# dattalab-6-cam/multicam-calibration

Hardware: AMD Instinct MI355X
Metric: LM iterations/sec (6 cams x 10k frames x 54 pts per GPU shard; + ms/Jacobian-eval) (higher is better)
Workload: dtype f64

## Files before the change

multicam-calibration_amd/build.py:

```python
import hashlib
import os
import shutil
import subprocess
import sys

PKG = os.path.dirname(os.path.abspath(__file__))
CSRC = os.path.join(PKG, "csrc")
LIB = os.path.join(PKG, "libmcba.so")
SOURCES = ["mcba_kernels.hip", "mcba_solve.hip", "mcba_triangulate.hip", "mcba_diag.hip", "mcba_calib.hip", "mcba_pnp.hip", "mcba_flat.hip", "mcba_api.hip", "mcba_lm_api.hip",
           "mcba_prefilter_api.hip", "mcba_calib_api.hip", "mcba_geom_api.hip", "mcba_comm_api.hip", "mcba_sparse.hip", "mcba_sparse_api.hip", "mcba_detect.hip", "mcba_keypoints.hip", "mcba_consensus.hip", "mcba_cov.hip", "mcba_cov_api.hip",
           "mcba_tricov.hip", "mcba_tricov_api.hip", "mcba_kpba.hip", "mcba_kpba_tiled.hip", "mcba_kpba_api.hip", "mcba_kpcam.hip", "mcba_kpcam_api.hip", "mcba_twoview.hip", "mcba_fivepoint.hip", "mcba_twoview_api.hip", "mcba_resect.hip", "mcba_resect_p3p.hip", "mcba_resect_api.hip",
           "mcba_smooth.hip", "mcba_smooth_api.hip", "mcba_smooth_cov.hip", "mcba_smooth_cov_api.hip", "mcba_traj_refine.hip", "mcba_traj_refine_api.hip"]
DEPS = SOURCES + ["mcba_gram_finish.inc", "mcba_math.h", "mcba_geom_math.h", "mcba_pnp_math.h", "mcba_keypoint_math.h", "mcba_consensus_math.h", "mcba_cov_math.h", "mcba_tricov_math.h", "mcba_kpba_math.h", "mcba_kpcam_math.h", "mcba_detect_math.h", "mcba_twoview_math.h", "mcba_fivepoint_math.h", "mcba_resect_math.h", "mcba_resect_p3p_math.h", "mcba_smooth_math.h", "mcba_smooth_cov_math.h", "mcba_traj_refine_math.h", "mcba_smooth_host.h", "mcba_hyp_score.h", "mcba_ransac_host.h", "mcba_device.h", "mcba_quadform.h", "mcba_backsub.h", "mcba_kernels.h", "mcba_gram_plan.h", "mcba_lm.h", "mcba_lm_state.h", "mcba_handle.h", os.path.join("..", "..", "include", "mcba.h")]


SCHED_FLAGS = ["-mllvm", "-amdgpu-disable-unclustered-high-rp-reschedule=1", "-mllvm", "-greedy-reverse-local-assignment=1"]


def hipcc_path():
    for cand in (shutil.which("hipcc"), "/opt/rocm/bin/hipcc"):
        if cand and os.path.exists(cand):
            return cand
    raise RuntimeError("hipcc not found: libmcba.so cannot be built (ROCm toolchain required)")


def is_stale():
    if not os.path.exists(LIB):
        return True
    t = os.path.getmtime(LIB)
    return any(os.path.getmtime(os.path.join(CSRC, d)) > t for d in DEPS)


def build(force=False, verbose=False, out=None):
    if out is None and not force and not is_stale():
        return LIB
    from concurrent.futures import ThreadPoolExecutor

    extra = os.environ.get("MCBA_HIPCC_FLAGS", "").split()
    common = [hipcc_path(), "-O3", "--offload-arch=gfx950", "-std=c++17", "-fPIC"] + SCHED_FLAGS + extra
    tag = hashlib.sha1(repr((out, common[1:])).encode()).hexdigest()[:12]
    objdir = os.path.join(CSRC, ".obj" if out is None and not extra else ".obj_" + tag)
    os.makedirs(objdir, exist_ok=True)
    flags_file = os.path.join(objdir, "flags.txt")
    flags_now = " ".join(common[1:])
    flags_same = os.path.exists(flags_file) and open(flags_file).read() == flags_now
    headers = [os.path.join(CSRC, d) for d in DEPS if d not in SOURCES]
    hdr_time = max(os.path.getmtime(hh) for hh in headers)

    def compile_one(src):
        obj = os.path.join(objdir, src.replace(".hip", ".o"))
        srcp = os.path.join(CSRC, src)
        if not force and flags_same and os.path.exists(obj) and os.path.getmtime(obj) > max(os.path.getmtime(srcp), hdr_time):
            return obj
        tmp = obj + ".%d.tmp" % os.getpid()
        cmd = common + ["-c", "-o", tmp, srcp]
        if verbose:
            print(" ".join(cmd))
        subprocess.check_call(cmd, cwd=CSRC)
        os.replace(tmp, obj)
        return obj

    with ThreadPoolExecutor(max_workers=min(len(SOURCES), os.cpu_count() or 2, 16)) as ex:
        objs = list(ex.map(compile_one, SOURCES))
    with open(flags_file, "w") as fh:
        fh.write(flags_now)
    target = out or LIB
    tmp_lib = target + ".%d.tmp" % os.getpid()
    cmd = [hipcc_path(), "--offload-arch=gfx950", "-fPIC", "-shared", "-o", tmp_lib, "-ldl"] + objs
    if verbose:
        print(" ".join(cmd))
    subprocess.check_call(cmd, cwd=CSRC)
    os.replace(tmp_lib, target)
    return target


if __name__ == "__main__":
    out = sys.argv[sys.argv.index("--out") + 1] if "--out" in sys.argv else None
    print(build(force="--force" in sys.argv, verbose=True, out=out))
```

multicam-calibration_amd/csrc/mcba_api.hip:

```cpp
#include <map>
#include <mutex>

#include "mcba_handle.h"

namespace mcba_internal {

thread_local std::string g_err;

struct ParkedBuf {
  void* p;
  hipStream_t stream;
  bool busy;
};
struct BufferPool {
  std::mutex mu;
  std::multimap<std::pair<int, size_t>, ParkedBuf> dev;
  std::multimap<std::pair<unsigned, size_t>, void*> host;
  size_t parked = 0, parked_host = 0;
  const size_t host_cap = (size_t)256 << 20;
  size_t cap() {
    static size_t c = [] { const char* e = getenv("MCBA_POOL_MB"); return (size_t)(e ? atoll(e) : 2048) << 20; }();
    return c;
  }
};
static BufferPool g_pool;

static void pool_release_all();
hipError_t pool_malloc(void** p, size_t bytes, int device, hipStream_t stream, bool any_stream) {
  {
    ParkedBuf got{nullptr, nullptr, false};
    {
      std::lock_guard<std::mutex> lk(g_pool.mu);
      auto it = g_pool.dev.find({device, bytes});
      if (it != g_pool.dev.end()) { got = it->second; g_pool.dev.erase(it); g_pool.parked -= bytes; }
    }
    if (got.p) {
      if (got.busy && (any_stream || got.stream != stream)) (void)hipStreamSynchronize(got.stream);
      *p = got.p;
      return hipSuccess;
    }
  }
  hipError_t e = hipMalloc(p, bytes);
  if (e == hipErrorOutOfMemory) {
    (void)hipGetLastError();
    pool_release_all();
    e = hipMalloc(p, bytes);
  }
  return e;
}
void pool_free(void* p, size_t bytes, int device, hipStream_t stream, bool busy) {
  if (!p) return;
  {
    std::lock_guard<std::mutex> lk(g_pool.mu);
    if (g_pool.parked + bytes <= g_pool.cap()) { g_pool.dev.insert({{device, bytes}, ParkedBuf{p, stream, busy}}); g_pool.parked += bytes; return; }
  }
  if (busy) (void)hipStreamSynchronize(stream);
  (void)hipFree(p);
}
hipError_t pool_host_malloc(void** p, size_t bytes, unsigned flags) {
  {
    std::lock_guard<std::mutex> lk(g_pool.mu);
    auto it = g_pool.host.find({flags, bytes});
    if (it != g_pool.host.end()) { *p = it->second; g_pool.host.erase(it); g_pool.parked_host -= bytes; return hipSuccess; }
  }
  return hipHostMalloc(p, bytes, flags);
}
void pool_host_free(void* p, size_t bytes, unsigned flags) {
  if (!p) return;
  std::lock_guard<std::mutex> lk(g_pool.mu);
  if (g_pool.cap() == 0 || g_pool.parked_host + bytes > g_pool.host_cap) { (void)hipHostFree(p); return; }
  g_pool.host.insert({{flags, bytes}, p});
  g_pool.parked_host += bytes;
}
static void pool_release_all() {
  std::lock_guard<std::mutex> lk(g_pool.mu);
  int cur = 0;
  (void)hipGetDevice(&cur);
  for (auto& kv : g_pool.dev) { (void)hipSetDevice(kv.first.first); if (kv.second.busy) (void)hipStreamSynchronize(kv.second.stream); (void)hipFree(kv.second.p); }
  for (auto& kv : g_pool.host) (void)hipHostFree(kv.second);
  g_pool.dev.clear();
  g_pool.host.clear();
  g_pool.parked = g_pool.parked_host = 0;
  (void)hipSetDevice(cur);
}

int poison_byte() {
  static const int b = [] { const char* e = getenv("MCBA_POISON"); const int v = e ? atoi(e) : 0; return v == 1 ? 0xFF : (v == 2 ? 0x3F : 0); }();
  return b;
}

}

using namespace mcba_internal;

static int tile_tables(int device, int NT, int** ti, int** tj) {
  static std::mutex mu;
  static std::map<std::pair<int, int>, std::pair<int*, int*>> cache;
  std::lock_guard<std::mutex> lk(mu);
  auto it = cache.find({device, NT});
  if (it == cache.end()) {
    std::vector<int> ci, cj;
    for (int a = 0; a < NT; ++a) for (int b = a; b < NT; ++b) { ci.push_back(a); cj.push_back(b); }
    int *di = nullptr, *dj = nullptr;
    HIPCHK(hipMalloc(reinterpret_cast<void**>(&di), ci.size() * sizeof(int)));
    HIPCHK(hipMalloc(reinterpret_cast<void**>(&dj), cj.size() * sizeof(int)));
    HIPCHK(hipMemcpy(di, ci.data(), ci.size() * sizeof(int), hipMemcpyHostToDevice));
    HIPCHK(hipMemcpy(dj, cj.data(), cj.size() * sizeof(int), hipMemcpyHostToDevice));
    it = cache.insert({{device, NT}, {di, dj}}).first;
  }
  *ti = it->second.first;
  *tj = it->second.second;
  return MCBA_OK;
}

static int derive_geometry(mcba_handle* h) {
  const int C = h->C, F = h->F, N = h->N, device = h->device;
  const int ncu = h->ncu, slots = 4 * h->ncu;
  h->n = h->cw * C;
  h->nsys = (size_t)h->n * h->n + 3 * h->n + 16;
  if (h->sparse) {
    h->NT = h->NP = h->G = h->sq = h->sr = 0;
    h->FS = 0;
    h->ppw = 4;
  } else {
  h->NT = (h->n + 1 + 15) / 16;
  h->NP = h->NT * (h->NT + 1) / 2;
  h->ppw = h->NP <= 64 ? 4 : 16;
  h->FS = 8;
  while (h->FS > 2 && (mcba::syrk_lds_bytes(C, h->FS, h->cw) > (size_t)h->lds_optin * 3 / 5 || (h->n + 1) * h->FS > 256 * mcba::syrk_items_per_thread())) h->FS /= 2;
  if ((h->n + 1) * h->FS > 256 * mcba::syrk_items_per_thread()) { return fail(MCBA_ERR_ARG, "too many cameras for k_syrk's per-thread item budget"); }
  if (mcba::syrk_lds_bytes(C, h->FS, h->cw) > (size_t)h->lds_optin) { return fail(MCBA_ERR_ARG, "too many cameras for the LDS staging of k_syrk"); }
  {
    int nstage = (F + h->FS - 1) / h->FS;
    int gmax = h->ppw == 4 ? std::min(512, 2 * ncu) : std::max(1, ncu / ((h->NP + 63) / 64));
    int g = std::min(nstage, gmax);
    if (h->ppw == 4) {
      h->G = g;
      h->sq = nstage / g;
      h->sr = nstage % g;
    } else {
      h->sq = (nstage + g - 1) / g;
      h->sr = 0;
      h->G = (nstage + h->sq - 1) / h->sq;
    }
  }
  }
  h->nbblocks = h->Fpad / 64;
  {
    static bool ps_ready[64] = {};
    static std::mutex ps_mu;
    bool ps_ok = (size_t)h->lds_optin >= mcba::kGramPsplitLdsMax + 2048;
    {
      std::lock_guard<std::mutex> lk(ps_mu);
      if (ps_ok && !ps_ready[device & 63]) { ps_ok = mcba::gram_psplit_set_lds_limit() == 0; ps_ready[device & 63] = ps_ok; (void)hipGetLastError(); }
    }
    mcba::GramShape shape{C, h->nfb, N, slots, h->cw, ps_ok, -1, -1};
    if (const char* e = getenv("MCBA_GRAM_SPLIT")) shape.force_split = std::max(0, std::min(5, atoi(e)));
    if (const char* e = getenv("MCBA_GRAM_NPW")) shape.force_npw = atoi(e) == 2 ? 2 : 4;
    h->gram = mcba::gram_plan(shape);
    if (h->gram.refused) { return fail(MCBA_ERR_ARG, "MCBA_GRAM_SPLIT=4/5: this device cannot give k_gram_psplit its LDS"); }
  }
  h->nch = std::max(1, std::min(std::min(8, N / 8), (4 * slots + C * h->nfb - 1) / (C * h->nfb)));
  h->nfblocks = h->G;
  h->npad = 16 * h->NT;
  h->solve_lds = mcba::solve_fits_lds(h->npad, h->lds_optin);
  if (h->sparse) {
    h->nfblocks = h->nfb;
    h->npad = mcba::sp_npad(h->n);
    h->solve_lds = 0;
  }
  return MCBA_OK;
}

static int compose_dscale(mcba_handle* h) {
  const bool any_frozen = !h->frozen_host.empty();
  h->have_red = false;
  if (h->xs_host.empty() && !any_frozen) { h->have_xscale = false; return MCBA_OK; }
  std::vector<double> d(h->nx, 0.0);
  const size_t cnt = (size_t)12 * h->C + (size_t)6 * h->F, ncam = (size_t)12 * h->C;
  for (size_t i = 0; i < cnt; ++i) {
    d[i] = h->xs_host.empty() ? 0.0 : h->xs_host[i];
    if (any_frozen && i >= ncam && h->frozen_host[i]) d[i] = -1.0;
  }
  HIPCHK(hipMemcpyAsync(h->dscale, d.data(), h->nx * sizeof(double), hipMemcpyHostToDevice, h->stream));
  HIPCHK(hipStreamSynchronize(h->stream));
  h->have_xscale = true;
  return MCBA_OK;
}

static int ensure_res(mcba_handle* h) {
  if (!h->res) return dalloc(h, &h->res, (size_t)2 * h->C * h->F * h->N, false);
  return MCBA_OK;
}


namespace mcba_internal {

int ensure_solver(mcba_handle* h) {
  if (h->have_solver) return MCBA_OK;
  const int C = h->C;
  int rc;
  if (!h->solver_arena) {
    struct Piece { double** p; size_t count; };
    size_t n_swork = h->solve_lds ? 16 : 2 * (size_t)h->npad * h->npad + 64 * (size_t)h->npad;
    if (h->sparse) n_swork = (size_t)h->npad * h->npad;
    Piece zeroed[] = {{&h->gpart2[0], (size_t)C * h->nfb * MCBA_GP}, {&h->gpart2[1], (size_t)C * h->nfb * MCBA_GP}, {&h->fbuf, (size_t)h->Fpad * MCBA_FB}, {&h->fpart, (size_t)2 * h->nfblocks},
                      {&h->cpart, (size_t)2 * C * h->nfb * h->nch}, {&h->bpart, (size_t)3 * h->nbblocks}, {&h->red_own, h->nsys + 8 + 2 * MCBA_LMS},
                      {&h->dcbuf, (size_t)h->n + 8},
                      {&h->swork, n_swork}, {&h->dscale, h->nx}, {reinterpret_cast<double**>(&h->fixed), ((size_t)h->n + 7) / 8},
                      {&h->sp_damp, h->sparse ? (size_t)h->npad : 0}, {&h->sp_y, h->sparse ? (size_t)h->npad : 0}, {reinterpret_cast<double**>(&h->sp_ctl), h->sparse ? (size_t)1 : 0}};
    Piece plain[] = {{&h->rec2[0], (size_t)h->Fpad * C * MCBA_REC}, {&h->rec2[1], (size_t)h->Fpad * C * MCBA_REC},
                     {&h->spart, (size_t)h->G * h->NP * 256 + 64},
                     {&h->gchunk, h->gram.chunk_doubles()}};
    auto padded = [](size_t count) { return (std::max<size_t>(count, 1) * sizeof(double) + 255) / 256 * 256; };
    size_t zero_bytes = 0, total = 0;
    for (auto& pc : zeroed) if (pc.count) zero_bytes += padded(pc.count);
    total = zero_bytes;
    for (auto& pc : plain) if (pc.count) total += padded(pc.count);
    if ((rc = dalloc(h, &h->solver_arena, total, false)) != MCBA_OK) return rc;
    HIPCHK(hipMemsetAsync(h->solver_arena, 0, zero_bytes, h->stream));
    if (poison_byte()) HIPCHK(hipMemsetAsync(h->solver_arena + zero_bytes, poison_byte(), total - zero_bytes, h->stream));
    size_t off = 0;
    for (auto& pc : zeroed) if (pc.count) { *pc.p = reinterpret_cast<double*>(h->solver_arena + off); off += padded(pc.count); }
    for (auto& pc : plain) if (pc.count) { *pc.p = reinterpret_cast<double*>(h->solver_arena + off); off += padded(pc.count); }
  }
  if (h->sparse) {
    h->sp_A = h->swork;
  } else if (mcba::solve_set_lds_limit(h->npad, h->solve_lds) != 0) return fail(MCBA_ERR_HIP, "cannot raise the dynamic LDS limit of k_solve_cam");
  h->fuse_backsub = h->solve_lds != 0;
  if (const char* e = getenv("MCBA_FUSE_BACKSUB")) h->fuse_backsub = h->fuse_backsub && atoi(e) != 0;
  if (h->fuse_backsub && mcba::solve_backsub_set_lds_limit(h->npad, h->cw) != 0) h->fuse_backsub = false;
  h->fuse_max_polls = 200000;
  if (const char* e = getenv("MCBA_FUSE_MAX_POLLS")) h->fuse_max_polls = std::max(0, atoi(e));
  if (!h->ring) {
    h->ring_bytes = ((size_t)kRing * MCBA_LMS + 8) * sizeof(double);
    h->ring_flags = hipHostMallocMapped | hipHostMallocCoherent;
    hipError_t e = pool_host_malloc(reinterpret_cast<void**>(&h->ring), h->ring_bytes, h->ring_flags);
    if (e != hipSuccess) { (void)hipGetLastError(); h->ring_flags = hipHostMallocDefault; e = pool_host_malloc(reinterpret_cast<void**>(&h->ring), h->ring_bytes, h->ring_flags); }
    if (e != hipSuccess) return fail(MCBA_ERR_HIP, "cannot allocate the host-mapped LM state ring");
    memset(h->ring, 0, h->ring_bytes);
    if (hipHostGetDevicePointer(reinterpret_cast<void**>(&h->ring_dev), h->ring, 0) != hipSuccess) return fail(MCBA_ERR_HIP, "hipHostGetDevicePointer failed for the LM state ring");
  }
  h->red = h->red_own;
  if (!h->sparse && (rc = tile_tables(h->device, h->NT, &h->tile_i, &h->tile_j)) != MCBA_OK) return rc;
  if (!h->pinned) {
    h->pinned_bytes = (h->nsys + 8 + MCBA_LMS + h->n) * sizeof(double);
    HIPCHK(pool_host_malloc(reinterpret_cast<void**>(&h->pinned), h->pinned_bytes, hipHostMallocDefault));
  }
  size_t lds = h->sparse ? 0 : mcba::syrk_lds_bytes(C, h->FS, h->cw);
  if (lds > 64 * 1024) {
    if (mcba::syrk_set_lds_limit(lds) != 0) return fail(MCBA_ERR_HIP, "cannot raise the dynamic LDS limit of k_syrk");
  }
  h->have_solver = true;
  if (!h->xs_host.empty() || !h->frozen_host.empty()) return compose_dscale(h);
  return MCBA_OK;
}
int upload_impl(mcba_handle* h, const double* uvs, const double* objpoints, bool sync) {
  size_t raw_count = (size_t)2 * h->C * h->F * h->N;
  hipError_t e = hipMemcpyAsync(h->obs_raw, uvs, raw_count * sizeof(double), hipMemcpyHostToDevice, h->stream);
  if (e == hipSuccess && !mcba::launch_store_small(h->stream, h->obj, objpoints, (size_t)3 * h->N))
    e = hipMemcpyAsync(h->obj, objpoints, (size_t)3 * h->N * sizeof(double), hipMemcpyHostToDevice, h->stream);
  if (e == hipSuccess) {
    Scope sc(h, K_TRANSPOSE);
    mcba::launch_transpose_obs(h->stream, h->obs_raw, h->obs_t, h->C, h->F, h->N, h->Fpad);
  }
  if (e == hipSuccess) e = hipGetLastError();
  hipError_t e2 = sync ? hipStreamSynchronize(h->stream) : hipSuccess;
  if (e != hipSuccess || e2 != hipSuccess) { g_err = std::string("upload: ") + hipGetErrorString(e != hipSuccess ? e : e2); return MCBA_ERR_HIP; }
  if (!h->obj_host) h->obj_host = static_cast<double*>(malloc((size_t)3 * h->N * sizeof(double)));
  if (h->obj_host) memcpy(h->obj_host, objpoints, (size_t)3 * h->N * sizeof(double));
  h->planar = 1;
  for (int p = 0; p < h->N; ++p) if (objpoints[3 * p + 2] != 0.0) h->planar = 0;
  if (const char* e = getenv("MCBA_GRAM_FAST")) { if (atoi(e) == 0) h->planar = 0; }
  h->have_obs = true;
  h->have_lin = h->have_red = h->have_jac = false;
  h->sp_ready = false;
  return MCBA_OK;
}

int gram_launch(mcba_handle* h, mcba::Sel sel, const double* xa, const double* xb, int la, int lb) {
  sel.cfl = h->curv_floor;
  { Scope sc(h, K_GRAM); mcba::launch_gram(h->stream, h->loss, h->f_scale, h->obs_t, h->obj, sel, xa, xb, h->rec2[la], h->rec2[lb], h->gpart2[la], h->gpart2[lb], h->C, h->N, h->Fpad, h->gram, h->planar, h->gchunk, h->loss_tab); }
  return check_launch();
}

int trial_sum(mcba_handle* h, mcba::Sel sel, int la, int lb, const mcba::DecideArgs& da) {
  { Scope sc(h, K_SUM_TRIAL); mcba::launch_sum_trial(h->stream, sel, h->gpart2[la] + (size_t)90 * h->nfb, h->gpart2[lb] + (size_t)90 * h->nfb, 1, h->nfb, (size_t)MCBA_GP * h->nfb, h->C * h->nfb, h->bpart, h->nbblocks, h->red + h->nsys, da); }
  return check_launch();
}

int backsub_launch(mcba_handle* h, mcba::Sel sel, int la, int lb, int xa, int xb, const double* delta_cam) {
  if (h->sparse && delta_cam) {
    HIPCHK(hipMemcpyAsync(h->dcbuf, delta_cam, (size_t)h->n * sizeof(double), hipMemcpyHostToDevice, h->stream));
    delta_cam = nullptr;
  }
  mcba::CamStep cs;
  if (delta_cam) memcpy(cs.v, delta_cam, h->n * sizeof(double));
  {
    Scope sc(h, K_BACKSUB);
    if (delta_cam) mcba::launch_backsub(h->stream, sel, h->rec2[la], h->rec2[lb], h->fbuf, cs, h->x[xa], h->x[xb], h->bpart, h->C, h->F, h->Fpad, h->cw);
    else mcba::launch_backsub_dev(h->stream, sel, h->rec2[la], h->rec2[lb], h->fbuf, h->dcbuf, h->x[xa], h->x[xb], h->bpart, h->C, h->F, h->Fpad, h->cw);
  }
  return check_launch();
}

int syrk_launch(mcba_handle* h, mcba::Sel sel, const mcba::SyrkFuse& fz) {
  if (h->sparse) {
    if (fz.decide) return fail(MCBA_ERR_ARG, "sparse-Schur handle: the decision is not fused into the Schur reduction");
    return sparse_build(h, sel);
  }
  { Scope sc(h, K_SYRK); mcba::launch_syrk(h->stream, sel, fz, h->rec2[0], h->rec2[1], h->fbuf, h->fpart, h->tile_i, h->tile_j, h->spart, h->C, h->F, h->Fpad, h->NT, h->NP, h->G, h->sq, h->sr, h->FS, h->ppw, h->have_xscale ? h->dscale : nullptr, h->cw); }
  return check_launch();
}

int reduce_launch(mcba_handle* h, mcba::Sel sel, int rank_slot, bool spec) {
  {
    Scope sc(h, K_REDUCE);
    mcba::launch_reduce_system(h->stream, sel, h->gpart2[0], h->gpart2[1], h->spart, h->fpart, h->tile_i, h->tile_j, h->red, h->C, h->nfb, h->G, h->NT, h->NP, h->nfblocks, rank_slot,
                               spec ? h->bpart : nullptr, h->nbblocks, spec ? post_state(h) : nullptr, h->cw, spec ? timeout_word(h) : nullptr, (double)h->last_solve_seq);
  }
  return check_launch();
}

}

extern "C" {

int mcba_abi_version(void) { return 7; }
const char* mcba_last_error(void) { return g_err.c_str(); }
const char* mcba_profile_names(void) { return kKernelNames; }

int mcba_device_count(int* count) {
  if (!count) return fail(MCBA_ERR_ARG, "count is NULL");
  hipError_t e = hipGetDeviceCount(count);
  if (e != hipSuccess) { *count = 0; g_err = hipGetErrorString(e); return MCBA_ERR_NODEVICE; }
  return MCBA_OK;
}

}

namespace mcba_internal {
int create_impl(mcba_handle** out, int C, int F, int N, int device, bool sparse) {
  const char* who = sparse ? "mcba_create_sparse" : "mcba_create";
  if (!out || C < 1 || F < 1 || N < 1) { g_err = std::string(who) + ": need cameras >= 1, frames >= 1, points >= 1"; return MCBA_ERR_ARG; }
  if (!sparse && C > 40) {
    g_err = "mcba_create: " + std::to_string(C) + " cameras -- this build handles at most 40 per handle: the (12 C + 1)-row reduced camera system is factorised by ONE workgroup "
            "(k_solve_cam: tile tables, LDS and scratch are sized for 481 rows) and k_backsub takes the camera step through the kernel arguments (480 doubles); reduced_solver=\"host\" does not "
            "lift it (the Schur product's tile grid has the same bound).  The reference has no such limit (scipy's sparse LSMR); the sparse-Schur handle (mcba_create_sparse; ops.Problem(..., schur=\"sparse\"), bundle_adjust's default above 40 cameras) has none";
    return MCBA_ERR_ARG;
  }
  int ndev = 0;
  if (hipGetDeviceCount(&ndev) != hipSuccess || ndev == 0) return fail(MCBA_ERR_NODEVICE, "no HIP device visible");
  if (device < 0 || device >= ndev) return fail(MCBA_ERR_ARG, "device ordinal out of range");
  HIPCHK(hipSetDevice(device));
  mcba_handle* h = new mcba_handle();
  h->C = C; h->F = F; h->N = N; h->device = device;
  h->sparse = sparse;
  h->speculate = !sparse;
  {
    hipDeviceProp_t prop;
    if (hipGetDeviceProperties(&prop, device) == hipSuccess) {
      if (prop.multiProcessorCount > 0) h->ncu = prop.multiProcessorCount;
      if (prop.sharedMemPerBlockOptin > 0) h->lds_optin = (int)std::min<size_t>(prop.sharedMemPerBlockOptin, 160 * 1024);
    }
  }
  if (const char* e = getenv("MCBA_STRICT_SYNC")) h->strict_sync = atoi(e) != 0;
  h->Fpad = (F + 63) / 64 * 64;
  h->nfb = h->Fpad / 64;
  h->nx = (size_t)12 * C + (size_t)6 * h->Fpad;
  {
    const int grc = derive_geometry(h);
    if (grc != MCBA_OK) { delete h; return grc; }
  }
  int rc;
#define DA(p, cnt, zero) if ((rc = dalloc(h, &h->p, (cnt), zero)) != MCBA_OK) { mcba_destroy(h); return rc; }
  DA(obs_t, (size_t)2 * C * N * h->Fpad, false);
  DA(obs_raw, (size_t)2 * C * F * N, false);
  {
    const size_t nxp = (h->nx + 31) / 32 * 32;
    DA(core_arena, 2 * nxp + (size_t)3 * N, true);
    h->x[0] = h->core_arena; h->x[1] = h->core_arena + nxp; h->obj = h->core_arena + 2 * nxp;
  }
#undef DA
  *out = h;
  return MCBA_OK;
}
}

extern "C" {

int mcba_create(mcba_handle** out, int C, int F, int N, int device) { return create_impl(out, C, F, N, device, false); }

int mcba_create_sparse(mcba_handle** out, int C, int F, int N, int device) { return create_impl(out, C, F, N, device, true); }
int mcba_is_sparse(const mcba_handle* h) { return h && h->sparse ? 1 : 0; }

int mcba_destroy(mcba_handle* h) {
  if (!h) return MCBA_OK;
  (void)hipSetDevice(h->device);
  const bool quiet = h->last_solve_seq == h->waited_seq && h->evs.empty() && !h->comm && !h->prof;
  if (!quiet) (void)hipStreamSynchronize(h->stream);
  if (h->comm && g_rccl.ok) { g_rccl.CommDestroy(h->comm); h->comm = nullptr; }
  for (auto& b : h->bufs) { pool_free(*b.slot, b.bytes, h->device, h->stream, quiet); *b.slot = nullptr; }
  free(h->obj_host);
  pool_host_free(h->pinned, h->pinned_bytes, hipHostMallocDefault);
  pool_host_free(h->ring, h->ring_bytes, h->ring_flags);
  pool_host_free(h->pf_host, h->pf_host_bytes, hipHostMallocDefault);
  for (auto& e : h->evs) { (void)hipEventDestroy(e.a); (void)hipEventDestroy(e.b); }
  for (auto& e : h->pool) (void)hipEventDestroy(e);
  delete h;
  return MCBA_OK;
}

size_t mcba_device_bytes(const mcba_handle* h) {
  size_t tot = 0;
  if (h) for (auto& b : h->bufs) tot += b.bytes;
  return tot;
}

int mcba_trim(mcba_handle* h) {
  if (!h) return fail(MCBA_ERR_ARG, "NULL handle");
  HIPCHK(hipSetDevice(h->device));
  HIPCHK(hipStreamSynchronize(h->stream));
  void** keep[] = {reinterpret_cast<void**>(&h->obs_t), reinterpret_cast<void**>(&h->obs_raw), reinterpret_cast<void**>(&h->core_arena), reinterpret_cast<void**>(&h->sub_frames),
                   reinterpret_cast<void**>(&h->blo), reinterpret_cast<void**>(&h->bhi)};
  std::vector<DevBuf> kept;
  for (auto& b : h->bufs) {
    bool k = false;
    for (void** s : keep) k = k || b.slot == s;
    if (k) { kept.push_back(b); continue; }
    pool_free(*b.slot, b.bytes, h->device);
    *b.slot = nullptr;
  }
  h->bufs.swap(kept);
  h->rec2[0] = h->rec2[1] = h->gpart2[0] = h->gpart2[1] = h->fbuf = h->fpart = h->spart = h->cpart = h->bpart = h->red_own = h->red = h->dcbuf = h->swork = h->dscale = h->gchunk = nullptr;
  h->fixed = nullptr;
  sparse_forget(h);
  h->cal_out_cap = h->cal_rel_cap = h->cal_sel_cap = h->cal_views_cap = 0;
  h->have_cal_poses = false;
  h->have_solver = h->have_lin = h->have_red = h->have_spec = h->have_jac = h->auto_ready = h->have_xscale = h->have_fixed = h->trial_ready = false;
  return MCBA_OK;
}

int mcba_download_observations(mcba_handle* h, double* uvs) {
  if (!h || !uvs) return fail(MCBA_ERR_ARG, "mcba_download_observations: bad argument");
  if (!h->have_obs) return fail(MCBA_ERR_ARG, "mcba_download_observations: no observations");
  HIPCHK(hipSetDevice(h->device));
  HIPCHK(hipMemcpyAsync(uvs, h->obs_raw, (size_t)2 * h->C * h->F * h->N * sizeof(double), hipMemcpyDeviceToHost, h->stream));
  HIPCHK(hipStreamSynchronize(h->stream));
  return MCBA_OK;
}

int mcba_pool_trim(void) {
  pool_release_all();
  return MCBA_OK;
}

int mcba_set_stream(mcba_handle* h, void* s) {
  if (!h) return fail(MCBA_ERR_ARG, "NULL handle");
  if (h->stream != reinterpret_cast<hipStream_t>(s)) HIPCHK(hipStreamSynchronize(h->stream));
  h->stream = reinterpret_cast<hipStream_t>(s);
  return MCBA_OK;
}

int mcba_synchronize(mcba_handle* h) {
  if (!h) return fail(MCBA_ERR_ARG, "NULL handle");
  HIPCHK(hipStreamSynchronize(h->stream));
  return MCBA_OK;
}

int mcba_upload_observations(mcba_handle* h, const double* uvs, const double* objpoints) {
  if (!h || !uvs || !objpoints) return fail(MCBA_ERR_ARG, "mcba_upload_observations: NULL argument");
  HIPCHK(hipSetDevice(h->device));
  return upload_impl(h, uvs, objpoints, true);
}

int mcba_set_loss(mcba_handle* h, int loss, double f_scale) {
  if (!h || loss < 0 || loss > 4 || !(f_scale > 0.0)) return fail(MCBA_ERR_ARG, "mcba_set_loss: loss in 0..4 and f_scale > 0 required");
  h->loss = loss; h->f_scale = f_scale;
  h->have_lin = h->have_red = false;
  return MCBA_OK;
}

int mcba_set_loss_table(mcba_handle* h, const double* tab3) {
  if (!h || !tab3) return fail(MCBA_ERR_ARG, "mcba_set_loss_table: NULL argument");
  if (!h->have_obs) return fail(MCBA_ERR_ARG, "mcba_set_loss_table: upload observations first");
  HIPCHK(hipSetDevice(h->device));
  int rc = ensure_res(h);
  if (rc) return rc;
  const size_t raw = (size_t)2 * h->C * h->F * h->N, plane = (size_t)2 * h->C * h->N * h->Fpad;
  if (!h->loss_tab && (rc = dalloc(h, &h->loss_tab, 3 * plane, false))) return rc;
  for (int k = 0; k < 3; ++k) {
    HIPCHK(hipMemcpyAsync(h->res, tab3 + k * raw, raw * sizeof(double), hipMemcpyHostToDevice, h->stream));
    mcba::launch_transpose_obs(h->stream, h->res, h->loss_tab + k * plane, h->C, h->F, h->N, h->Fpad);
  }
  if ((rc = check_launch())) return rc;
  HIPCHK(hipStreamSynchronize(h->stream));
  h->loss = mcba::LOSS_TABLE;
  h->f_scale = 1.0;
  h->have_lin = h->have_red = false;
  return MCBA_OK;
}

int mcba_set_camera_block(mcba_handle* h, int width) {
  if (!h || (width != 6 && width != 12)) return fail(MCBA_ERR_ARG, "mcba_set_camera_block: width 6 or 12");
  if (width == h->cw) return MCBA_OK;
  if (h->have_solver || h->solver_arena) return fail(MCBA_ERR_ARG, "mcba_set_camera_block: call it before the first solver entry point of the handle");
  if (width == 6 && !h->sparse) {
    const int nt = (6 * h->C + 1 + 15) / 16;
    if (nt * (nt + 1) / 2 > 64) return fail(MCBA_ERR_ARG, "mcba_set_camera_block: more than 26 cameras -- hold the intrinsics with the flags of mcba_lm_auto_config instead");
  }
  const int old = h->cw;
  h->cw = width;
  HIPCHK(hipSetDevice(h->device));
  const int rc = derive_geometry(h);
  if (rc != MCBA_OK) { h->cw = old; (void)derive_geometry(h); return rc; }
  h->have_lin = h->have_red = h->have_spec = false;
  h->auto_ready = false;
  return MCBA_OK;
}
int mcba_get_camera_block(const mcba_handle* h) { return h ? h->cw : 0; }

int mcba_set_curvature_floor(mcba_handle* h, double floor) {
  if (!h || !(floor > 0.0) || floor > 1.0) return fail(MCBA_ERR_ARG, "mcba_set_curvature_floor: 0 < floor <= 1");
  h->curv_floor = floor;
  return MCBA_OK;
}
double mcba_get_curvature_floor(const mcba_handle* h) { return h ? h->curv_floor : 0.0; }

int mcba_set_params(mcba_handle* h, int slot, const double* x) {
  if (!slot_ok(h, slot) || !x) return fail(MCBA_ERR_ARG, "mcba_set_params: bad handle/slot/pointer");
  HIPCHK(hipSetDevice(h->device));
  HIPCHK(hipMemcpyAsync(h->x[slot], x, ((size_t)12 * h->C + (size_t)6 * h->F) * sizeof(double), hipMemcpyHostToDevice, h->stream));
  HIPCHK(hipStreamSynchronize(h->stream));
  return MCBA_OK;
}

int mcba_get_params(mcba_handle* h, int slot, double* x) {
  if (!slot_ok(h, slot) || !x) return fail(MCBA_ERR_ARG, "mcba_get_params: bad handle/slot/pointer");
  HIPCHK(hipSetDevice(h->device));
  HIPCHK(hipMemcpyAsync(x, h->x[slot], ((size_t)12 * h->C + (size_t)6 * h->F) * sizeof(double), hipMemcpyDeviceToHost, h->stream));
  HIPCHK(hipStreamSynchronize(h->stream));
  return MCBA_OK;
}

int mcba_copy_params(mcba_handle* h, int dst, int src) {
  if (!slot_ok(h, dst) || !slot_ok(h, src)) return fail(MCBA_ERR_ARG, "mcba_copy_params: bad slot");
  if (dst == src) return MCBA_OK;
  HIPCHK(hipMemcpyAsync(h->x[dst], h->x[src], h->nx * sizeof(double), hipMemcpyDeviceToDevice, h->stream));
  return MCBA_OK;
}

static int run_cost(mcba_handle* h, int slot, double* res_dev, const double* bpart, int nbp) {
  {
    Scope sc(h, K_COST);
    mcba::launch_cost(h->stream, h->loss, h->f_scale, h->obs_t, h->obj, h->x[slot], h->cpart, res_dev, h->C, h->F, h->N, h->Fpad, h->nch);
  }
  int rc = check_launch();
  if (rc) return rc;
  {
    Scope sc(h, K_SUM_TRIAL);
    mcba::launch_sum_trial(h->stream, host_sel(0), h->cpart, h->cpart, 2, h->C * h->nfb * h->nch, 0, h->C * h->nfb * h->nch, bpart, nbp, h->red + h->nsys, mcba::DecideArgs{0, 0.0, 0.0, 0.0, 0.0, 0.0, nullptr});
  }
  return check_launch();
}

static int fetch_trial(mcba_handle* h, double* host8) {
  HIPCHK(hipMemcpyAsync(h->pinned + h->nsys, h->red + h->nsys, 8 * sizeof(double), hipMemcpyDeviceToHost, h->stream));
  HIPCHK(hipStreamSynchronize(h->stream));
  memcpy(host8, h->pinned + h->nsys, 8 * sizeof(double));
  return MCBA_OK;
}

int mcba_cost(mcba_handle* h, int slot, double* cost, double* n_residuals) {
  if (!slot_ok(h, slot) || !cost) return fail(MCBA_ERR_ARG, "mcba_cost: bad argument");
  if (!h->have_obs) return fail(MCBA_ERR_ARG, "mcba_cost: upload observations first");
  HIPCHK(hipSetDevice(h->device));
  NEED_SOLVER(h);
  int rc = run_cost(h, slot, nullptr, nullptr, 0);
  if (rc) return rc;
  double t[8];
  rc = fetch_trial(h, t);
  if (rc) return rc;
  *cost = t[0];
  if (n_residuals) *n_residuals = t[4];
  if (!isfinite(t[0])) return fail(MCBA_ERR_NONFINITE, "Residuals are not finite");
  return MCBA_OK;
}

int mcba_residuals(mcba_handle* h, int slot, double* res) {
  if (!slot_ok(h, slot) || !res) return fail(MCBA_ERR_ARG, "mcba_residuals: bad argument");
  if (!h->have_obs) return fail(MCBA_ERR_ARG, "mcba_residuals: upload observations first");
  HIPCHK(hipSetDevice(h->device));
  NEED_SOLVER(h);
  int rc = ensure_res(h);
  if (rc) return rc;
  rc = run_cost(h, slot, h->res, nullptr, 0);
  if (rc) return rc;
  HIPCHK(hipMemcpyAsync(res, h->res, (size_t)2 * h->C * h->F * h->N * sizeof(double), hipMemcpyDeviceToHost, h->stream));
  HIPCHK(hipStreamSynchronize(h->stream));
  return MCBA_OK;
}

int mcba_jacobian_eval(mcba_handle* h, int slot, int robust_scaled) {
  if (!slot_ok(h, slot)) return fail(MCBA_ERR_ARG, "mcba_jacobian_eval: bad argument");
  if (!h->have_obs) return fail(MCBA_ERR_ARG, "mcba_jacobian_eval: upload observations first");
  HIPCHK(hipSetDevice(h->device));
  int rc = ensure_res(h);
  if (rc) return rc;
  if (!h->jac) {
    rc = dalloc(h, &h->jac, (size_t)36 * h->C * h->F * h->N, false);
    if (rc) return rc;
  }
  {
    Scope sc(h, K_JACOBIAN);
    mcba::launch_jacobian(h->stream, h->loss, h->f_scale, h->obs_raw, h->obj, h->x[slot], h->jac, h->res, h->C, h->F, h->N, h->Fpad, robust_scaled);
  }
  rc = check_launch();
  if (rc) return rc;
  h->have_jac = true;
  return MCBA_OK;
}

int mcba_jacobian_download(mcba_handle* h, double* jac, double* res) {
  if (!h) return fail(MCBA_ERR_ARG, "NULL handle");
  if (!h->have_jac) return fail(MCBA_ERR_ARG, "mcba_jacobian_download: call mcba_jacobian_eval first");
  size_t cnt = (size_t)h->C * h->F * h->N;
  if (jac) HIPCHK(hipMemcpyAsync(jac, h->jac, cnt * 36 * sizeof(double), hipMemcpyDeviceToHost, h->stream));
  if (res) HIPCHK(hipMemcpyAsync(res, h->res, cnt * 2 * sizeof(double), hipMemcpyDeviceToHost, h->stream));
  HIPCHK(hipStreamSynchronize(h->stream));
  return MCBA_OK;
}

int mcba_linearize(mcba_handle* h, int slot) {
  if (!slot_ok(h, slot)) return fail(MCBA_ERR_ARG, "mcba_linearize: bad argument");
  if (!h->have_obs) return fail(MCBA_ERR_ARG, "mcba_linearize: upload observations first");
  if (h->loss == mcba::LOSS_TABLE && !h->loss_tab) return fail(MCBA_ERR_ARG, "mcba_linearize: the loss table was released (mcba_trim): call mcba_set_loss_table again");
  HIPCHK(hipSetDevice(h->device));
  NEED_SOLVER(h);
  int rc = gram_launch(h, host_sel(0), h->x[slot], h->x[slot], h->lin, h->lin);
  if (rc) return rc;
  h->have_lin = true;
  h->have_red = false;
  h->have_spec = false;
  return MCBA_OK;
}

int mcba_build_reduced(mcba_handle* h, double lambda, int rank_slot) {
  if (!h || !(lambda >= 0.0) || rank_slot < 0 || rank_slot > 11) return fail(MCBA_ERR_ARG, "mcba_build_reduced: lambda >= 0 and rank_slot in 0..11 required");
  if (!h->have_lin) return fail(MCBA_ERR_ARG, "mcba_build_reduced: call mcba_linearize first");
  HIPCHK(hipSetDevice(h->device));
  int rc;
  if ((rc = syrk_launch(h, host_sel(h->lin, lambda), no_fuse()))) return rc;
  if ((rc = reduce_launch(h, host_sel(h->lin), rank_slot, false))) return rc;
  h->have_red = true;
  return MCBA_OK;
}

size_t mcba_reduced_size(const mcba_handle* h) { return h ? h->nsys + 8 + 2 * MCBA_LMS : 0; }

int mcba_bind_reduce_buffer(mcba_handle* h, double* p) {
  if (!h) return fail(MCBA_ERR_ARG, "NULL handle");
  HIPCHK(hipSetDevice(h->device));
  NEED_SOLVER(h);
  h->red = p ? p : h->red_own;
  h->have_red = false;
  return MCBA_OK;
}

int mcba_get_reduced(mcba_handle* h, double* host) {
  if (!h || !host) return fail(MCBA_ERR_ARG, "mcba_get_reduced: bad argument");
  if (!h->have_red) return fail(MCBA_ERR_ARG, "mcba_get_reduced: call mcba_build_reduced first");
  HIPCHK(hipMemcpyAsync(h->pinned, h->red, h->nsys * sizeof(double), hipMemcpyDeviceToHost, h->stream));
  HIPCHK(hipStreamSynchronize(h->stream));
  memcpy(host, h->pinned, h->nsys * sizeof(double));
  return MCBA_OK;
}

static int step_common(mcba_handle* h, const double* delta_cam, double lambda, int src, int dst) {
  int rc = backsub_launch(h, host_sel(0, lambda), h->lin, h->lin, src, dst, delta_cam);
  if (rc || !h->have_bounds) return rc;
  mcba::launch_clip(h->stream, h->x[dst], h->blo, h->bhi, (size_t)12 * h->C + (size_t)6 * h->F);
  return check_launch();
}

int mcba_step(mcba_handle* h, const double* delta_cam, double lambda, int src, int dst) {
  if (!slot_ok(h, src) || !slot_ok(h, dst) || src == dst || !delta_cam) return fail(MCBA_ERR_ARG, "mcba_step: bad argument (slots must differ)");
  if (!h->have_red) return fail(MCBA_ERR_ARG, "mcba_step: call mcba_build_reduced first");
  HIPCHK(hipSetDevice(h->device));
  int rc = step_common(h, delta_cam, lambda, src, dst);
  if (rc) return rc;
  h->have_spec = false;
  return run_cost(h, dst, nullptr, h->bpart, h->nbblocks);
}

int mcba_step_linearize(mcba_handle* h, const double* delta_cam, double lambda, int src, int dst) {
  if (!slot_ok(h, src) || !slot_ok(h, dst) || src == dst || !delta_cam) return fail(MCBA_ERR_ARG, "mcba_step_linearize: bad argument (slots must differ)");
  if (!h->have_red) return fail(MCBA_ERR_ARG, "mcba_step_linearize: call mcba_build_reduced first");
  if (h->loss == mcba::LOSS_TABLE) return fail(MCBA_ERR_ARG, "mcba_step_linearize: a tabulated loss is set -- step (mcba_step), evaluate the function at the trial residuals, mcba_set_loss_table, then mcba_linearize");
  HIPCHK(hipSetDevice(h->device));
  int rc = step_common(h, delta_cam, lambda, src, dst);
  if (rc) return rc;
  const int alt = 1 - h->lin;
  if ((rc = gram_launch(h, host_sel(0), h->x[dst], h->x[dst], alt, alt))) return rc;
  if ((rc = trial_sum(h, host_sel(0), alt, alt, mcba::DecideArgs{0, 0.0, 0.0, 0.0, 0.0, 0.0, nullptr}))) return rc;
  h->have_spec = true;
  return MCBA_OK;
}

int mcba_accept_linearization(mcba_handle* h) {
  if (!h) return fail(MCBA_ERR_ARG, "NULL handle");
  if (!h->have_spec) return fail(MCBA_ERR_ARG, "mcba_accept_linearization: no speculative linearisation (call mcba_step_linearize first)");
  h->lin = 1 - h->lin;
  h->have_spec = false;
  h->have_red = false;
  return MCBA_OK;
}

int mcba_get_trial(mcba_handle* h, double* host8) {
  if (!h || !host8) return fail(MCBA_ERR_ARG, "mcba_get_trial: bad argument");
  return fetch_trial(h, host8);
}

int mcba_set_trial(mcba_handle* h, const double* host8) {
  if (!h || !host8 || !h->red) return fail(MCBA_ERR_ARG, "mcba_set_trial: bad argument, or no reduce buffer yet (call mcba_step first)");
  HIPCHK(hipSetDevice(h->device));
  memcpy(h->pinned + h->nsys, host8, 8 * sizeof(double));
  HIPCHK(hipMemcpyAsync(h->red + h->nsys, h->pinned + h->nsys, 8 * sizeof(double), hipMemcpyHostToDevice, h->stream));
  HIPCHK(hipStreamSynchronize(h->stream));
  return MCBA_OK;
}

int mcba_reduce_fetch(mcba_handle* h, double lambda, int rank_slot, double* host) {
  int rc = mcba_build_reduced(h, lambda, rank_slot);
  if (rc) return rc;
  return mcba_get_reduced(h, host);
}

int mcba_step_fetch(mcba_handle* h, const double* delta_cam, double lambda, int src, int dst, int linearize, double* host8) {
  int rc = linearize ? mcba_step_linearize(h, delta_cam, lambda, src, dst) : mcba_step(h, delta_cam, lambda, src, dst);
  if (rc) return rc;
  return mcba_get_trial(h, host8);
}

int mcba_set_x_scale(mcba_handle* h, const double* x_scale) {
  if (!h) return fail(MCBA_ERR_ARG, "NULL handle");
  HIPCHK(hipSetDevice(h->device));
  NEED_SOLVER(h);
  if (!x_scale) {
    if (h->xs_host.empty() && h->frozen_host.empty()) { h->have_red = false; h->have_xscale = false; return MCBA_OK; }
    h->xs_host.clear();
    return compose_dscale(h);
  }
  const size_t cnt = (size_t)12 * h->C + (size_t)6 * h->F;
  std::vector<double> d(cnt);
  for (size_t i = 0; i < cnt; ++i) {
    if (!(x_scale[i] > 0.0) || !std::isfinite(x_scale[i])) return fail(MCBA_ERR_ARG, "`x_scale` must be 'jac' or array_like with positive numbers.");
    d[i] = 1.0 / (x_scale[i] * x_scale[i]);
  }
  h->xs_host.swap(d);
  return compose_dscale(h);
}

int mcba_set_frozen(mcba_handle* h, const unsigned char* mask) {
  if (!h) return fail(MCBA_ERR_ARG, "NULL handle");
  HIPCHK(hipSetDevice(h->device));
  NEED_SOLVER(h);
  const size_t cnt = (size_t)12 * h->C + (size_t)6 * h->F, ncam = (size_t)12 * h->C;
  bool any = false;
  if (mask) for (size_t i = ncam; i < cnt; ++i) any = any || mask[i] != 0;
  if (!any) {
    if (h->frozen_host.empty()) return MCBA_OK;
    h->frozen_host.clear();
    return compose_dscale(h);
  }
  h->frozen_host.assign(mask, mask + cnt);
  return compose_dscale(h);
}

int mcba_set_bounds(mcba_handle* h, const double* lo, const double* hi) {
  if (!h || (lo == nullptr) != (hi == nullptr)) return fail(MCBA_ERR_ARG, "mcba_set_bounds: bad argument");
  HIPCHK(hipSetDevice(h->device));
  if (!lo) { h->have_bounds = false; return MCBA_OK; }
  const size_t cnt = (size_t)12 * h->C + (size_t)6 * h->F;
  for (size_t i = 0; i < cnt; ++i)
    if (!(lo[i] < hi[i])) return fail(MCBA_ERR_ARG, "Each lower bound must be strictly less than each upper bound.");
  int rc;
  if (!h->blo && (rc = dalloc(h, &h->blo, h->nx, false))) return rc;
  if (!h->bhi && (rc = dalloc(h, &h->bhi, h->nx, false))) return rc;
  std::vector<double> a(h->nx, -INFINITY), b(h->nx, INFINITY);
  memcpy(a.data(), lo, cnt * sizeof(double));
  memcpy(b.data(), hi, cnt * sizeof(double));
  HIPCHK(hipMemcpyAsync(h->blo, a.data(), h->nx * sizeof(double), hipMemcpyHostToDevice, h->stream));
  HIPCHK(hipMemcpyAsync(h->bhi, b.data(), h->nx * sizeof(double), hipMemcpyHostToDevice, h->stream));
  HIPCHK(hipStreamSynchronize(h->stream));
  h->have_bounds = true;
  return MCBA_OK;
}


int mcba_residuals_detach(mcba_handle* h, int slot, mcba_buffer** out) {
  if (!slot_ok(h, slot) || !out) return fail(MCBA_ERR_ARG, "mcba_residuals_detach: bad argument");
  if (!h->have_obs) return fail(MCBA_ERR_ARG, "mcba_residuals_detach: upload observations first");
  HIPCHK(hipSetDevice(h->device));
  NEED_SOLVER(h);
  int rc = ensure_res(h);
  if (rc) return rc;
  {
    Scope sc(h, K_COST);
    mcba::launch_cost(h->stream, h->loss, h->f_scale, h->obs_t, h->obj, h->x[slot], h->cpart, h->res, h->C, h->F, h->N, h->Fpad, h->nch, NAN);
  }
  if ((rc = check_launch())) return rc;
  mcba_buffer* b = new mcba_buffer{h->res, (size_t)2 * h->C * h->F * h->N, h->device, h->stream, h->res, (size_t)2 * h->C * h->F * h->N};
  for (size_t i = 0; i < h->bufs.size(); ++i)
    if (h->bufs[i].slot == reinterpret_cast<void**>(&h->res)) { h->bufs.erase(h->bufs.begin() + i); break; }
  h->res = nullptr;
  h->have_jac = false;
  *out = b;
  return MCBA_OK;
}
size_t mcba_buffer_count(const mcba_buffer* b) { return b ? b->count : 0; }
int mcba_buffer_download(mcba_buffer* b, double* host) {
  if (!b || !host) return fail(MCBA_ERR_ARG, "mcba_buffer_download: bad argument");
  HIPCHK(hipSetDevice(b->device));
  HIPCHK(hipMemcpyAsync(host, b->dev, b->count * sizeof(double), hipMemcpyDeviceToHost, b->stream));
  HIPCHK(hipStreamSynchronize(b->stream));
  return MCBA_OK;
}
int mcba_buffer_free(mcba_buffer* b) {
  if (!b) return MCBA_OK;
  (void)hipSetDevice(b->device);
  pool_free(b->base, b->base_count * sizeof(double), b->device, b->stream, true);
  delete b;
  return MCBA_OK;
}
int mcba_fp64_issue_rate(int device, double* tflops) {
  if (!tflops) return fail(MCBA_ERR_ARG, "mcba_fp64_issue_rate: NULL");
  *tflops = 0.0;
  if (int rc = stateless_device(device)) return rc;
  hipDeviceProp_t prop;
  int ncu = 256;
  if (hipGetDeviceProperties(&prop, device) == hipSuccess && prop.multiProcessorCount > 0) ncu = prop.multiProcessorCount;
  *tflops = mcba::measure_fp64_issue_rate(ncu);
  if (!(*tflops > 0.0)) return fail(MCBA_ERR_HIP, "mcba_fp64_issue_rate: the measurement kernel failed");
  return MCBA_OK;
}

int mcba_profile_enable(mcba_handle* h, int on) {
  if (!h) return fail(MCBA_ERR_ARG, "NULL handle");
  h->prof = on != 0;
  h->prof_mask = (on == 0 || on == 1) ? ~0u : ((unsigned)on >> 1);
  h->prof_stride = 1;
  h->prof_exact = false;
  return MCBA_OK;
}

int mcba_profile_exact(mcba_handle* h, int on) {
  if (!h) return fail(MCBA_ERR_ARG, "NULL handle");
  h->prof_exact = on != 0;
  return MCBA_OK;
}

int mcba_profile_stride(mcba_handle* h, int stride) {
  if (!h || stride < 1) return fail(MCBA_ERR_ARG, "mcba_profile_stride: stride >= 1 required");
  h->prof_stride = stride;
  return MCBA_OK;
}

int mcba_profile_bracket_overhead(mcba_handle* h, int pairs, double* us) {
  if (!h || !us || pairs < 1 || pairs > 4096) return fail(MCBA_ERR_ARG, "mcba_profile_bracket_overhead: bad argument");
  HIPCHK(hipSetDevice(h->device));
  std::vector<hipEvent_t> ev(2 * (size_t)pairs);
  for (auto& e : ev) HIPCHK(hipEventCreate(&e));
  HIPCHK(hipStreamSynchronize(h->stream));
  for (int i = 0; i < pairs; ++i) { HIPCHK(hipEventRecord(ev[2 * i], h->stream)); HIPCHK(hipEventRecord(ev[2 * i + 1], h->stream)); }
  HIPCHK(hipStreamSynchronize(h->stream));
  double tot = 0.0;
  for (int i = 0; i < pairs; ++i) { float ms = 0.f; HIPCHK(hipEventElapsedTime(&ms, ev[2 * i], ev[2 * i + 1])); tot += ms; }
  for (auto& e : ev) (void)hipEventDestroy(e);
  *us = 1e3 * tot / pairs;
  return MCBA_OK;
}

int mcba_profile_read(mcba_handle* h, double* ms_total, int* calls, int capacity, int* n_kernels) {
  if (!h || !ms_total || !calls || capacity < K_COUNT) return fail(MCBA_ERR_ARG, "mcba_profile_read: need capacity >= number of kernels");
  HIPCHK(hipStreamSynchronize(h->stream));
  for (int i = 0; i < K_COUNT; ++i) { ms_total[i] = 0.0; calls[i] = 0; }
  for (auto& e : h->evs) {
    float ms = 0.f;
    if (hipEventElapsedTime(&ms, e.a, e.b) == hipSuccess) { ms_total[e.kid] += ms; calls[e.kid] += 1; }
    h->pool.push_back(e.a);
    h->pool.push_back(e.b);
  }
  h->evs.clear();
  if (n_kernels) *n_kernels = K_COUNT;
  return MCBA_OK;
}

}
```

multicam-calibration_amd/csrc/mcba_handle.h:

```cpp
#pragma once
#include <hip/hip_runtime.h>
#include <math.h>
#include <stdlib.h>
#include <string.h>
#include <algorithm>
#include <rccl/rccl.h>
#include <string>
#include <vector>

#include "../../include/mcba.h"
#include "mcba_kernels.h"
#include "mcba_math.h"

namespace mcba_internal {

extern thread_local std::string g_err;

enum KernelId { K_TRANSPOSE = 0, K_GRAM, K_COST, K_SYRK, K_REDUCE, K_BACKSUB, K_SUM_TRIAL, K_JACOBIAN, K_DECIDE, K_SOLVE,
                K_SP_FACTOR, K_SP_PAIRS, K_SP_SOLVE_PRE, K_SP_POTRF, K_SP_TRSM, K_SP_UPDATE, K_SP_FINISH, K_COUNT };
constexpr const char* kKernelNames = "k_transpose_obs\nk_gram\nk_cost\nk_syrk\nk_reduce_system\nk_backsub\nk_sum_trial\nk_jacobian\nk_decide\nk_solve_cam"
                                     "\nk_sp_factor\nk_sp_pairs\nk_sp_solve_pre\nk_sp_potrf\nk_sp_trsm\nk_sp_update\nk_sp_finish";
constexpr int kRing = 16;

struct EvRec { int kid; hipEvent_t a, b; };
struct DevBuf { void** slot; size_t bytes; };

}

struct mcba_handle {
  int C = 0, F = 0, N = 0, Fpad = 0, nfb = 0, n = 0;
  int device = 0;
  hipStream_t stream = nullptr;
  int loss = MCBA_LOSS_SOFT_L1;
  double f_scale = 1.0;
  bool have_obs = false, have_lin = false, have_red = false, have_jac = false;
  double *obs_t = nullptr, *obs_raw = nullptr, *obj = nullptr, *x[2] = {nullptr, nullptr};
  double *rec2[2] = {nullptr, nullptr}, *gpart2[2] = {nullptr, nullptr}, *fbuf = nullptr, *fpart = nullptr;
  int lin = 0;
  bool have_spec = false;
  double *spart = nullptr, *cpart = nullptr, *bpart = nullptr;
  double *red_own = nullptr, *red = nullptr;
  double *jac = nullptr, *res = nullptr;
  double *err = nullptr, *dmean = nullptr, *dfull = nullptr, *repro = nullptr, *trans = nullptr, *und = nullptr;
  mcba::SelState* sel = nullptr;
  unsigned char* fmask = nullptr;
  unsigned char *pf_state = nullptr, *pf_status = nullptr, *pf_packed = nullptr, *pf_host = nullptr;
  double* pf_worst = nullptr;
  size_t pf_host_bytes = 0;
  double* core_arena = nullptr;
  unsigned char* solver_arena = nullptr;
  int* sub_frames = nullptr;
  double* cov_work = nullptr;
  double* outbuf = nullptr;
  double *cal_intr = nullptr, *cal_poses_t = nullptr, *cal_out = nullptr, *cal_rel = nullptr, *cal_world = nullptr;
  unsigned char *cal_valid = nullptr, *cal_nit = nullptr;
  mcba::SelState* cal_sel = nullptr;
  int* cal_views = nullptr;
  size_t cal_out_cap = 0, cal_rel_cap = 0, cal_sel_cap = 0, cal_views_cap = 0;
  bool have_cal_poses = false;
  double* obj_host = nullptr;
  int planar = 0;
  int *tile_i = nullptr, *tile_j = nullptr;
  int NT = 0, NP = 0, G = 0, sq = 0, sr = 0, FS = 0, ppw = 4, nfblocks = 0, nbblocks = 0, nch = 1;
  mcba::GramPlan gram;
  double* gchunk = nullptr;
  double curv_floor = 1.0;
  int cw = 12;
  size_t nx = 0, nsys = 0;
  double* pinned = nullptr;
  ncclComm_t comm = nullptr;
  double *dcbuf = nullptr, *swork = nullptr;
  double* dscale = nullptr;
  bool have_xscale = false;
  std::vector<double> xs_host;
  std::vector<unsigned char> frozen_host;
  double *blo = nullptr, *bhi = nullptr;
  bool have_bounds = false;
  double* loss_tab = nullptr;
  int fuse_max_polls = 200000;
  bool strict_sync = true;
  unsigned char* fixed = nullptr;
  bool have_fixed = false, auto_ready = false;
  bool speculate = true;
  double* ring = nullptr;
  double* ring_dev = nullptr;
  int npad = 0, solve_lds = 0;
  bool fuse_backsub = false, trial_ready = false;
  unsigned long long last_solve_seq = 0;
  unsigned long long waited_seq = 0;
  unsigned long long solve_launches = 0;
  int ncu = 256, lds_optin = 160 * 1024;
  bool spec_copy_ready = false;
  double ftol = 1e-8, xtol = 1e-8, gtol = 1e-8, lam_min = 1e-12, lam_max = 1e12;
  double dec_floor = 0.0;
  bool prof = false;
  unsigned prof_mask = ~0u;
  int prof_stride = 1;
  bool prof_exact = false;
  unsigned prof_count[32] = {};
  std::vector<mcba_internal::EvRec> evs;
  std::vector<hipEvent_t> pool;
  std::vector<mcba_internal::DevBuf> bufs;
  std::vector<double> hist;
  bool have_solver = false;
  size_t ring_bytes = 0, pinned_bytes = 0;
  unsigned ring_flags = 0;
  bool sparse = false, sp_ready = false;
  int sp_nent = 0, sp_npairs = 0, sp_nchunks = 0;
  int *sp_index = nullptr, *sp_frame_off = nullptr, *sp_ent_cam = nullptr, *sp_ent_frame = nullptr, *sp_items = nullptr, *sp_chunks = nullptr, *sp_pair_map = nullptr, *sp_pair_chunks = nullptr;
  int* sp_ctl = nullptr;
  double *sp_Y = nullptr, *sp_part = nullptr, *sp_A = nullptr, *sp_damp = nullptr, *sp_y = nullptr;
  size_t sp_index_ints = 0, sp_Y_count = 0, sp_part_count = 0;
};

struct mcba_buffer { double* dev; size_t count; int device; hipStream_t stream; double* base; size_t base_count; };

namespace mcba_internal {

#define HIPCHK(expr)                                                                                     \
  do {                                                                                                   \
    hipError_t e_ = (expr);                                                                              \
    if (e_ != hipSuccess) {                                                                              \
      mcba_internal::g_err = std::string(#expr) + ": " + hipGetErrorString(e_);                          \
      return MCBA_ERR_HIP;                                                                               \
    }                                                                                                    \
  } while (0)

inline int fail(int code, const char* msg) { g_err = msg; return code; }

inline int check_launch() {
  hipError_t e = hipGetLastError();
  if (e != hipSuccess) { g_err = std::string("kernel launch: ") + hipGetErrorString(e); return MCBA_ERR_HIP; }
  return MCBA_OK;
}

inline hipEvent_t get_event(mcba_handle* h) {
  if (!h->pool.empty()) { hipEvent_t e = h->pool.back(); h->pool.pop_back(); return e; }
  hipEvent_t e;
  (void)hipEventCreate(&e);
  return e;
}

struct Scope {
  mcba_handle* h; int kid; hipEvent_t a{}, b{};
  bool on, exact;
  Scope(mcba_handle* h_, int k) : h(h_), kid(k), on(h_->prof && ((h_->prof_mask >> k) & 1u) && (h_->prof_count[k]++ % (unsigned)h_->prof_stride) == 0), exact(false) {
    if (!on) return;
    a = get_event(h); b = get_event(h);
    exact = h->prof_exact && k == K_GRAM;
    if (exact) mcba::gram_time_next_launch(a, b);
    else (void)hipEventRecord(a, h->stream);
  }
  ~Scope() {
    if (!on) return;
    if (exact && mcba::gram_time_pending()) {
      mcba::gram_time_next_launch(nullptr, nullptr);
      h->pool.push_back(a); h->pool.push_back(b);
      return;
    }
    if (!exact) (void)hipEventRecord(b, h->stream);
    h->evs.push_back({kid, a, b});
  }
};

hipError_t pool_malloc(void** p, size_t bytes, int device, hipStream_t stream = nullptr, bool any_stream = false);
void pool_free(void* p, size_t bytes, int device, hipStream_t stream = nullptr, bool busy = false);
hipError_t pool_host_malloc(void** p, size_t bytes, unsigned flags);
void pool_host_free(void* p, size_t bytes, unsigned flags);
int poison_byte();

template <class T>
int dalloc(mcba_handle* h, T** p, size_t count, bool zero = true) {
  const size_t bytes = std::max<size_t>(count, 1) * sizeof(T);
  HIPCHK(pool_malloc(reinterpret_cast<void**>(p), bytes, h->device, h->stream));
  h->bufs.push_back({reinterpret_cast<void**>(p), bytes});
  if (zero) HIPCHK(hipMemsetAsync(*p, 0, bytes, h->stream));
  else if (int pz = poison_byte()) HIPCHK(hipMemsetAsync(*p, pz, bytes, h->stream));
  return MCBA_OK;
}

struct RcclApi {
  bool ok = false;
  ncclResult_t (*GetUniqueId)(ncclUniqueId*) = nullptr;
  ncclResult_t (*CommInitRank)(ncclComm_t*, int, ncclUniqueId, int) = nullptr;
  ncclResult_t (*AllReduce)(const void*, void*, size_t, ncclDataType_t, ncclRedOp_t, ncclComm_t, hipStream_t) = nullptr;
  ncclResult_t (*CommDestroy)(ncclComm_t) = nullptr;
  ncclResult_t (*CommCount)(const ncclComm_t, int*) = nullptr;
  const char* (*GetErrorString)(ncclResult_t) = nullptr;
};
extern RcclApi g_rccl;

inline int stateless_device(int device, const char* who = nullptr) {
  int ndev = 0;
  if (hipGetDeviceCount(&ndev) != hipSuccess || ndev == 0) return fail(MCBA_ERR_NODEVICE, "no HIP device visible");
  if (device < 0 || device >= ndev) { g_err = who ? std::string(who) + ": device ordinal out of range" : "device ordinal out of range"; return MCBA_ERR_ARG; }
  HIPCHK(hipSetDevice(device));
  return MCBA_OK;
}

inline int lds_optin_of(int device) {
  hipDeviceProp_t prop;
  if (hipGetDeviceProperties(&prop, device) == hipSuccess && prop.sharedMemPerBlockOptin > 0) return (int)std::min<size_t>(prop.sharedMemPerBlockOptin, 160 * 1024);
  return 64 * 1024;
}

struct StatelessCall {
  std::vector<void*> bufs;
  hipEvent_t e0 = nullptr, e1 = nullptr;
  ~StatelessCall() {
    for (void* b : bufs) (void)hipFree(b);
    if (e0) (void)hipEventDestroy(e0);
    if (e1) (void)hipEventDestroy(e1);
  }
  template <class T>
  int alloc(T** p, size_t count, bool poison) {
    const size_t bytes = count * sizeof(T) > 0 ? count * sizeof(T) : 16;
    void* v = nullptr;
    HIPCHK(hipMalloc(&v, bytes));
    bufs.push_back(v);
    *p = static_cast<T*>(v);
    if (int pz = poison ? poison_byte() : 0) HIPCHK(hipMemset(v, pz, bytes));
    return MCBA_OK;
  }
  template <class T>
  int scratch(T** p, size_t count) { return alloc(p, count, true); }
  template <class T>
  int put(T* dst, const T* host, size_t count) {
    HIPCHK(hipMemcpy(dst, host, count * sizeof(T), hipMemcpyHostToDevice));
    return MCBA_OK;
  }
  template <class T>
  int upload(T** p, const T* host, size_t count) {
    if (int rc = alloc(p, count, false)) return rc;
    return put(*p, host, count);
  }
  template <class T>
  int download(T* host, const T* src, size_t count) {
    HIPCHK(hipMemcpy(host, src, count * sizeof(T), hipMemcpyDeviceToHost));
    return MCBA_OK;
  }
  hipError_t start() {
    hipError_t e = hipEventCreate(&e0);
    if (e == hipSuccess) e = hipEventCreate(&e1);
    if (e == hipSuccess) e = hipEventRecord(e0, nullptr);
    return e;
  }
  hipError_t stop(double* kernel_ms) {
    hipError_t e = hipEventRecord(e1, nullptr);
    if (e == hipSuccess) e = hipEventSynchronize(e1);
    if (e == hipSuccess && kernel_ms) {
      float ms = 0.f;
      e = hipEventElapsedTime(&ms, e0, e1);
      *kernel_ms = ms;
    }
    return e;
  }
};

template <int N>
struct StageEvents {
  hipEvent_t ev[N] = {};
  int marked = 0;
  ~StageEvents() { for (hipEvent_t e : ev) if (e) (void)hipEventDestroy(e); }
  hipError_t create() {
    hipError_t e = hipSuccess;
    for (int i = 0; i < N && e == hipSuccess; ++i) e = hipEventCreate(&ev[i]);
    return e;
  }
  hipError_t mark() { return hipEventRecord(ev[marked++], nullptr); }
  hipError_t fill(const StatelessCall& call, double total, double* kernel_ms) const {
    double ms[N + 2] = {total};
    for (int i = 0; i <= N; ++i) {
      float span = 0.f;
      hipError_t e = hipEventElapsedTime(&span, i == 0 ? call.e0 : ev[i - 1], i == N ? call.e1 : ev[i]);
      if (e != hipSuccess) return e;
      ms[1 + i] = span;
    }
    for (int i = 0; i < N + 2; ++i) kernel_ms[i] = ms[i];
    return hipSuccess;
  }
};

inline int check_weights(const char* who, const double* weights, size_t count) {
  if (!weights) return MCBA_OK;
  for (size_t i = 0; i < count; ++i)
    if (weights[i] < 0.0 || weights[i] > 1.7976931348623157e308) {
      g_err = std::string(who) + ": weights must be finite and not negative (0 or NaN = the detection is unseen)";
      return MCBA_ERR_ARG;
    }
  return MCBA_OK;
}
inline int upload_sqrt_weights(StatelessCall& call, const double* weights, size_t count, double** d_sw) {
  *d_sw = nullptr;
  if (!weights) return MCBA_OK;
  std::vector<double> sq(count);
  for (size_t i = 0; i < count; ++i) sq[i] = weights[i] > 0.0 ? sqrt(weights[i]) : 0.0;
  return call.upload(d_sw, sq.data(), count);
}

inline int slot_ok(const mcba_handle* h, int slot) { return h && (slot == 0 || slot == 1); }

int create_impl(mcba_handle** out, int C, int F, int N, int device, bool sparse);
int ensure_solver(mcba_handle* h);
#define NEED_SOLVER(h) do { int rc_ = mcba_internal::ensure_solver(h); if (rc_) return rc_; } while (0)
int upload_impl(mcba_handle* h, const double* uvs, const double* objpoints, bool sync);

inline mcba::Sel host_sel(int idx, double lam = 0.0) { return mcba::Sel{nullptr, idx, lam, 0, 0.0}; }
inline mcba::Sel dev_sel(const mcba_handle* h, int flip) { return mcba::Sel{h->red + h->nsys + 8, flip, 0.0, 0, 0.0}; }
inline mcba::Sel spec_sel(const mcba_handle* h) { return mcba::Sel{h->red + h->nsys + 8, 0, h->lam_min, 1, h->dec_floor}; }
inline double* post_state(const mcba_handle* h) { return h->red + h->nsys + 8 + MCBA_LMS; }
inline mcba::Sel post_sel(const mcba_handle* h) { return mcba::Sel{post_state(h), 0, 0.0, 0, 0.0}; }
inline double* timeout_word(const mcba_handle* h) { return h->dcbuf + h->n + 1; }
inline mcba::SyrkFuse no_fuse() { mcba::SyrkFuse z{}; return z; }

int gram_launch(mcba_handle* h, mcba::Sel sel, const double* xa, const double* xb, int la, int lb);
int trial_sum(mcba_handle* h, mcba::Sel sel, int la, int lb, const mcba::DecideArgs& da);
int backsub_launch(mcba_handle* h, mcba::Sel sel, int la, int lb, int xa, int xb, const double* delta_cam);
int syrk_launch(mcba_handle* h, mcba::Sel sel, const mcba::SyrkFuse& fz);
int reduce_launch(mcba_handle* h, mcba::Sel sel, int rank_slot, bool spec);

int sparse_build(mcba_handle* h, mcba::Sel sel);
int sparse_solve(mcba_handle* h, const mcba::SolveArgs& a);
void sparse_forget(mcba_handle* h);

}
```

multicam-calibration_amd/csrc/mcba_kernels.h:

```cpp
#pragma once
#include <hip/hip_runtime.h>
#include <stddef.h>

#include <type_traits>

#define MCBA_REC 100
#define MCBA_GP 92
#define MCBA_FB 40

#include "mcba_gram_plan.h"
#include "mcba_lm_state.h"
#include "mcba_math.h"

namespace mcba {
template <int... Vs, class F>
int with_int(int v, F&& f) {
  int rc = 1;
  (void)((v == Vs && ((rc = f(std::integral_constant<int, Vs>{})), true)) || ...);
  return rc;
}
template <int... Vs>
struct IntList {};
template <int... Vs, class F>
int with_int(IntList<Vs...>, int v, F&& f) { return with_int<Vs...>(v, f); }
template <int... Vs, class F>
void for_each_int(IntList<Vs...>, F&& f) { (f(std::integral_constant<int, Vs>{}), ...); }
using LossList = IntList<LOSS_LINEAR, LOSS_SOFT_L1, LOSS_HUBER, LOSS_CAUCHY, LOSS_ARCTAN>;
template <class F>
int with_loss(int loss, F&& f) { return with_int(LossList{}, loss, f); }
template <class F>
int with_bool(bool b, F&& f) { return b ? f(std::true_type{}) : f(std::false_type{}); }
template <class F>
void for_each_bool(F&& f) { f(std::false_type{}); f(std::true_type{}); }
template <class F>
int with_weights(const double* sw, F&& f) { return with_bool(sw != nullptr, f); }
template <class... P, class... A>
int launch(void (*kernel)(P...), dim3 grid, dim3 block, size_t lds, hipStream_t st, const A&... args) {
  hipLaunchKernelGGL(kernel, grid, block, lds, st, args...);
  return 0;
}
template <class... P, class... A>
int launch_with_lds(void (*kernel)(P...), dim3 grid, size_t lds, hipStream_t st, A... args) {
  if (lds > 64 * 1024 && hipFuncSetAttribute(reinterpret_cast<const void*>(kernel), hipFuncAttributeMaxDynamicSharedMemorySize, (int)lds) != hipSuccess) return 1;
  return launch(kernel, grid, dim3(256), lds, st, args...);
}

struct CamStep {
  double v[480];
};

struct Sel {
  const double* lms;
  int idx;
  double lam;
  int spec;
  double dec;
  double cfl = 1.0;
};
struct SyrkFuse {
  int decide;
  const double* cp0;
  const double* cp1;
  int cinner;
  int cstride;
  int cdense;
  size_t couter;
  int ncp;
  const double* bpart;
  int nbp;
  double* trial_out;
  double* lms_post;
  DecideArgs da;
  const double* timeout_word;
  double seq_prev;
};
struct SolveArgs {
  const double* red;
  const double* lms_in;
  double* lms;
  double* work;
  double* dc;
  const double* x0;
  const double* x1;
  const unsigned char* fixed;
  const double* dscale;
  double* host_state;
  double* flag;
  const double* timeout_word;
  double seq;
  double gtol, lam_max;
  int n, npad, use_lds;
  int cw;
  int decide;
  double lam_min, ftol, xtol;
  double dec_floor;
  double stage_tag;
};
void launch_transpose_obs(hipStream_t st, const double* raw, double* obs_t, int C, int F, int N, int Fpad);
void launch_gram(hipStream_t st, int loss, double f_scale, const double* obs_t, const double* obj, Sel s, const double* x0, const double* x1, double* rec0, double* rec1, double* gp0, double* gp1, int C, int N, int Fpad,
                 const GramPlan& plan, int planar = 0, double* chunk = nullptr, const double* ltab = nullptr);
void gram_time_next_launch(hipEvent_t start, hipEvent_t stop);
bool gram_time_pending();
int gram_psplit_set_lds_limit();
void launch_cost(hipStream_t st, int loss, double f_scale, const double* obs_t, const double* obj, const double* x, double* cpart, double* res, int C, int F, int N, int Fpad, int nch,
                 double fill = 0.0);
size_t syrk_lds_bytes(int C, int FS, int cw = 12);
void launch_syrk(hipStream_t st, Sel s, const SyrkFuse& fz, const double* rec0, const double* rec1, double* fbuf, double* fpart, const int* tile_i, const int* tile_j, double* spart, int C, int F, int Fpad, int NT, int NP, int G, int sq, int sr, int FS, int ppw,
                 const double* dscale = nullptr,
                 int cw = 12);
int syrk_items_per_thread();
void launch_reduce_system(hipStream_t st, Sel s, const double* gp0, const double* gp1, const double* spart, const double* fpart, const int* tile_i, const int* tile_j, double* red, int C, int nfb, int G, int NT, int NP, int nfblocks, int rank_slot,
                          const double* bpart = nullptr, int nbp = 0, double* state_copy = nullptr, int cw = 12,
                          const double* timeout_word = nullptr, double seq_prev = 0.0);
void launch_backsub(hipStream_t st, Sel s, const double* rec0, const double* rec1, const double* fbuf, const CamStep& dc, double* x0, double* x1, double* bpart, int C, int F, int Fpad, int cw = 12);
void launch_backsub_dev(hipStream_t st, Sel s, const double* rec0, const double* rec1, const double* fbuf, const double* dc_dev, double* x0, double* x1, double* bpart, int C, int F, int Fpad, int cw = 12);
size_t solve_lds_bytes(int npad, int use_lds);
int solve_fits_lds(int npad, int lds_limit);
int solve_set_lds_limit(int npad, int use_lds);
void launch_solve_cam(hipStream_t st, const SolveArgs& a);
int solve_backsub_set_lds_limit(int npad, int cw = 12);
void launch_solve_backsub(hipStream_t st, const SolveArgs& a, Sel sl, const double* rec0, const double* rec1, const double* fbuf, double* x0, double* x1, double* bpart, int C, int F, int Fpad,
                          const double* early_state, int max_polls, int spec, double* timeout_dev, double* timeout_host,
                          int strict = 0);
void launch_sum_trial(hipStream_t st, Sel s, const double* cp0, const double* cp1, int cstride, int cinner, size_t couter, int ncp, const double* bpart, int nbp, double* out, DecideArgs da);
void launch_decide(hipStream_t st, const double* trial8, DecideArgs da);
void launch_lm_init(hipStream_t st, const double* red_scal, double* lms, double lam0, int sel, double cfl, double cfl_switch, double* clear8 = nullptr);
void launch_pack_result(hipStream_t st, const double* x, const double* gc, const double* fbuf, const unsigned char* fixed, double* out, int C, int F, int cw);
void launch_jacobian(hipStream_t st, int loss, double f_scale, const double* obs_raw, const double* obj, const double* x, double* jac, double* res, int C, int F, int N, int Fpad, int robust);
int syrk_set_lds_limit(size_t bytes);
void launch_sp_seen(hipStream_t st, const double* obs_raw, unsigned char* seen, int C, int F, int N);
void launch_sp_factor(hipStream_t st, Sel s, const double* rec0, const double* rec1, double* fbuf, double* fpart, const int* frame_off, const int* ent_cam, const int* ent_frame, int nent,
                      double* Y, const double* dscale, int C, int F, int Fpad, int cw);
void launch_sp_pairs(hipStream_t st, Sel s, const double* Y, const double* fbuf, const int* items, const int* chunks, int nchunks, double* part, const double* gp0, const double* gp1,
                     const int* pair_map, const int* pair_chunks, double* red, int C, int nfb, int cw);
int sp_npad(int n);
void launch_sp_solve(hipStream_t st, const SolveArgs& a, int* ctl, double* damp, double* A, double* y, void (*bracket)(void*, int, int), void* ctx);
void launch_frame_err(hipStream_t st, const double* obs_t, const double* obj, const double* x, double* err, double* mean_cf, double* full_cf, int C, int F, int N, int Fpad,
                      void* prefilter_state = nullptr);
struct SelState {
  unsigned long long prefix;
  unsigned long long rank;
  unsigned long long count;
  unsigned long long value;
  unsigned int hist[256];
};
constexpr int kSelMaxRanks = 8;
MCBA_HD double sel_value(const SelState& s) { return __builtin_bit_cast(double, s.value); }
MCBA_HD double sel_median(const SelState& lo, const SelState& hi) {
  const double m = 0.5 * (sel_value(lo) + sel_value(hi));
  return lo.count ? m : __builtin_nan("");
}
void launch_select(hipStream_t st, const double* v, const unsigned char* fmask, size_t per_group, int groups, int Fpad, SelState* sel,
                   int skey,
                   const unsigned long long* ranks = nullptr, int nranks = 0);
int launch_select_hist(hipStream_t st, const double* v, const unsigned char* fmask, size_t per_group, int Fpad, SelState* sel, unsigned long long prefix, int pass, unsigned int* hist256);
size_t prefilter_state_bytes();
void launch_prefilter_select(hipStream_t st, const double* err, const double* mean_cf, const double* full_cf, unsigned char* fmask, unsigned char* status, double* worst, void* state,
                             unsigned char* packed, int C, int F, int N, int Fpad, double threshold, bool state_cleared = false);
void launch_prefilter_status(hipStream_t st, unsigned char* status, const double* worst, void* state, unsigned char* packed, int F, double threshold, int from_state);
void launch_gather_params(hipStream_t st, const double* x_src, const int* frames, double* x_dst, int C, int Fdst);
void launch_clip(hipStream_t st, double* x, const double* lo, const double* hi, size_t n);
bool launch_store_small(hipStream_t st, double* dst, const double* src_host, size_t n);
double measure_fp64_issue_rate(int ncu);
void launch_gather_frames(hipStream_t st, const double* src_raw, const int* frames, double* dst_raw, int C, int Fsrc, int Fdst, int N,
                          const int* only_cam = nullptr);
void launch_seen_bits(hipStream_t st, const double* obs_raw, size_t count, unsigned long long* words);
void launch_undistort(hipStream_t st, const double* uv, double* out, size_t n, const double* K4, const double* dist5, int iters);
void launch_reproj_diag(hipStream_t st, const double* obs_t, const double* obj, const double* x, const double* dist5, const double* bn, double* und, double* repro, double* trans, double* err, int C, int F, int N,
                        int Fpad, int iters, int lm_iters);
void launch_view_complete(hipStream_t st, const double* obs_t, unsigned char* out, int C, int F, int N, int Fpad);
void launch_pnp(hipStream_t st, int mode, const double* obs_t, const double* obj, const double* intr9, const int* views, int nviews, const double* bn3, int C, int F, int N, int Fpad, int und_iters, int lm_iters,
                double* out, double* poses_t, unsigned char* valid, unsigned char* nit);
void launch_zhang(hipStream_t st, const double* H, const unsigned char* ok, const int* views, int nviews, const double* sizes, int C, double* intr9, unsigned char* closed);
void launch_pose_pairs(hipStream_t st, const double* poses, size_t sc, size_t sf, size_t sk, const int* edges, int n_edges, int F, int Fpad, double* rel);
void launch_pose_chain(hipStream_t st, const SelState* sel, const int* edges, int n_edges, int root, int C, double* ext, double* transforms, double* counts);
void launch_pose_consensus(hipStream_t st, const double* poses, size_t sc, size_t sf, size_t sk, const double* ext, int C, int F, int Fpad, double* world, double* out);
struct TriCams {
  double P[8][12];
  double K[8][4];
  double dist[8][5];
};
void launch_calib_views(hipStream_t st, const double* uvs, const double* obj, const double* intr9, const double* poses, int V, int N, double* out);
int launch_triangulate(hipStream_t st, int C, const double* uvs, const TriCams& cams, double* out, size_t npts, int iters);
int launch_triangulate_wave(hipStream_t st, int C, const double* uvs, const void* cams_dev, double* out, size_t npts, int iters);
struct KpCam;
struct TcCam;
int launch_project(hipStream_t st, int mode, const double* pts, size_t npts, const KpCam* cams, int C, double* out);
int launch_keypoint_errors(hipStream_t st, const double* pts, const double* uvs, size_t npts, size_t npad, const KpCam* cams, int C, double* err);
template <bool WEIGHTED>
struct KpDetections;
template <>
struct KpDetections<false> {
  const double2* det;
  size_t npts;
  __device__ KpDetections(const double2* uvs, const double*, size_t npts_, size_t p) : det(uvs + p), npts(npts_) {}
  __host__ __device__ void operator()(int c, double& ou, double& ov) const {
    const double2 o = det[(size_t)c * npts];
    ou = o.x; ov = o.y;
  }
};
template <>
struct KpDetections<true> {
  const double2* det;
  const double* sq;
  size_t npts;
  __device__ KpDetections(const double2* uvs, const double* sw, size_t npts_, size_t p) : det(uvs + p), sq(sw + p), npts(npts_) {}
  __host__ __device__ void operator()(int c, double& ou, double& ov, double& s) const {
    const double2 o = det[(size_t)c * npts];
    ou = o.x; ov = o.y;
    s = sq[(size_t)c * npts];
  }
};
template <int SRC_STRIDE>
__device__ __forceinline__ void stage_cam_doubles(KpCam* s_cam, const double* __restrict__ src, int C) {
  double* dst = reinterpret_cast<double*>(s_cam);
  for (int i = threadIdx.x; i < 21 * C; i += blockDim.x) dst[i] = SRC_STRIDE == 21 ? src[i] : src[SRC_STRIDE * (i / 21) + i % 21];
  __syncthreads();
}
__device__ __forceinline__ void stage_cams(KpCam* s_cam, const KpCam* __restrict__ cams, int C) { stage_cam_doubles<21>(s_cam, reinterpret_cast<const double*>(cams), C); }
__device__ __forceinline__ void stage_cams(KpCam* s_cam, const TcCam* __restrict__ cams, int C) { stage_cam_doubles<30>(s_cam, reinterpret_cast<const double*>(cams), C); }
int launch_tri_refine(hipStream_t st, int loss, const double* uvs, const double* start, size_t npts, const KpCam* cams, int C, double f_scale, int max_iterations, double* out, double* info,
                      const double* sw = nullptr);
enum ConsensusForm { CONSENSUS_AUTO = -1, CONSENSUS_LANE = 0, CONSENSUS_WAVE = 1, CONSENSUS_LANE_SEARCH = 2 };
int launch_consensus(hipStream_t st, int form, int loss, const double* uvs, size_t npts, const KpCam* cams, int C, double threshold, int min_views, int und_iters, double f_scale,
                     int max_iterations, double* out, unsigned long long* mask, double* hyp, double* info);
constexpr int kHypThreads = 256, kHypPPT = 4, kHypPoints = kHypThreads * kHypPPT;
constexpr int kHypChunk = 64;
inline size_t hyp_score_blocks(size_t n) { return (n + kHypPoints - 1) / kHypPoints; }
inline size_t hyp_point_blocks(size_t n) { return (n + kHypThreads - 1) / kHypThreads; }
void launch_hyp_finish(hipStream_t st, const double* part_c, const unsigned* part_n, size_t nblk, int C, int H, const int* status, double* cost, unsigned* count);
struct TvCams { double ka[4], da[5], kb[4], db[5]; };
void launch_tv_prepare(hipStream_t st, const double* uv_a, const double* uv_b, size_t M, const TvCams& cams, int und_iters, double* prep);
void launch_tv_hypotheses(hipStream_t st, const double* prep, size_t M, const int* samples, int H, const double* e_in, const TvCams& cams, double* E, double* F, int* status);
void launch_tv_score(hipStream_t st, const double* prep, size_t M, const double* F, int H, double threshold, double* part_c, unsigned* part_n);
void launch_tv_finish(hipStream_t st, const double* part_c, const unsigned* part_n, size_t nblk, int H, const double* E, const int* status, double* cost, unsigned* count, int* win_idx, double* best4,
                      double* cand);
void launch_tv_pose(hipStream_t st, const double* prep, size_t M, const double* F, const int* status, double threshold, const double* cand, unsigned* part_f, int* win_idx, double* best4, double* rt12,
                    unsigned char* inliers, double* points);
void launch_tv5_hypotheses(hipStream_t st, const double* prep, size_t M, const int* samples, int H, const TvCams& cams, double* E10, double* F10, int* status10, double* Ep, double* Fp, int* stp,
                           int* map, int* n_packed);
void launch_rs_prepare(hipStream_t st, const double* points, const double* uvs, size_t P, int C, const double* cams, int und_iters, double* prep, unsigned char* usable);
void launch_rs_hypotheses(hipStream_t st, const double* points, const double* prep, size_t P, int C, const int* samples, int H, const double* pose_in, const double* cams, double* pose, double* KP,
                          int* status);
void launch_rs3_hypotheses(hipStream_t st, const double* points, const double* prep, size_t P, int C, const int* samples, int H, const double* cams, double* pose, double* KP, int* status);
void launch_rs_score(hipStream_t st, const double* points, const double* prep, const unsigned char* usable, size_t P, int C, const double* KP, int H, double threshold, double* part_c,
                     unsigned* part_n);
void launch_rs_finish(hipStream_t st, const double* part_c, const unsigned* part_n, size_t nblk, int C, int H, const double* pose, const int* status, double* cost, unsigned* count, int* win_idx,
                      double* best4, double* rt12);
void launch_rs_mask(hipStream_t st, const double* points, const double* prep, const unsigned char* usable, size_t P, int C, const double* KP, const int* status, int H, double threshold,
                    const int* win_idx, unsigned char* inliers);
int launch_rs_normal(hipStream_t st, int loss, bool cost_only, const double* points, const double* uvs, const unsigned char* mask, size_t P, int n, const int* ids, const TcCam* tcs, double f_scale,
                     double* part, double* sys);
int launch_cov_wss(hipStream_t st, int loss, double f_scale, const double* res, size_t count, double* part, double* out);
void launch_cov_check(hipStream_t st, const double* rec, unsigned char* flag, int* counts, int C, int F, int Fpad);
void launch_cov_cam(hipStream_t st, const double* S0, int n, int cw, int gauge, double sigma2, double* R, double* M, double* isd, double* Sig, int ld, int* pivot);
int cov_frames_group(int n, int lds_limit, int force_g);
int launch_cov_frames(hipStream_t st, const double* rec, const double* fbuf, const unsigned char* flag, const double* Sig, int ld, double sigma2, double* out, int C, int F, int Fpad, int cw, int G);

int tricov_point_blocks(size_t npts);
int launch_tricov_point(hipStream_t st, int loss, const double* uvs, const double* pts, size_t npts, const TcCam* cams, int C, double f_scale, double sigma2_in, double* hinv, int* views, int* status,
                        double* part, double* info, const double* sw = nullptr);
void launch_tricov_scale(hipStream_t st, const double* hinv, const int* status, const double* info, size_t npts, double* det6);
int tricov_group(int n, int lds_limit, int force_g);
int launch_tricov_cal(hipStream_t st, int loss, const double* uvs, const double* pts, size_t npts, const TcCam* cams, int C, double f_scale, const double* hinv, const int* status, const double* Sig,
                      int ld, const double* info, double* det6, double* cal6, int G, const double* sw = nullptr);

struct SmLevel;
struct SmData;
void launch_smooth_prepare(hipStream_t st, size_t T, int K, const double* pts, const double* cov6, const double* w_in, double* p, double* winv, double* w, int* n_usable);
int launch_smooth_reduce(hipStream_t st, const SmLevel* lv, int levels, const SmData& td, int K, const int* list, int nact, int* bad, bool rhs = false);
int launch_smooth_backsub(hipStream_t st, const SmLevel* lv, int levels, const SmData& td, int K, const int* list, int nact, bool rhs = false);
int launch_smooth_solve(hipStream_t st, const SmLevel* lv, int levels, const SmData& td, int K, const int* list, int nact, int* bad, double* part, double* res);

int launch_smooth_selinv(hipStream_t st, const SmLevel* lv, int levels, const SmData& td, double* const* z, double* cov6, double* lag9, int K, const int* list, int nact);

struct TrData;
int launch_traj_count(hipStream_t st, const TrData& rd, int C, int K, int* n_usable, int* n_single, int* n_bad);
int launch_traj_linearise(hipStream_t st, int loss, const TrData& rd, const KpCam* cams, int C, int K, const int* run);
int launch_traj_trial(hipStream_t st, int loss, const TrData& rd, const KpCam* cams, int C, int K, const int* list, int nact, double* part, double* res);
int launch_traj_apply(hipStream_t st, const TrData& rd, int K, const double* alpha);

int kpba_group(int C, int lds_limit, int force_g);
int kpba_groups(size_t npts);
size_t kpba_partial_size(int C);
int launch_kpba_status(hipStream_t st, const double* uvs, const double* pts, size_t npts, const TcCam* cams, int C, int* status, const double* sw = nullptr, bool wide = false);
int launch_kpba_reduce(hipStream_t st, int loss, const double* uvs, const double* pts, const int* status, size_t npts, const TcCam* cams, const int* held, int C, double f_scale, double lam, int G,
                       double* part, double* sys, const double* sw = nullptr);
int launch_kpba_step(hipStream_t st, int loss, const double* uvs, const double* pts, double* trial, const int* status, size_t npts, const TcCam* cams2, const double* dtheta, int C, double f_scale,
                     double lam, double* part4, double* out4, const double* sw = nullptr, bool wide = false);
void launch_kpba_finish(hipStream_t st, const double* part, int nwg, int C, double* sys);
void launch_kpba_finish_sized(hipStream_t st, const double* part, int nwg, int NP, int nacc, double* sys);
int kpcam_group(int C, int lds_limit, int force_g);
size_t kpcam_partial_size(int C);
size_t kpcam_reduce_lds(int C, int G);
int launch_kpcam_reduce(hipStream_t st, int loss, const double* uvs, const double* pts, const int* status, size_t npts, const TcCam* cams, const int* held, int C, double f_scale, double lam, int G,
                        double* part, double* sys, const double* sw = nullptr);
int launch_kpcam_step(hipStream_t st, int loss, const double* uvs, const double* pts, double* trial, const int* status, size_t npts, const TcCam* cams2, const double* dtheta, int C, double f_scale,
                      double lam, double* part4, double* out4, const double* sw = nullptr);
constexpr int kKtMaxCams = 64, kKtBand = 16, kKtGroup = 16;
int kpba_tiled_groups(int C, size_t npts);
int kpba_tiled_pairs(int C);
size_t kpba_tiled_lds();
int launch_kpba_reduce_tiled(hipStream_t st, int loss, const double* uvs, const double* pts, const int* status, size_t npts, const TcCam* cams, const int* held, int C, double f_scale, double lam,
                             double* fac, double* part, double* sys, const double* sw = nullptr);
}
```

multicam-calibration_amd/csrc/mcba_kernels.hip:

```cpp
#include <hip/hip_runtime.h>
#include <hip/hip_ext.h>
#include <stdlib.h>
#include <type_traits>
#include "mcba_math.h"
#include <algorithm>
#include "mcba_kernels.h"
#include "mcba_lm.h"
#include "mcba_device.h"
#include "mcba_backsub.h"

#ifndef MCBA_GRAM_PIPE
#define MCBA_GRAM_PIPE 1
#endif

namespace mcba {

template <int CTRL>
__device__ __forceinline__ double dpp_perm(double v) {
  union { double d; int i[2]; } a, b;
  a.d = v;
  b.i[0] = __builtin_amdgcn_mov_dpp(a.i[0], CTRL, 0xF, 0xF, true);
  b.i[1] = __builtin_amdgcn_mov_dpp(a.i[1], CTRL, 0xF, 0xF, true);
  return b.d;
}
template <int LEVEL>
__device__ __forceinline__ double halve_pair(double x, double y, int lane) {
  if constexpr (LEVEL <= 1) {
    union { double d; unsigned u[2]; } a, b;
    a.d = x; b.d = y;
    if constexpr (LEVEL == 0) {
      auto r0 = __builtin_amdgcn_permlane32_swap(a.u[0], b.u[0], false, false);
      auto r1 = __builtin_amdgcn_permlane32_swap(a.u[1], b.u[1], false, false);
      a.u[0] = r0[0]; b.u[0] = r0[1]; a.u[1] = r1[0]; b.u[1] = r1[1];
    } else {
      auto r0 = __builtin_amdgcn_permlane16_swap(a.u[0], b.u[0], false, false);
      auto r1 = __builtin_amdgcn_permlane16_swap(a.u[1], b.u[1], false, false);
      a.u[0] = r0[0]; b.u[0] = r0[1]; a.u[1] = r1[0]; b.u[1] = r1[1];
    }
    return a.d + b.d;
  } else {
    constexpr int BIT = LEVEL == 2 ? 8 : LEVEL == 3 ? 4 : 2;
    constexpr int CTRL = LEVEL == 2 ? 0x140 : LEVEL == 3 ? 0x141 : 0x1B;
    const bool up = (lane & BIT) != 0;
    const double keep = up ? y : x, send = up ? x : y;
    return keep + dpp_perm<CTRL>(send);
  }
}
template <int LEVEL>
__device__ __forceinline__ double pair_sum(double v) {
  if constexpr (LEVEL == 4) return v + dpp_perm<0x1B>(v);
  else return v + dpp_perm<0xB1>(v);
}
template <int K, int LEVEL = 0>
__device__ __forceinline__ void wave_reduce_scatter(double* v, double (&out)[3], int lane) {
  if constexpr (K > 3) {
    constexpr int H = K / 2;
#pragma unroll
    for (int k = 0; k < H; ++k) v[k] = halve_pair<LEVEL>(v[k], v[k + H], lane);
    wave_reduce_scatter<H, LEVEL + 1>(v, out, lane);
  } else {
#pragma unroll
    for (int r = 0; r < 3; ++r) {
      double t = v[r];
      if constexpr (LEVEL <= 4) t = pair_sum<4>(t);
      t = pair_sum<5>(t);
      out[r] = t;
    }
    static_assert(LEVEL == 4 || LEVEL == 5, "K must be 48 or 96");
  }
}
__device__ __forceinline__ double uni(double v) {
  union { double d; int i[2]; } u;
  u.d = v;
  u.i[0] = __builtin_amdgcn_readfirstlane(u.i[0]);
  u.i[1] = __builtin_amdgcn_readfirstlane(u.i[1]);
  return u.d;
}
__device__ __forceinline__ bool is_num(double v) { return v == v; }
template <int LOSS, bool UNIT = false>
__device__ __forceinline__ void obs_weights(double r, bool valid, double fs2, double ifs2, double cfl, double& cost, double& w2, double& g) {
  double rh, gw, ww;
  loss_weights<LOSS, UNIT>(r, fs2, ifs2, rh, gw, ww);
  cost += valid ? rh : 0.0;
  w2 = valid ? lm_weight(gw, ww, cfl) : 0.0;
  g = valid ? gw * r : 0.0;
}

__device__ __forceinline__ void obs_weights_table(double r, bool valid, double rh, double gw, double ww, double cfl, double& cost, double& w2, double& g) {
  cost += valid ? rh : 0.0;
  w2 = valid ? lm_weight(gw, ww, cfl) : 0.0;
  g = valid ? gw * r : 0.0;
}

__global__ __launch_bounds__(256) void k_transpose_obs(const double2* __restrict__ raw, double2* __restrict__ obs_t, int C, int F, int N, int Fpad) {
  __shared__ double2 tile[64][17];
  const int fb = blockIdx.x, c = blockIdx.y, p0 = 16 * blockIdx.z;
  const int tx = threadIdx.x & 15, ty = threadIdx.x >> 4;
  double2 nanv;
  nanv.x = nanv.y = __builtin_nan("");
#pragma unroll
  for (int fr = 0; fr < 4; ++fr) {
    const int f = fb * 64 + fr * 16 + ty, p = p0 + tx;
    tile[fr * 16 + ty][tx] = (f < F && p < N) ? raw[((size_t)c * F + f) * N + p] : nanv;
  }
  __syncthreads();
  const int fl = threadIdx.x & 63, pp = threadIdx.x >> 6;
#pragma unroll
  for (int k = 0; k < 4; ++k) {
    const int p = p0 + pp + 4 * k;
    if (p < N) obs_t[((size_t)c * N + p) * Fpad + fb * 64 + fl] = tile[fl][pp + 4 * k];
  }
}

template <int LOSS, int ROLE, bool FAST = false, int MODE = 0, int NPW = 1>
__device__ __forceinline__ void gram_body(const CamConst& s_cam, const double2* __restrict__ obs_t, const double* __restrict__ obj, const double* __restrict__ x,
                                          double* __restrict__ rec, double* __restrict__ gpart, int c, int fb, int lane, int C, int N, int Fpad, int nfb, double fs2, double ifs2, double cfl,
                                          const double (&pz0)[6], const double2 (&pre)[4], double* s_cost, int nrun, int p_lo = 0, int p_hi = -1, double2* chunk = nullptr, int nchunk = 1,
                                          size_t chunk_stride = 0, const double2* __restrict__ ltab = nullptr) {
  static_assert(LOSS != LOSS_TABLE || (ROLE != 2 && MODE == 0), "the tabulated loss runs the split-role kernel (k_gram_table)");
  if (p_hi < 0) p_hi = N;
  static_assert(MODE == 0 || ((ROLE == 2 || (MODE == 3 && ROLE == 0)) && MCBA_GRAM_PIPE), "point chunks exist for the pipelined loop only (both roles; role A alone in MODE 3: intrinsics held fixed)");
  static_assert(MODE == 3 ? (NPW == 2 || NPW == 4) : NPW == 1, "NPW wavefronts share a (camera, frame block) in MODE 3 only");
  const int f = fb * 64 + lane;
  Intr K;
  K.fx = uni(s_cam.fx); K.fy = uni(s_cam.fy); K.cx = uni(s_cam.cx); K.cy = uni(s_cam.cy); K.k1 = uni(s_cam.k1); K.k2 = uni(s_cam.k2);
  double Rc[9], tc[3];
#pragma unroll
  for (int i = 0; i < 9; ++i) Rc[i] = uni(s_cam.R[i]);
#pragma unroll
  for (int i = 0; i < 3; ++i) tc[i] = uni(s_cam.t[i]);

  const double* pose = x + 12 * C + 6 * (size_t)f;
  PairConst pc;
  double abc[3];
  {
    double Rf[9];
    rot_only(pz0, Rf, abc);
    make_pair_const(Rc, tc, Rf, pz0 + 3, pc);
  }

  constexpr bool DO_A = ROLE != 1, DO_B = ROLE != 0;
  GramA ga;
  GramB gb;
  if (DO_A) gram_zero(ga);
  if (DO_B) gram_zero(gb);
  double cost = 0.0;
  bool any = false;
  constexpr int PF = 2;
  const double2* op = obs_t + (size_t)c * N * Fpad + f;
  double2 ring[PF];
  double xring[PF][3];
#pragma unroll
  for (int j = 0; j < PF; ++j) {
    const int pj = min(j, N - 1);
    ring[j] = pre[j];
    xring[j][0] = obj[3 * pj]; xring[j][1] = obj[3 * pj + 1]; xring[j][2] = obj[3 * pj + 2];
  }
  auto point = [&](double2 o2, const double Xo[3], int pi) {
    bool vu = is_num(o2.x), vv = is_num(o2.y);
    if (vu || vv) {
      any = true;
      ObsCommon q;
      obs_common(K, pc, Xo, q);
      double wu2, wv2, gu, gv;
      if constexpr (LOSS == LOSS_TABLE) {
        const size_t plane = (size_t)C * N * Fpad, at = (size_t)c * N * Fpad + (size_t)pi * Fpad + f;
        const double2 t0 = ltab[at], t1 = ltab[plane + at], t2 = ltab[2 * plane + at];
        obs_weights_table(o2.x - q.up, vu, t0.x, t1.x, t2.x, cfl, cost, wu2, gu);
        obs_weights_table(o2.y - q.vp, vv, t0.y, t1.y, t2.y, cfl, cost, wv2, gv);
      } else {
      obs_weights<LOSS>(o2.x - q.up, vu, fs2, ifs2, cfl, cost, wu2, gu);
      obs_weights<LOSS>(o2.y - q.vp, vv, fs2, ifs2, cfl, cost, wv2, gv);
      }
      {
        double E[6];
        obs_row_cam<0>(q, E);
        if (DO_A) gram_add_row<0>(ga, E, wu2, gu);
        if (DO_B) { double l4 = q.fa * q.s; gram_add_row<0>(gb, E, wu2, gu, q.a * q.d, l4, l4 * q.s); }
      }
      {
        double E[6];
        obs_row_cam<1>(q, E);
        if (DO_A) gram_add_row<1>(ga, E, wv2, gv);
        if (DO_B) { double l4 = q.fb * q.s; gram_add_row<1>(gb, E, wv2, gv, q.b * q.d, l4, l4 * q.s); }
      }
    }
  };
  if constexpr ((ROLE == 2 || MODE == 3) && MCBA_GRAM_PIPE) {
    constexpr int RD = 4;
    double2 r4[RD];
    double x4[RD][3];
#pragma unroll
    for (int j = 0; j < RD; ++j) {
      int pj = min(p_lo + j, p_hi - 1);
      if constexpr (MODE == 3) pj = max(pj, 0);
      r4[j] = pre[j];
      x4[j][0] = obj[3 * pj]; x4[j][1] = obj[3 * pj + 1]; x4[j][2] = obj[3 * pj + 2];
    }
    ObsLead qc;
    obs_lead<true, FAST>(pc, x4[0], qc, is_num(r4[0].x) || is_num(r4[0].y));
    auto accumulate = [&](double2 o2, const double Xo[3], const ObsLead& ql) {
      ObsCommon q;
      obs_finish(K, ql, q);
      const bool vu = is_num(o2.x), vv = is_num(o2.y);
      any = any || vu || vv;
      double wu2, wv2, gu, gv;
      obs_weights<LOSS, FAST>(o2.x - q.up, vu, fs2, ifs2, cfl, cost, wu2, gu);
      obs_weights<LOSS, FAST>(o2.y - q.vp, vv, fs2, ifs2, cfl, cost, wv2, gv);
      {
        double E[6];
        obs_row_cam<0>(q, E);
        gram_add_row<0>(ga, E, wu2, gu);
        if constexpr (DO_B) {
        double l4 = q.fa * q.s;
        gram_add_row<0>(gb, E, wu2, gu, q.a * q.d, l4, l4 * q.s);
        }
      }
      {
        double E[6];
        obs_row_cam<1>(q, E);
        gram_add_row<1>(ga, E, wv2, gv);
        if constexpr (DO_B) {
        double l4 = q.fb * q.s;
        gram_add_row<1>(gb, E, wv2, gv, q.b * q.d, l4, l4 * q.s);
        }
      }
    };
    int p = p_lo;
    if constexpr (MODE != 2)
    for (; p + RD <= p_hi; p += RD) {
#pragma unroll
      for (int j = 0; j < RD; ++j) {
        const int jn = (j + 1) % RD;
        ObsLead qn;
        obs_lead<true, FAST>(pc, x4[jn], qn, is_num(r4[jn].x) || is_num(r4[jn].y));
        const double2 o2 = r4[j];
        const double Xo[3] = {x4[j][0], x4[j][1], x4[j][2]};
        const int pn = min(p + j + RD, p_hi - 1);
        r4[j] = op[(size_t)pn * Fpad];
        x4[j][0] = obj[3 * pn]; x4[j][1] = obj[3 * pn + 1]; x4[j][2] = obj[3 * pn + 2];
        accumulate(o2, Xo, qc);
        qc = qn;
      }
    }
    if constexpr (MODE != 2)
#pragma unroll
    for (int j = 0; j < RD; ++j) {
      if (p + j < p_hi) {
        const int jn = (j + 1) % RD;
        ObsLead qn;
        obs_lead<true, FAST>(pc, x4[jn], qn, is_num(r4[jn].x) || is_num(r4[jn].y));
        accumulate(r4[j], x4[j], qc);
        qc = qn;
      }
    }
  } else {
  int p = 0;
  for (; p + PF <= N; p += PF) {
#pragma unroll
    for (int j = 0; j < PF; ++j) {
      double2 o2 = ring[j];
      double Xo[3] = {xring[j][0], xring[j][1], xring[j][2]};
      const int pn = min(p + j + PF, N - 1);
      ring[j] = op[(size_t)pn * Fpad];
      xring[j][0] = obj[3 * pn]; xring[j][1] = obj[3 * pn + 1]; xring[j][2] = obj[3 * pn + 2];
      point(o2, Xo, p + j);
    }
  }
#pragma unroll
  for (int j = 0; j < PF; ++j)
    if (p + j < N) point(ring[j], xring[j], p + j);
  }

  if constexpr (MODE == 1) {
    double raw[kGramRaw];
#pragma unroll
    for (int i = 0; i < 21; ++i) raw[i] = ga.ee[i];
#pragma unroll
    for (int i = 0; i < 6; ++i) { raw[21 + i] = ga.he[i]; raw[81 + i] = gb.hi[i]; }
    raw[27] = cost;
#pragma unroll
    for (int i = 0; i < 17; ++i) raw[28 + i] = gb.ii[i];
#pragma unroll
    for (int i = 0; i < 36; ++i) raw[45 + i] = gb.ie[i];
    raw[87] = any ? 1.0 : 0.0;
#pragma unroll
    for (int k = 0; k < kGramRaw; k += 2) chunk[(k >> 1) * 64] = make_double2(raw[k], raw[k + 1]);
    return;
  }
  if constexpr (MODE == 2) {
    constexpr int HR = kGramRaw / 2, CB = 3;
    double acc[kGramRaw];
#pragma unroll
    for (int k = 0; k < kGramRaw; ++k) acc[k] = 0.0;
    for (int c0 = 0; c0 < nchunk; c0 += CB) {
      double2 v[CB][HR];
#pragma unroll
      for (int j = 0; j < CB; ++j) {
        const double2* src = chunk + (size_t)min(c0 + j, nchunk - 1) * chunk_stride;
#pragma unroll
        for (int k = 0; k < HR; ++k) v[j][k] = src[k * 64];
      }
#pragma unroll
      for (int j = 0; j < CB; ++j) {
        if (c0 + j < nchunk) {
#pragma unroll
          for (int k = 0; k < HR; ++k) { acc[2 * k] += v[j][k].x; acc[2 * k + 1] += v[j][k].y; }
        }
      }
    }
#pragma unroll
    for (int i = 0; i < 21; ++i) ga.ee[i] = acc[i];
#pragma unroll
    for (int i = 0; i < 6; ++i) { ga.he[i] = acc[21 + i]; gb.hi[i] = acc[81 + i]; }
    cost = acc[27];
#pragma unroll
    for (int i = 0; i < 17; ++i) gb.ii[i] = acc[28 + i];
#pragma unroll
    for (int i = 0; i < 36; ++i) gb.ie[i] = acc[45 + i];
    any = acc[87] != 0.0;
  }
  if constexpr (MODE == 3) {
    const int wv = __builtin_amdgcn_readfirstlane((int)(threadIdx.x >> 6)), part = wv % NPW, grp = wv / NPW;
    if constexpr (NPW == 4) {
      constexpr int NBL = 32, NBH = 27;
      double* xA = reinterpret_cast<double*>(chunk) + lane;
      double* xL = xA + 4 * kGramRawA * 64;
      double* xH = xL + 3 * NBL * 64;
      {
        double* d = xA + part * (kGramRawA * 64);
#pragma unroll
        for (int i = 0; i < 21; ++i) d[i * 64] = ga.ee[i];
#pragma unroll
        for (int i = 0; i < 6; ++i) d[(21 + i) * 64] = ga.he[i];
        d[27 * 64] = cost;
        d[28 * 64] = any ? 1.0 : 0.0;
      }
      if (DO_B && part != 1) {
        double* d = xL + (part == 0 ? 0 : part - 1) * (NBL * 64);
#pragma unroll
        for (int i = 0; i < 11; ++i) d[i * 64] = gb.ii[i];
#pragma unroll
        for (int i = 0; i < 18; ++i) d[(11 + i) * 64] = gb.ie[i];
#pragma unroll
        for (int i = 0; i < 3; ++i) d[(29 + i) * 64] = gb.hi[i];
      }
      if (DO_B && part != 2) {
        double* d = xH + (part == 3 ? 2 : part) * (NBH * 64);
#pragma unroll
        for (int i = 0; i < 6; ++i) d[i * 64] = gb.ii[11 + i];
#pragma unroll
        for (int i = 0; i < 18; ++i) d[(6 + i) * 64] = gb.ie[18 + i];
#pragma unroll
        for (int i = 0; i < 3; ++i) d[(24 + i) * 64] = gb.hi[3 + i];
      }
      double pz[6];
#pragma unroll
      for (int i = 0; i < 6; ++i) pz[i] = pose[i];
      __syncthreads();
      if (!DO_B && (part == 1 || part == 2)) return;
      ChainConst ch;
      {
        double Rf[9], Jrf[9], Jrc[9];
        rot_and_jr(pz, Rf, Jrf, abc);
#pragma unroll
        for (int i = 0; i < 9; ++i) Jrc[i] = uni(s_cam.Jr[i]);
        make_chain_const(Rc, Jrc, Rf, Jrf, pz + 3, ch);
        chain_to_cam_rows(pc.Rcf, ch);
      }
      double2* r2 = reinterpret_cast<double2*>(rec + ((size_t)c * nfb + fb) * (MCBA_REC * 64)) + lane;
      double red[48];
#pragma unroll
      for (int i = 0; i < 48; ++i) red[i] = 0.0;
      int kofs_lo = 0, kofs_hi = 0, nlo = 0, nown = 0;
      if (part == 0 || part == 3) {
        GramA gs;
#pragma unroll
        for (int i = 0; i < 21; ++i) gs.ee[i] = xA[i * 64];
#pragma unroll
        for (int i = 0; i < 6; ++i) gs.he[i] = xA[(21 + i) * 64];
        double cs = xA[27 * 64];
        bool an = xA[28 * 64] != 0.0;
#pragma unroll
        for (int j = 1; j < 4; ++j) {
          const double* sA = xA + j * (kGramRawA * 64);
#pragma unroll
          for (int i = 0; i < 21; ++i) gs.ee[i] += sA[i * 64];
#pragma unroll
          for (int i = 0; i < 6; ++i) gs.he[i] += sA[(21 + i) * 64];
          cs += sA[27 * 64];
          an = an || sA[28 * 64] != 0.0;
        }
        double U[78], gc[12], W[72], V[21], gf[6];
        gram_expand(gs, ch, U, gc, W, V, gf);
        if (part == 3) {
#pragma unroll
          for (int i = 36; i < 72; i += 2) r2[(i >> 1) * 64] = make_double2(W[i], W[i + 1]);
#pragma unroll
          for (int i = 0; i < 20; i += 2) r2[(36 + (i >> 1)) * 64] = make_double2(V[i], V[i + 1]);
          r2[46 * 64] = make_double2(V[20], gf[0]);
          r2[47 * 64] = make_double2(gf[1], gf[2]);
          r2[48 * 64] = make_double2(gf[3], gf[4]);
          r2[49 * 64] = make_double2(gf[5], 0.0);
        } else {
#pragma unroll
          for (int a = 6; a < 12; ++a) {
#pragma unroll
            for (int b = a; b < 12; ++b) red[tri12(a, b) - 57] = U[tri12(a, b)];
            red[78 + a - 63] = gc[a];
          }
          red[27] = cs;
          red[28] = an ? 1.0 : 0.0;
          kofs_lo = 57; kofs_hi = 63; nlo = 21; nown = 29;
        }
      } else if constexpr (DO_B) {
        GramB gs;
        gram_zero(gs);
        if (part == 1) {
#pragma unroll
          for (int i = 0; i < 11; ++i) gs.ii[i] = xL[i * 64] + gb.ii[i];
#pragma unroll
          for (int i = 0; i < 18; ++i) gs.ie[i] = xL[(11 + i) * 64] + gb.ie[i];
#pragma unroll
          for (int i = 0; i < 3; ++i) gs.hi[i] = xL[(29 + i) * 64] + gb.hi[i];
#pragma unroll
          for (int j = 1; j < 3; ++j) {
            const double* sB = xL + j * (NBL * 64);
#pragma unroll
            for (int i = 0; i < 11; ++i) gs.ii[i] += sB[i * 64];
#pragma unroll
            for (int i = 0; i < 18; ++i) gs.ie[i] += sB[(11 + i) * 64];
#pragma unroll
            for (int i = 0; i < 3; ++i) gs.hi[i] += sB[(29 + i) * 64];
          }
        } else {
#pragma unroll
          for (int i = 0; i < 6; ++i) gs.ii[11 + i] = ((xH[i * 64] + xH[(NBH + i) * 64]) + gb.ii[11 + i]) + xH[(2 * NBH + i) * 64];
#pragma unroll
          for (int i = 0; i < 18; ++i) gs.ie[18 + i] = ((xH[(6 + i) * 64] + xH[(NBH + 6 + i) * 64]) + gb.ie[18 + i]) + xH[(2 * NBH + 6 + i) * 64];
#pragma unroll
          for (int i = 0; i < 3; ++i) gs.hi[3 + i] = ((xH[(24 + i) * 64] + xH[(NBH + 24 + i) * 64]) + gb.hi[3 + i]) + xH[(2 * NBH + 24 + i) * 64];
        }
        double U[78], gc[12], W[72];
        gram_expand(gs, ch, U, gc, W);
        if (part == 1) {
#pragma unroll
          for (int i = 0; i < 18; i += 2) r2[(i >> 1) * 64] = make_double2(W[i], W[i + 1]);
#pragma unroll
          for (int j = 0; j < 33; ++j) red[j] = U[j];
#pragma unroll
          for (int a = 0; a < 3; ++a) red[33 + a] = gc[a];
          kofs_lo = 0; kofs_hi = 78 - 33; nlo = 33; nown = 36;
        } else {
#pragma unroll
          for (int i = 18; i < 36; i += 2) r2[(i >> 1) * 64] = make_double2(W[i], W[i + 1]);
#pragma unroll
          for (int j = 0; j < 24; ++j) red[j] = U[33 + j];
#pragma unroll
          for (int a = 0; a < 3; ++a) red[24 + a] = gc[3 + a];
          kofs_lo = 33; kofs_hi = 81 - 24; nlo = 24; nown = 27;
        }
      }
      if (part != 3) {
        double o3[3];
        wave_reduce_scatter<48>(red, o3, lane);
        if ((lane & 3) == 0) {
          double* gp = gpart + (size_t)c * MCBA_GP * nfb + fb;
#pragma unroll
          for (int r = 0; r < 3; ++r) {
            const int j = 3 * (lane >> 2) + r;
            if (j < nown) gp[(size_t)(j < nlo ? kofs_lo + j : kofs_hi + j) * nfb] = o3[r];
          }
        }
      }
    } else {
    double* xa = reinterpret_cast<double*>(chunk) + (size_t)grp * ((NPW - 1) * (DO_B ? kGramRaw : kGramRawA) * 64) + lane;
    double* xb = xa + (NPW - 1) * kGramRawA * 64;
    if (part != 0) {
      double* d = xa + (part - 1) * (kGramRawA * 64);
#pragma unroll
      for (int i = 0; i < 21; ++i) d[i * 64] = ga.ee[i];
#pragma unroll
      for (int i = 0; i < 6; ++i) d[(21 + i) * 64] = ga.he[i];
      d[27 * 64] = cost;
      d[28 * 64] = any ? 1.0 : 0.0;
    }
    if (DO_B && part != 1) {
      double* d = xb + (part == 0 ? 0 : part - 1) * (kGramRawB * 64);
#pragma unroll
      for (int i = 0; i < 17; ++i) d[i * 64] = gb.ii[i];
#pragma unroll
      for (int i = 0; i < 36; ++i) d[(17 + i) * 64] = gb.ie[i];
#pragma unroll
      for (int i = 0; i < 6; ++i) d[(53 + i) * 64] = gb.hi[i];
    }
    __syncthreads();
    if (part == 0) {
#pragma unroll
      for (int j = 1; j < NPW; ++j) {
        const double* sA = xa + (j - 1) * (kGramRawA * 64);
#pragma unroll
        for (int i = 0; i < 21; ++i) ga.ee[i] += sA[i * 64];
#pragma unroll
        for (int i = 0; i < 6; ++i) ga.he[i] += sA[(21 + i) * 64];
        cost += sA[27 * 64];
        any = any || sA[28 * 64] != 0.0;
      }
      {
#define GF_ROLE 0
#define GF_A true
#define GF_B false
#define GF_PRESUM false
#include "mcba_gram_finish.inc"
#undef GF_ROLE
#undef GF_A
#undef GF_B
#undef GF_PRESUM
      }
    } else if (DO_B && part == 1) {
      {
        const double* sB = xb;
#pragma unroll
        for (int i = 0; i < 17; ++i) gb.ii[i] = sB[i * 64] + gb.ii[i];
#pragma unroll
        for (int i = 0; i < 36; ++i) gb.ie[i] = sB[(17 + i) * 64] + gb.ie[i];
#pragma unroll
        for (int i = 0; i < 6; ++i) gb.hi[i] = sB[(53 + i) * 64] + gb.hi[i];
      }
#pragma unroll
      for (int j = 2; j < NPW; ++j) {
        const double* sB = xb + (j - 1) * (kGramRawB * 64);
#pragma unroll
        for (int i = 0; i < 17; ++i) gb.ii[i] += sB[i * 64];
#pragma unroll
        for (int i = 0; i < 36; ++i) gb.ie[i] += sB[(17 + i) * 64];
#pragma unroll
        for (int i = 0; i < 6; ++i) gb.hi[i] += sB[(53 + i) * 64];
      }
      {
#define GF_ROLE 1
#define GF_A false
#define GF_B true
#define GF_PRESUM false
#include "mcba_gram_finish.inc"
#undef GF_ROLE
#undef GF_A
#undef GF_B
#undef GF_PRESUM
      }
    }
    }
    return;
  }
#define GF_ROLE ROLE
#define GF_A DO_A
#define GF_B DO_B
#define GF_PRESUM true
#include "mcba_gram_finish.inc"
#undef GF_ROLE
#undef GF_A
#undef GF_B
#undef GF_PRESUM
}

struct GramStart {
  const double* x;
  double* rec;
  double* gpart;
  double pz[6];
  double2 pre[4];
  int fb, lane;
  bool run;
  double cfl;
};
__device__ __forceinline__ void gram_start(GramStart& g, CamConst& s_cam, const double2* __restrict__ obs_t, Sel sl, const double* __restrict__ x0, const double* __restrict__ x1, double* rec0, double* rec1,
                                           double* gp0, double* gp1, int C, int N, int Fpad, int fb0, int fb1, int p_lo = 0, int p_hi = -1, int npw = 1,
                                           int bxo = -1, int co = -1) {
  if (p_hi < 0) p_hi = N;
  const int c = co >= 0 ? co : (int)blockIdx.y;
  const int bx = bxo >= 0 ? bxo : (int)blockIdx.x;
  const int wave = threadIdx.x >> 6;
  g.lane = threadIdx.x & 63;
  g.fb = fb0 + bx * ((blockDim.x >> 6) / npw) + wave / npw;
  const bool have = g.fb < fb1;
  const int fbc = have ? g.fb : fb1 - 1;
  double st3 = 0.0, st14 = 0.0, st15 = 0.0, st25 = sl.cfl;
  if (sl.lms) { st3 = sl.lms[3]; st14 = sl.lms[MCBA_LM_SKIP]; st15 = sl.lms[MCBA_LM_DONE]; st25 = sl.lms[MCBA_LM_CFL]; }
  const size_t po = (size_t)12 * C + 6 * ((size_t)fbc * 64 + g.lane);
  double pa[6], pb[6], ca[12], cb[12];
#pragma unroll
  for (int i = 0; i < 6; ++i) { pa[i] = x0[po + i]; pb[i] = x1[po + i]; }
  if (threadIdx.x == 0) {
#pragma unroll
    for (int i = 0; i < 12; ++i) { ca[i] = x0[12 * c + i]; cb[i] = x1[12 * c + i]; }
  }
  const double2* op = obs_t + (size_t)c * N * Fpad + (size_t)fbc * 64 + g.lane;
#pragma unroll
  for (int j = 0; j < 4; ++j) g.pre[j] = op[(size_t)min(p_lo + j, p_hi - 1) * Fpad];
  const bool active = !sl.lms || (st15 == 0.0 && st14 == 0.0);
  const bool spec = sl.spec && st14 == 0.0;
  const int sidx = sl.lms ? ((static_cast<int>(st3) ^ sl.idx ^ (spec ? 1 : 0)) & 1) : sl.idx;
  g.x = sidx ? x1 : x0;
  g.rec = sidx ? rec1 : rec0;
  g.gpart = sidx ? gp1 : gp0;
#pragma unroll
  for (int i = 0; i < 6; ++i) g.pz[i] = sidx ? pb[i] : pa[i];
  if (active && threadIdx.x == 0) {
    double cm[12];
#pragma unroll
    for (int i = 0; i < 12; ++i) cm[i] = sidx ? cb[i] : ca[i];
    make_cam_const(cm, s_cam);
  }
  g.cfl = st25;
  g.run = active;
  if (active) __syncthreads();
  g.run = active && have;
}

template <int LOSS>
__global__ __launch_bounds__(256, 2) void k_gram_split(const double2* __restrict__ obs_t, const double* __restrict__ obj, Sel sl, const double* __restrict__ x0, const double* __restrict__ x1,
                                                       double* __restrict__ rec0, double* __restrict__ rec1, double* __restrict__ gp0, double* __restrict__ gp1, int C, int N, int Fpad, int nfb, int fb0, int fb1,
                                                       double fs2, double ifs2) {
  __shared__ CamConst s_cam;
  __shared__ double s_cost[8];
  GramStart g;
  gram_start(g, s_cam, obs_t, sl, x0, x1, rec0, rec1, gp0, gp1, C, N, Fpad, fb0, fb1);
  if (!g.run) return;
  const int c = blockIdx.y;
  const int nrun = min(4, fb1 - (fb0 + (int)blockIdx.x * 4));
  if (blockIdx.z == 0) gram_body<LOSS, 0>(s_cam, obs_t, obj, g.x, g.rec, g.gpart, c, g.fb, g.lane, C, N, Fpad, nfb, fs2, ifs2, g.cfl, g.pz, g.pre, s_cost, nrun);
  else gram_body<LOSS, 1>(s_cam, obs_t, obj, g.x, g.rec, g.gpart, c, g.fb, g.lane, C, N, Fpad, nfb, fs2, ifs2, g.cfl, g.pz, g.pre, s_cost, nrun);
}

__global__ __launch_bounds__(256, 2) void k_gram_table(const double2* __restrict__ obs_t, const double* __restrict__ obj, Sel sl, const double* __restrict__ x0, const double* __restrict__ x1,
                                                       double* __restrict__ rec0, double* __restrict__ rec1, double* __restrict__ gp0, double* __restrict__ gp1, int C, int N, int Fpad, int nfb, int fb0, int fb1,
                                                       const double2* __restrict__ ltab) {
  __shared__ CamConst s_cam;
  __shared__ double s_cost[8];
  GramStart g;
  gram_start(g, s_cam, obs_t, sl, x0, x1, rec0, rec1, gp0, gp1, C, N, Fpad, fb0, fb1);
  if (!g.run) return;
  const int c = blockIdx.y;
  const int nrun = min(4, fb1 - (fb0 + (int)blockIdx.x * 4));
  if (blockIdx.z == 0) gram_body<LOSS_TABLE, 0>(s_cam, obs_t, obj, g.x, g.rec, g.gpart, c, g.fb, g.lane, C, N, Fpad, nfb, 1.0, 1.0, g.cfl, g.pz, g.pre, s_cost, nrun, 0, -1, nullptr, 1, 0, ltab);
  else gram_body<LOSS_TABLE, 1>(s_cam, obs_t, obj, g.x, g.rec, g.gpart, c, g.fb, g.lane, C, N, Fpad, nfb, 1.0, 1.0, g.cfl, g.pz, g.pre, s_cost, nrun, 0, -1, nullptr, 1, 0, ltab);
}

template <int LOSS, bool FAST>
__global__ __launch_bounds__(256) void k_gram(const double2* __restrict__ obs_t, const double* __restrict__ obj, Sel sl, const double* __restrict__ x0, const double* __restrict__ x1,
                                                 double* __restrict__ rec0, double* __restrict__ rec1, double* __restrict__ gp0, double* __restrict__ gp1, int C, int N, int Fpad, int nfb, int fb0, int fb1,
                                                 double fs2, double ifs2) {
  __shared__ CamConst s_cam;
  __shared__ double s_cost[8];
  GramStart g;
  gram_start(g, s_cam, obs_t, sl, x0, x1, rec0, rec1, gp0, gp1, C, N, Fpad, fb0, fb1);
  if (!g.run) return;
  const int nrun = min(4, fb1 - (fb0 + (int)blockIdx.x * 4));
  gram_body<LOSS, 2, FAST>(s_cam, obs_t, obj, g.x, g.rec, g.gpart, blockIdx.y, g.fb, g.lane, C, N, Fpad, nfb, fs2, ifs2, g.cfl, g.pz, g.pre, s_cost, nrun);
}

template <int LOSS, bool FAST, int NPW, int ROLE = 2>
__global__ __launch_bounds__(256) void k_gram_psplit(const double2* __restrict__ obs_t, const double* __restrict__ obj, Sel sl, const double* __restrict__ x0, const double* __restrict__ x1,
                                                        double* __restrict__ rec0, double* __restrict__ rec1, double* __restrict__ gp0, double* __restrict__ gp1, int C, int N, int Fpad, int nfb, int fb0, int fb1,
                                                        double fs2, double ifs2) {
  __shared__ CamConst s_cam;
  __shared__ double s_cost[8];
  extern __shared__ __align__(16) double s_xch[];
  const int part = __builtin_amdgcn_readfirstlane((int)(threadIdx.x >> 6)) % NPW;
  const int p_lo = (int)(((long long)N * part) / NPW), p_hi = (int)(((long long)N * (part + 1)) / NPW);
  GramStart g;
  gram_start(g, s_cam, obs_t, sl, x0, x1, rec0, rec1, gp0, gp1, C, N, Fpad, fb0, fb1, p_lo, max(p_hi, p_lo + 1), NPW);
  if (!g.run) return;
  gram_body<LOSS, ROLE, FAST, 3, NPW>(s_cam, obs_t, obj, g.x, g.rec, g.gpart, blockIdx.y, g.fb, g.lane, C, N, Fpad, nfb, fs2, ifs2, g.cfl, g.pz, g.pre, s_cost, 0, p_lo, p_hi, reinterpret_cast<double2*>(s_xch));
}

template <int LOSS, bool FAST, int NPW>
__global__ __launch_bounds__(256) void k_gram_mixed(const double2* __restrict__ obs_t, const double* __restrict__ obj, Sel sl, const double* __restrict__ x0, const double* __restrict__ x1,
                                                       double* __restrict__ rec0, double* __restrict__ rec1, double* __restrict__ gp0, double* __restrict__ gp1, int C, int N, int Fpad, int nfb, int fba,
                                                       int nf, int nt, double fs2, double ifs2) {
  __shared__ CamConst s_cam;
  __shared__ double s_cost[8];
  extern __shared__ __align__(16) double s_xch[];
  const int id = blockIdx.x;
  GramStart g;
  if (id < nf * C) {
    const int c = id / nf, bx = id - c * nf;
    gram_start(g, s_cam, obs_t, sl, x0, x1, rec0, rec1, gp0, gp1, C, N, Fpad, 0, fba, 0, -1, 1, bx, c);
    if (!g.run) return;
    const int nrun = min(4, fba - bx * 4);
    gram_body<LOSS, 2, FAST>(s_cam, obs_t, obj, g.x, g.rec, g.gpart, c, g.fb, g.lane, C, N, Fpad, nfb, fs2, ifs2, g.cfl, g.pz, g.pre, s_cost, nrun);
  } else {
    const int id2 = id - nf * C, c = id2 / nt, bx = id2 - c * nt;
    const int part = __builtin_amdgcn_readfirstlane((int)(threadIdx.x >> 6)) % NPW;
    const int p_lo = (int)(((long long)N * part) / NPW), p_hi = (int)(((long long)N * (part + 1)) / NPW);
    gram_start(g, s_cam, obs_t, sl, x0, x1, rec0, rec1, gp0, gp1, C, N, Fpad, fba, nfb, p_lo, max(p_hi, p_lo + 1), NPW, bx, c);
    if (!g.run) return;
    gram_body<LOSS, 2, FAST, 3, NPW>(s_cam, obs_t, obj, g.x, g.rec, g.gpart, c, g.fb, g.lane, C, N, Fpad, nfb, fs2, ifs2, g.cfl, g.pz, g.pre, s_cost, 0, p_lo, p_hi, reinterpret_cast<double2*>(s_xch));
  }
}

template <int LOSS, bool FAST>
__global__ __launch_bounds__(64) void k_gram_chunk(const double2* __restrict__ obs_t, const double* __restrict__ obj, Sel sl, const double* __restrict__ x0, const double* __restrict__ x1,
                                                       double2* __restrict__ chunk, int C, int N, int Fpad, int nfb, int fb0, int fb1, double fs2, double ifs2, int ppc, int nchunk) {
  __shared__ CamConst s_cam;
  __shared__ double s_cost[8];
  const int p_lo = (int)blockIdx.z * ppc, p_hi = min(N, p_lo + ppc);
  GramStart g;
  gram_start(g, s_cam, obs_t, sl, x0, x1, nullptr, nullptr, nullptr, nullptr, C, N, Fpad, fb0, fb1, p_lo, p_hi);
  if (!g.run) return;
  const int ntb = fb1 - fb0;
  double2* dst = chunk + ((((size_t)blockIdx.y * ntb + (g.fb - fb0)) * nchunk + blockIdx.z) * (kGramRaw / 2)) * 64 + g.lane;
  gram_body<LOSS, 2, FAST, 1>(s_cam, obs_t, obj, g.x, nullptr, nullptr, blockIdx.y, g.fb, g.lane, C, N, Fpad, nfb, fs2, ifs2, g.cfl, g.pz, g.pre, s_cost, 0, p_lo, p_hi, dst);
}
template <int LOSS, bool FAST>
__global__ __launch_bounds__(256) void k_gram_combine(const double2* __restrict__ obs_t, const double* __restrict__ obj, Sel sl, const double* __restrict__ x0, const double* __restrict__ x1,
                                                         double* __restrict__ rec0, double* __restrict__ rec1, double* __restrict__ gp0, double* __restrict__ gp1, const double2* __restrict__ chunk,
                                                         int C, int N, int Fpad, int nfb, int fb0, int fb1, double fs2, double ifs2, int nchunk) {
  __shared__ CamConst s_cam;
  __shared__ double s_cost[8];
  GramStart g;
  gram_start(g, s_cam, obs_t, sl, x0, x1, rec0, rec1, gp0, gp1, C, N, Fpad, fb0, fb1);
  if (!g.run) return;
  const int nrun = min(4, fb1 - (fb0 + (int)blockIdx.x * 4));
  const int ntb = fb1 - fb0;
  const double2* src = chunk + (((size_t)blockIdx.y * ntb + (g.fb - fb0)) * nchunk * (kGramRaw / 2)) * 64 + g.lane;
  gram_body<LOSS, 2, FAST, 2>(s_cam, obs_t, obj, g.x, g.rec, g.gpart, blockIdx.y, g.fb, g.lane, C, N, Fpad, nfb, fs2, ifs2, g.cfl, g.pz, g.pre, s_cost, nrun, 0, N, const_cast<double2*>(src), nchunk,
                              (size_t)(kGramRaw / 2) * 64);
}

template <int LOSS, bool WRITE_RES>
__global__ __launch_bounds__(256) void k_cost(const double2* __restrict__ obs_t, const double* __restrict__ obj, const double* __restrict__ x,
                                              double* __restrict__ cpart, double* __restrict__ res, int C, int F, int N, int Fpad, int nfb, int nch, double fs2, double ifs2,
                                              double fill) {
  __shared__ CamConst s_cam;
  const int c = blockIdx.y;
  if (threadIdx.x == 0) make_cam_const(x + 12 * c, s_cam);
  __syncthreads();
  const int wave = threadIdx.x >> 6, lane = threadIdx.x & 63;
  const int fb = blockIdx.x * 4 + wave;
  if (fb >= nfb) return;
  const int f = fb * 64 + lane;
  const int ch = blockIdx.z;
  const int p0 = (int)(((long long)N * ch) / nch), p1 = (int)(((long long)N * (ch + 1)) / nch);
  Intr K;
  K.fx = uni(s_cam.fx); K.fy = uni(s_cam.fy); K.cx = uni(s_cam.cx); K.cy = uni(s_cam.cy); K.k1 = uni(s_cam.k1); K.k2 = uni(s_cam.k2);
  double Rc[9], tc[3];
#pragma unroll
  for (int i = 0; i < 9; ++i) Rc[i] = uni(s_cam.R[i]);
#pragma unroll
  for (int i = 0; i < 3; ++i) tc[i] = uni(s_cam.t[i]);
  const double* pose = x + 12 * C + 6 * (size_t)f;
  double pz[6];
#pragma unroll
  for (int i = 0; i < 6; ++i) pz[i] = pose[i];
  PairConst pc;
  {
    double Rf[9];
    rot_only(pz, Rf);
    make_pair_const(Rc, tc, Rf, pz + 3, pc);
  }
  double cost = 0.0, nres = 0.0;
  const double2* op = obs_t + (size_t)c * N * Fpad + f;
  constexpr int PF = 4;
  double2 ring[PF];
#pragma unroll
  for (int j = 0; j < PF; ++j) ring[j] = op[(size_t)min(p0 + j, p1 - 1) * Fpad];
  auto point = [&](double2 o2, int p) {
    bool vu = is_num(o2.x), vv = is_num(o2.y);
    double ru = 0.0, rv = 0.0;
    if (vu || vv) {
      double Xo[3] = {obj[3 * p], obj[3 * p + 1], obj[3 * p + 2]};
      double up, vp;
      project_only(K, pc, Xo, up, vp);
      double rh, gw, w2;
      ru = o2.x - up; rv = o2.y - vp;
      loss_weights<LOSS>(ru, fs2, ifs2, rh, gw, w2);
      cost += vu ? rh : 0.0;
      loss_weights<LOSS>(rv, fs2, ifs2, rh, gw, w2);
      cost += vv ? rh : 0.0;
      nres += (vu ? 1.0 : 0.0) + (vv ? 1.0 : 0.0);
    }
    if (WRITE_RES && f < F) {
      *reinterpret_cast<double2*>(res + (((size_t)c * F + f) * N + p) * 2) = make_double2(vu ? ru : fill, vv ? rv : fill);
    }
  };
  int p = p0;
  for (; p + PF <= p1; p += PF) {
#pragma unroll
    for (int j = 0; j < PF; ++j) {
      double2 o2 = ring[j];
      ring[j] = op[(size_t)min(p + j + PF, p1 - 1) * Fpad];
      point(o2, p + j);
    }
  }
#pragma unroll
  for (int j = 0; j < PF; ++j)
    if (p + j < p1) point(ring[j], p + j);
  double cs = wave_sum(cost), ns = wave_sum(nres);
  size_t o = 2 * (((size_t)c * nfb + fb) * nch + ch);
  if (lane == 0) { cpart[o] = cs; cpart[o + 1] = ns; }
}

typedef double mfma_d4 __attribute__((ext_vector_type(4)));
constexpr int kSyrkSuper = 32;

template <int PPW, int IPT, bool DECIDE, bool XS, int CW = 12>
__global__ __launch_bounds__(256, PPW <= 4 ? 2 : 1) void k_syrk(Sel sl, SyrkFuse fz, const double* __restrict__ rec0, const double* __restrict__ rec1, double* __restrict__ fbuf, double* __restrict__ fpart,
                                              const int* __restrict__ tile_i, const int* __restrict__ tile_j, double* __restrict__ spart, int C, int F, int Fpad, int NT, int NP, int sq, int sr, int FS,
                                              const double* __restrict__ dscale, int xg, int yg) {
  int bx = blockIdx.x, by = blockIdx.y, gx = gridDim.x;
  if (xg > 0) {
    const int id = blockIdx.x, xcd = id & 7, slot = id >> 3, nfull = xg >> 3;
    gx = xg;
    if (slot < nfull * yg) {
      by = slot % yg;
      bx = (slot / yg) * 8 + xcd;
    } else {
      const int e = (slot - nfull * yg) * 8 + xcd;
      bx = 8 * nfull + e / yg;
      by = e % yg;
      if (bx >= xg) return;
    }
  }
  extern __shared__ __align__(16) double lds[];
  __shared__ double s_st[MCBA_LMS];
  __shared__ double s_sum[8];
  __shared__ double s_tw;
  const int t = threadIdx.x, lane = t & 63;
  const int wave = __builtin_amdgcn_readfirstlane(t >> 6);
  const bool have_state = sl.lms != nullptr;
  if (have_state && t < MCBA_LMS) s_st[t] = sl.lms[t];
  if (DECIDE && t == MCBA_LMS) s_tw = fz.timeout_word ? *fz.timeout_word : -1.0;
  if (DECIDE) {
    const double *pa, *pb;
    int stride = 1, count, inner = 1 << 30;
    size_t outer = 0;
    int dense = 1 << 30;
    if (wave == 0) { pa = fz.cp0; pb = fz.cp1; count = fz.ncp; inner = fz.cinner; outer = fz.couter; stride = fz.cstride; dense = fz.cdense; }
    else { pa = pb = fz.bpart + (wave - 1); stride = 3; count = fz.nbp; }
    const bool two = pa != pb;
    double sa = 0.0, sb = 0.0;
    for (int base = 0; base < count; base += 512) {
      double va[8], vb[8];
#pragma unroll
      for (int k = 0; k < 8; ++k) {
        const int idx = base + lane + 64 * k;
        const int hi = idx / inner, lo = idx - hi * inner;
        const size_t at = (size_t)hi * outer + (size_t)(lo < dense ? lo * stride : dense * stride + (lo - dense));
        va[k] = idx < count ? pa[at] : 0.0;
        vb[k] = (two && idx < count) ? pb[at] : 0.0;
      }
#pragma unroll
      for (int k = 0; k < 8; ++k) { sa += va[k]; sb += vb[k]; }
    }
    sa = wave_sum63(sa);
    sb = wave_sum63(sb);
    if (lane == 63) { s_sum[wave] = sa; s_sum[4 + wave] = sb; }
  }
  __syncthreads();
  if (have_state && s_st[MCBA_LM_DONE] != 0.0) {
    if (DECIDE && bx == 0 && by == 0 && t < MCBA_LMS) fz.lms_post[t] = s_st[t];
    return;
  }
  if (DECIDE) {
    if (t == 0) {
      const bool stale = s_tw == fz.seq_prev && fz.seq_prev > 0.0;
      if (s_st[MCBA_LM_SKIP] != 0.0 || stale) lm_mark_rebuild(s_st);
      else {
        const bool trial1 = ((static_cast<int>(s_st[3]) ^ 1) & 1) != 0;
        const double tr[8] = {trial1 ? s_sum[4] : s_sum[0], s_sum[1], s_sum[2], s_sum[3], 0.0, 0.0, 0.0, 0.0};
        s_sum[0] = tr[0];
        DecideArgs da = fz.da;
        da.decide = 2;
        da.lms = s_st;
        lm_decide(tr, da);
      }
    }
    __syncthreads();
    if (bx == 0 && by == 0) {
      if (t < MCBA_LMS) fz.lms_post[t] = s_st[t];
      if (t < 4) fz.trial_out[t] = s_sum[t];
    }
  }
  int sidx;
  double lambda;
  if (have_state) {
    const bool spec = sl.spec && s_st[MCBA_LM_SKIP] == 0.0;
    sidx = (static_cast<int>(s_st[3]) ^ sl.idx ^ (spec ? 1 : 0)) & 1;
    lambda = spec ? lm_spec_lambda(s_st[1], sl.lam, sl.dec) : s_st[1];
  } else {
    sidx = sl.idx;
    lambda = sl.lam;
  }
  const double* __restrict__ rec = sidx ? rec1 : rec0;
  const int n = CW * C, nfb = Fpad >> 6;
  const int RS = 6 * FS + 2;
  double* s_y = lds;
  double* s_L = lds + (size_t)NT * 16 * RS;

  int qi[PPW], rowa[PPW], rowb[PPW];
  mfma_d4 acc[PPW];
#pragma unroll
  for (int k = 0; k < PPW; ++k) {
    int q = by * (4 * PPW) + wave + 4 * k;
    qi[k] = q < NP ? q : -1;
    int ti = 0, tj = 0;
    if (q < NP) {
      int rem = q;
      while (rem >= NT - ti) { rem -= NT - ti; ++ti; }
      tj = ti + rem;
    }
    rowa[k] = (16 * ti + (lane & 15)) * RS + (lane >> 4);
    rowb[k] = (16 * tj + (lane & 15)) * RS + (lane >> 4);
    acc[k] = mfma_d4{0.0, 0.0, 0.0, 0.0};
  }
  for (int i = t; i < (NT * 16 - (n + 1)) * RS; i += 256) s_y[(size_t)(n + 1) * RS + i] = 0.0;

  const int f0 = (bx * sq + min(bx, sr)) * FS, f1 = min(F, f0 + (sq + (bx < sr ? 1 : 0)) * FS);
  double wreg[IPT][6];

  const int tb = t % FS, tr0 = t / FS, rstep = 256 / FS;
  auto prefetch = [&](int fb) {
#pragma unroll
    for (int it = 0; it < IPT; ++it) {
      int row = tr0 + rstep * it, b = tb, f = fb + b;
      if (row < n) {
        int c = row / CW, lr = row - CW * c + (12 - CW);
        const double2* w2 = reinterpret_cast<const double2*>(rec + ((size_t)c * nfb + (f >> 6)) * (MCBA_REC * 64)) + (size_t)(3 * lr) * 64 + (f & 63);
#pragma unroll
        for (int k = 0; k < 3; ++k) { double2 v = w2[k * 64]; wreg[it][2 * k] = v.x; wreg[it][2 * k + 1] = v.y; }
      }
    }
  };
  double* s_V = s_L + kSyrkSuper * 34;
  double gmax = 0.0, nfail = 0.0;
  auto vsum = [&](int s0, int ns) {
    const int fl = t & 31, part = t >> 5;
    const int f = s0 + min(fl, ns - 1);
    const double2* r2 = reinterpret_cast<const double2*>(rec + (size_t)(f >> 6) * (MCBA_REC * 64)) + (size_t)(36 + part) * 64 + (f & 63);
    const size_t cstride = (size_t)nfb * (MCBA_REC * 64 / 2);
    const bool two = part + 8 < 14;
    double2 a0 = make_double2(0.0, 0.0), a1 = make_double2(0.0, 0.0);
    constexpr int CB = 8;
    for (int c0 = 0; c0 < C; c0 += CB) {
      double2 u0[CB], u1[CB];
#pragma unroll
      for (int j = 0; j < CB; ++j) {
        const size_t o = (size_t)min(c0 + j, C - 1) * cstride;
        u0[j] = r2[o];
        u1[j] = r2[o + (two ? 8 * 64 : 0)];
      }
#pragma unroll
      for (int j = 0; j < CB; ++j) {
        if (c0 + j < C) { a0.x += u0[j].x; a0.y += u0[j].y; a1.x += u1[j].x; a1.y += u1[j].y; }
      }
    }
    if (fl < ns) {
      double* v = s_V + fl * 28;
      v[2 * part] = a0.x; v[2 * part + 1] = a0.y;
      if (two) { v[2 * (part + 8)] = a1.x; v[2 * (part + 8) + 1] = a1.y; }
    }
  };
  auto factor = [&](int s0, int ns) {
    const bool on = lane < ns;
    double* row = s_L + lane * 34;
    if (lane >= kSyrkSuper) return;
    if (on) {
      double V[28];
#pragma unroll
      for (int k = 0; k < 28; ++k) V[k] = s_V[lane * 28 + k];
      double* gf = V + 21;
      double D[6], dsv[6];
#pragma unroll
      for (int k = 0; k < 6; ++k) {
        double d = V[tri6(k, k)];
        const double ds = XS ? dscale[(size_t)12 * C + 6 * (size_t)(s0 + lane) + k] : 0.0;
        D[k] = ds > 0.0 ? ds : (d > 0.0 ? d : 1.0);
        dsv[k] = ds;
        V[tri6(k, k)] = d + lambda * D[k];
      }
      double gfm[6];
      unsigned fm = 0;
#pragma unroll
      for (int k = 0; k < 6; ++k) { gfm[k] = gf[k]; if (XS && dsv[k] < 0.0) fm |= 1u << k; }
      if (XS && fm) {
#pragma unroll
        for (int k = 0; k < 6; ++k) {
          if ((fm >> k) & 1u) {
#pragma unroll
            for (int j = 0; j < 6; ++j) V[j <= k ? tri6(j, k) : tri6(k, j)] = j == k ? 1.0 : 0.0;
            gfm[k] = 0.0;
          }
        }
      }
      double Lp[21], id[6], z[6];
      const bool ok = chol6i(V, Lp);
#pragma unroll
      for (int k = 0; k < 6; ++k) id[k] = Lp[k * (k + 1) / 2 + k];
      fwd6(Lp, id, gfm, z);
#pragma unroll
      for (int k = 0; k < 21; ++k) row[k] = Lp[k];
#pragma unroll
      for (int k = 0; k < 6; ++k) { row[21 + k] = id[k]; row[27 + k] = z[k]; gmax = fmax(gmax, fabs(gfm[k])); }
      if (XS) row[33] = (double)fm;
      nfail += ok ? 0.0 : 1.0;
      if (by == 0) {
        double o[40];
#pragma unroll
        for (int k = 0; k < 21; ++k) o[k] = Lp[k];
#pragma unroll
        for (int k = 0; k < 6; ++k) { o[21 + k] = z[k]; o[27 + k] = gf[k]; o[33 + k] = D[k]; }
        o[39] = XS ? (double)fm : 0.0;
        double* fbp = fbuf + (size_t)(s0 + lane) * MCBA_FB;
#pragma unroll
        for (int k = 0; k < 40; k += 2) *reinterpret_cast<double2*>(fbp + k) = make_double2(o[k], o[k + 1]);
      }
    } else {
#pragma unroll
      for (int k = 0; k < 34; ++k) row[k] = 0.0;
    }
  };

#define SLAP(i) do { } while (0)
  prefetch(f0);
  for (int s0 = f0; s0 < f1; s0 += kSyrkSuper) {
    const int s1 = min(f1, s0 + kSyrkSuper);
    vsum(s0, s1 - s0);
    __syncthreads();
    SLAP(4);
    if (wave == 0) factor(s0, s1 - s0);
    __syncthreads();
    SLAP(0);
    for (int fb = s0; fb < s1; fb += FS) {
      {
        double Lr[27];
        const double* Lp = s_L + (fb - s0 + tb) * 34;
#pragma unroll
        for (int k = 0; k < 27; ++k) Lr[k] = Lp[k];
        const bool live = fb + tb < F;
        const unsigned fm = XS ? (unsigned)Lp[33] : 0u;
#pragma unroll
        for (int it = 0; it < IPT; ++it) {
          const int row = tr0 + rstep * it;
          if (row <= n) {
            double* dst = s_y + (size_t)row * RS + tb * 6;
            if (row < n) {
              double yr[6];
              if (XS && fm) {
#pragma unroll
                for (int k = 0; k < 6; ++k) wreg[it][k] = ((fm >> k) & 1u) ? 0.0 : wreg[it][k];
              }
              fwd6(Lr, Lr + 21, wreg[it], yr);
#pragma unroll
              for (int k = 0; k < 6; ++k) dst[k] = live ? yr[k] : 0.0;
            } else {
#pragma unroll
              for (int k = 0; k < 6; ++k) dst[k] = Lp[27 + k];
            }
          }
        }
      }
      __syncthreads();
      SLAP(1);
      if (fb + FS < f1) prefetch(fb + FS);
      const int nks = (6 * FS) / 4;
      double a0[PPW], b0[PPW], a1[PPW], b1[PPW];
#pragma unroll
      for (int k = 0; k < PPW; ++k) { a0[k] = s_y[rowa[k]]; b0[k] = s_y[rowb[k]]; }
      for (int ks = 0; ks + 1 < nks; ks += 2) {
#pragma unroll
        for (int k = 0; k < PPW; ++k) { a1[k] = s_y[rowa[k] + 4 * ks + 4]; b1[k] = s_y[rowb[k] + 4 * ks + 4]; }
#pragma unroll
        for (int k = 0; k < PPW; ++k) acc[k] = __builtin_amdgcn_mfma_f64_16x16x4f64(a0[k], b0[k], acc[k], 0, 0, 0);
        if (ks + 2 < nks) {
#pragma unroll
          for (int k = 0; k < PPW; ++k) { a0[k] = s_y[rowa[k] + 4 * ks + 8]; b0[k] = s_y[rowb[k] + 4 * ks + 8]; }
        }
#pragma unroll
        for (int k = 0; k < PPW; ++k) acc[k] = __builtin_amdgcn_mfma_f64_16x16x4f64(a1[k], b1[k], acc[k], 0, 0, 0);
      }
      if (nks & 1) {
#pragma unroll
        for (int k = 0; k < PPW; ++k) acc[k] = __builtin_amdgcn_mfma_f64_16x16x4f64(a0[k], b0[k], acc[k], 0, 0, 0);
      }
      SLAP(2);
      __syncthreads();
      SLAP(3);
    }
  }
  if (wave == 0 && by == 0) {
    const double wm = wave_max(gmax), wn = wave_sum63(nfail);
    if (lane == 63) { fpart[2 * bx] = wm; fpart[2 * bx + 1] = wn; }
  }
#pragma unroll
  for (int k = 0; k < PPW; ++k) {
    if (qi[k] >= 0) {
      const size_t G = gx;
      double* o = spart + ((size_t)(4 * qi[k]) * G + bx) * 64 + lane;
      o[0] = acc[k][0]; o[G * 64] = acc[k][1]; o[2 * G * 64] = acc[k][2]; o[3 * G * 64] = acc[k][3];
    }
  }
}

__device__ __forceinline__ double run_sum(const double* __restrict__ p, int count, int lane) {
  double s = 0.0;
  for (int base = 0; base < count; base += 256) {
    double v[4];
#pragma unroll
    for (int k = 0; k < 4; ++k) { int i = base + lane + 64 * k; v[k] = i < count ? p[i] : 0.0; }
    s += (v[0] + v[1]) + (v[2] + v[3]);
  }
  return wave_sum63(s);
}

template <int RR>
__global__ __launch_bounds__(1024) void k_reduce_system(Sel sl, const double* __restrict__ gp0, const double* __restrict__ gp1, const double* __restrict__ spart, const double* __restrict__ fpart,
                                                        const int* __restrict__ tile_i, const int* __restrict__ tile_j, double* __restrict__ red, int C, int nfb, int G, int NT, int NP,
                                                        int nfblocks, int rank_slot, const double* __restrict__ bpart, int nbp, double* __restrict__ state_copy, int cw,
                                                        const double* __restrict__ timeout_word, double seq_prev) {
  const int n = cw * C, coff = 12 - cw;
  const int wave = threadIdx.x >> 6, lane = threadIdx.x & 63;
  __shared__ double s_part[RR][16][64];
  __shared__ double s_u[RR][16];
  const size_t camstride = (size_t)MCBA_GP * nfb;
  constexpr int BPQ = 16 / RR;
  if ((int)blockIdx.x < BPQ * NP) {
    const int q = blockIdx.x / BPQ, reg = RR == 1 ? (blockIdx.x >> 2) & 3 : blockIdx.x & 3, rr0 = RR == 1 ? blockIdx.x & 3 : 0;
    const int ti = tile_i[q], tj = tile_j[q];
    const int rg = lane >> 4, el = lane & 15;
    constexpr int NK = RR == 1 ? 8 : 2;
    double pv[RR][NK];
#pragma unroll
    for (int r = 0; r < RR; ++r) {
      const double* p = spart + (size_t)(4 * q + reg) * G * 64 + 16 * (rr0 + r) + el;
#pragma unroll
      for (int k = 0; k < NK; ++k) { const int g = wave + 16 * (rg + 4 * k); pv[r][k] = g < G ? p[(size_t)g * 64] : 0.0; }
    }
    if (!sel_active(sl, false)) return;
    const double* __restrict__ gpart = sel_index(sl) ? gp1 : gp0;
    const double* up[RR];
#pragma unroll
    for (int r = 0; r < RR; ++r) {
      up[r] = nullptr;
      const int row = 16 * ti + (rr0 + r) + 4 * reg, col = 16 * tj + wave;
      if (row < n && col < n && row / cw == col / cw) {
        int cam = row / cw, li = row - cw * cam + coff, lj = col - cw * cam + coff;
        int a = li <= lj ? li : lj, b2 = li <= lj ? lj : li;
        up[r] = gpart + cam * camstride + (size_t)tri12(a, b2) * nfb;
      } else if (col == n && row < n) {
        int cam = row / cw, li = row - cw * cam + coff;
        up[r] = gpart + cam * camstride + (size_t)(78 + li) * nfb;
      }
    }
    double us[RR];
#pragma unroll
    for (int r = 0; r < RR; ++r) us[r] = 0.0;
    for (int base = 0; base < nfb; base += 256) {
      double w[RR][4];
#pragma unroll
      for (int r = 0; r < RR; ++r) {
#pragma unroll
        for (int k = 0; k < 4; ++k) { const int i = base + lane + 64 * k; w[r][k] = (up[r] && i < nfb) ? up[r][i] : 0.0; }
      }
#pragma unroll
      for (int r = 0; r < RR; ++r) us[r] += (w[r][0] + w[r][1]) + (w[r][2] + w[r][3]);
    }
#pragma unroll
    for (int r = 0; r < RR; ++r) {
      const double u = wave_sum63(us[r]);
      if (lane == 63) s_u[r][wave] = u;
      double sum = 0.0;
#pragma unroll
      for (int k = 0; k < NK; ++k) sum += pv[r][k];
      s_part[r][wave][lane] = sum;
    }
    __syncthreads();
    if (wave < RR) {
      const int r = wave;
      double t = 0.0;
#pragma unroll
      for (int k = 0; k < 16; ++k) t += s_part[r][k][lane];
      const double v = (__shfl(t, el, 64) + __shfl(t, el + 16, 64)) + (__shfl(t, el + 32, 64) + __shfl(t, el + 48, 64));
      if (lane < 16) {
        const int row = 16 * ti + (rr0 + r) + 4 * reg, col = 16 * tj + el;
        if (row < n && col < n) {
          double out = s_u[r][el] - v;
          red[(size_t)row * n + col] = out;
          if (ti != tj) red[(size_t)col * n + row] = out;
        } else if (col == n && row < n) {
          red[(size_t)n * n + row] = v - s_u[r][el];
        }
      }
    }
    return;
  }
  if (!sel_active(sl, false)) return;
  const double* __restrict__ gpart = sel_index(sl) ? gp1 : gp0;
  const int task = ((int)blockIdx.x - BPQ * NP) * 16 + wave;
  double* tail = red + (size_t)n * n + n;
  if (task < n) {
    int cam = task / cw, l = task - cw * cam + coff;
    double v = run_sum(gpart + cam * camstride + (size_t)tri12(l, l) * nfb, nfb, lane);
    if (lane == 63) tail[task] = v;
  } else if (task < 2 * n) {
    int jj = task - n, cam = jj / cw, l = jj - cw * cam + coff;
    double v = run_sum(gpart + cam * camstride + (size_t)(78 + l) * nfb, nfb, lane);
    if (lane == 63) tail[n + jj] = v;
  } else if (task < 2 * n + 16) {
    int jj = task - 2 * n;
    double v = 0.0;
    if (jj == 0 || jj == 1) {
      double a = 0.0;
      const int total = C * nfb;
      for (int base = 0; base < total; base += 512) {
        double w[8];
#pragma unroll
        for (int k = 0; k < 8; ++k) {
          const int i = base + lane + 64 * k;
          const int cam = i / nfb, fbk = i - cam * nfb;
          w[k] = i < total ? gpart[cam * camstride + (size_t)(90 + jj) * nfb + fbk] : 0.0;
        }
        a += ((w[0] + w[1]) + (w[2] + w[3])) + ((w[4] + w[5]) + (w[6] + w[7]));
      }
      v = wave_sum63(a);
    } else if (jj == 2) {
      double a = 0.0;
      for (int k = lane; k < nfblocks; k += 64) a += fpart[2 * k + 1];
      v = wave_sum63(a);
    } else if (jj == 4 + rank_slot) {
      double a = 0.0;
      for (int k = lane; k < nfblocks; k += 64) a = fmax(a, fpart[2 * k]);
      v = wave_max(a);
    }
    if (lane == 63) tail[2 * n + jj] = v;
  } else if (bpart && task < 2 * n + 24) {
    const int jj = task - (2 * n + 16);
    double a = 0.0;
    if (jj == 5 && lane == 0 && timeout_word && seq_prev > 0.0 && *timeout_word == seq_prev) a = 1.0;
    if (jj == 0 || jj == 4) {
      const int total = C * nfb, kk = jj == 0 ? 90 : 91;
      for (int base = 0; base < total; base += 512) {
        double w[8];
#pragma unroll
        for (int k = 0; k < 8; ++k) {
          const int i = base + lane + 64 * k;
          const int cam = i / nfb, fbk = i - cam * nfb;
          w[k] = i < total ? gpart[cam * camstride + (size_t)kk * nfb + fbk] : 0.0;
        }
        a += ((w[0] + w[1]) + (w[2] + w[3])) + ((w[4] + w[5]) + (w[6] + w[7]));
      }
    } else if (jj >= 1 && jj <= 3) {
      for (int base = 0; base < nbp; base += 512) {
        double w[8];
#pragma unroll
        for (int k = 0; k < 8; ++k) { const int i = base + lane + 64 * k; w[k] = i < nbp ? bpart[3 * i + (jj - 1)] : 0.0; }
        a += ((w[0] + w[1]) + (w[2] + w[3])) + ((w[4] + w[5]) + (w[6] + w[7]));
      }
    }
    const double v = wave_sum63(a);
    if (lane == 63) tail[2 * n + 16 + jj] = v;
  } else if (bpart && state_copy && task == 2 * n + 24) {
    if (lane < MCBA_LMS) state_copy[lane] = sl.lms[lane];
  }
}

template <class DcSrc, int CW>
__global__ __launch_bounds__(64 * kBacksubWaves) void k_backsub(Sel sl, const double* __restrict__ rec0, const double* __restrict__ rec1, const double* __restrict__ fbuf, const DcSrc dcs,
                                                                double* __restrict__ x0, double* __restrict__ x1, double* __restrict__ bpart, int C, int F, int Fpad) {
  __shared__ double s_t[kBacksubWaves][6][64];
  backsub_body<DcSrc, CW>(sl, rec0, rec1, fbuf, dcs, x0, x1, bpart, C, F, Fpad, (int)blockIdx.x, (int)(blockDim.x >> 6), s_t, nullptr);
}

__global__ __launch_bounds__(512) void k_sum_trial(Sel sl, const double* __restrict__ cp0, const double* __restrict__ cp1, int cstride, int cinner, size_t couter, int ncp, const double* __restrict__ bpart, int nbp, double* __restrict__ out, DecideArgs da) {
  double st3 = 0.0, st14 = 0.0, st15 = 0.0;
  if (sl.lms) { st3 = sl.lms[3]; st14 = sl.lms[MCBA_LM_SKIP]; st15 = sl.lms[MCBA_LM_DONE]; }
  LmPre pre = {};
  if (da.decide && threadIdx.x == 0) lm_prefetch(da.lms, pre);
  __shared__ double s_out[8];
  const int w = threadIdx.x >> 6, l = threadIdx.x & 63;
  const double *pa = nullptr, *pb = nullptr;
  int stride = 1, count = 0, inner = 1 << 30;
  size_t outer = 0;
  if (w == 0) { pa = cp0; pb = cp1; stride = cstride; count = ncp; inner = cinner; outer = couter; }
  else if (w >= 1 && w <= 3 && bpart) { pa = pb = bpart + (w - 1); stride = 3; count = nbp; }
  else if (w == 4) {
    const size_t off = cstride == 2 ? 1 : (size_t)cinner;
    pa = cp0 + off; pb = cp1 + off; stride = cstride; count = ncp; inner = cinner; outer = couter;
  }
  const bool two = pa != pb;
  double sa = 0.0, sb = 0.0;
  for (int base = 0; base < count; base += 512) {
    double va[8], vb[8];
#pragma unroll
    for (int k = 0; k < 8; ++k) {
      int idx = base + l + 64 * k;
      int hi = idx / inner, lo = idx - hi * inner;
      const size_t at = (size_t)hi * outer + (size_t)lo * stride;
      va[k] = idx < count ? pa[at] : 0.0;
      vb[k] = (two && idx < count) ? pb[at] : 0.0;
    }
#pragma unroll
    for (int k = 0; k < 8; ++k) { sa += va[k]; sb += vb[k]; }
  }
  const bool active = !sl.lms || (st15 == 0.0 && st14 == 0.0);
  if (!active) {
    if (da.decide && threadIdx.x == 0 && st15 == 0.0) lm_mark_rebuild(da.lms);
    return;
  }
  const int sidx = sl.lms ? ((static_cast<int>(st3) ^ sl.idx) & 1) : sl.idx;
  double s = (two && sidx) ? sb : sa;
  s = wave_sum63(s);
  if (l == 63) { out[w] = s; s_out[w] = s; }
  if (da.decide) {
    __syncthreads();
    if (threadIdx.x == 0) lm_decide(s_out, da, pre);
  }
}

__global__ void k_decide(const double* __restrict__ trial8, DecideArgs da) {
  if (threadIdx.x != 0 || blockIdx.x != 0 || da.lms[MCBA_LM_DONE] != 0.0) return;
  if (da.lms[MCBA_LM_SKIP] != 0.0) lm_mark_rebuild(da.lms);
  else lm_decide(trial8, da);
}

template <int LOSS>
__global__ __launch_bounds__(64) void k_jacobian(const double2* __restrict__ obs_raw, const double* __restrict__ obj, const double* __restrict__ x, double* __restrict__ jac,
                                                 double* __restrict__ res, int C, int F, int N, int Fpad, int robust, double fs2, double ifs2) {
  __shared__ double s_rows[64 * 37];
  const int f = blockIdx.x, c = blockIdx.y, lane = threadIdx.x;
  CamConst cc;
  make_cam_const(x + 12 * c, cc);
  const double* pose = x + 12 * C + 6 * (size_t)f;
  double pz[6];
#pragma unroll
  for (int i = 0; i < 6; ++i) pz[i] = pose[i];
  double Rf[9], Jrf[9];
  rot_and_jr(pz, Rf, Jrf);
  PairConst pc;
  make_pair_const(cc.R, cc.t, Rf, pz + 3, pc);
  ChainConst ch;
  make_chain_const(cc.R, cc.Jr, Rf, Jrf, pz + 3, ch);
  Intr K{cc.fx, cc.fy, cc.cx, cc.cy, cc.k1, cc.k2};
  for (int p0 = 0; p0 < N; p0 += 64) {
    const int p = p0 + lane;
    const int np = min(64, N - p0);
    if (p < N) {
      double2 o2 = obs_raw[((size_t)c * F + f) * N + p];
      bool vu = is_num(o2.x), vv = is_num(o2.y);
      double Xo[3] = {obj[3 * p], obj[3 * p + 1], obj[3 * p + 2]};
      ObsRows o;
      obs_rows(K, pc, Xo, o);
      double ru = o2.x - o.up, rv = o2.y - o.vp;
      double su = -1.0, sv = -1.0;
      if (robust) {
        double rh, gw, w2;
        loss_weights<LOSS>(ru, fs2, ifs2, rh, gw, w2);
        su = -sqrt(w2);
        loss_weights<LOSS>(rv, fs2, ifs2, rh, gw, w2);
        sv = -sqrt(w2);
      }
      su = vu ? su : 0.0;
      sv = vv ? sv : 0.0;
      double Jcu[12], Jcv[12], Jfu[6], Jfv[6];
      expand_rows(o, ch, Jcu, Jcv, Jfu, Jfv);
      double* sr = s_rows + lane * 37;
#pragma unroll
      for (int k = 0; k < 12; ++k) { sr[k] = su * Jcu[k]; sr[18 + k] = sv * Jcv[k]; }
#pragma unroll
      for (int k = 0; k < 6; ++k) { sr[12 + k] = su * Jfu[k]; sr[30 + k] = sv * Jfv[k]; }
      if (res) *reinterpret_cast<double2*>(res + (((size_t)c * F + f) * N + p) * 2) = make_double2(vu ? ru : 0.0, vv ? rv : 0.0);
    }
    __syncthreads();
    double2* out = reinterpret_cast<double2*>(jac + (((size_t)c * F + f) * N + p0) * 36);
    for (int j = lane; j < np * 18; j += 64) {
      int pp = j / 18, kk = (j % 18) * 2;
      typedef double nt_d2 __attribute__((ext_vector_type(2)));
      nt_d2 v = {s_rows[pp * 37 + kk], s_rows[pp * 37 + kk + 1]};
      __builtin_nontemporal_store(v, reinterpret_cast<nt_d2*>(out) + j);
    }
    __syncthreads();
  }
}

void launch_transpose_obs(hipStream_t st, const double* raw, double* obs_t, int C, int F, int N, int Fpad) {
  k_transpose_obs<<<dim3(Fpad / 64, C, (N + 15) / 16), dim3(256), 0, st>>>(reinterpret_cast<const double2*>(raw), reinterpret_cast<double2*>(obs_t), C, F, N, Fpad);
}

static thread_local hipEvent_t t_ext_start = nullptr, t_ext_stop = nullptr;
void gram_time_next_launch(hipEvent_t start, hipEvent_t stop) { t_ext_start = start; t_ext_stop = stop; }
bool gram_time_pending() { return t_ext_start != nullptr; }

using GramNpwList = IntList<4, 2>;

void launch_gram(hipStream_t st, int loss, double f_scale, const double* obs_t, const double* obj, Sel s, const double* x0, const double* x1, double* rec0, double* rec1, double* gp0, double* gp1, int C, int N, int Fpad,
                 const GramPlan& p, int planar, double* chunk, const double* ltab) {
  const int nfb = Fpad / 64;
  const dim3 block(256);
  const double2* o2 = reinterpret_cast<const double2*>(obs_t);
  if (loss == LOSS_TABLE) {
    k_gram_table<<<dim3(GramPlan::quads(nfb), C, p.with_b ? 2 : 1), block, 0, st>>>(o2, obj, s, x0, x1, rec0, rec1, gp0, gp1, C, N, Fpad, nfb, 0, nfb, reinterpret_cast<const double2*>(ltab));
    return;
  }
  const double fs2 = f_scale * f_scale, ifs2 = 1.0 / fs2;
  const bool fast = planar && f_scale == 1.0;
  const int head = p.fused_blocks();
  auto go = [&](auto kernel, dim3 grid, size_t lds, int fb0, int fb1) { return launch(kernel, grid, block, lds, st, o2, obj, s, x0, x1, rec0, rec1, gp0, gp1, C, N, Fpad, nfb, fb0, fb1, fs2, ifs2); };
  auto fused = [&](int fb1) {
    const dim3 grid(GramPlan::quads(fb1), C, 1);
    hipEvent_t ea = t_ext_start, eb = t_ext_stop;
    const bool timed = ea && eb;
    if (timed) t_ext_start = t_ext_stop = nullptr;
    return with_loss(loss, [&](auto L) { return with_bool(fast, [&](auto FAST) {
      const auto kernel = k_gram<decltype(L)::value, decltype(FAST)::value>;
      if (!timed) return go(kernel, grid, 0, 0, fb1);
      hipExtLaunchKernelGGL(kernel, grid, block, 0, st, ea, eb, 0, o2, obj, s, x0, x1, rec0, rec1, gp0, gp1, C, N, Fpad, nfb, 0, fb1, fs2, ifs2);
      return 0;
    }); });
  };
  auto roles = [&](int fb0, int nroles) {
    return with_loss(loss, [&](auto L) { return go(k_gram_split<decltype(L)::value>, dim3(GramPlan::quads(nfb - fb0), C, nroles), 0, fb0, nfb); });
  };
  auto point_split = [&](auto&& launch) {
    return with_loss(loss, [&](auto L) { return with_bool(fast, [&](auto FAST) { return with_int(GramNpwList{}, p.npw, [&](auto NPW) { return launch(L, FAST, NPW); }); }); });
  };
  switch (p.whole) {
    case GRAM_PSPLIT:
      (void)point_split([&](auto L, auto FAST, auto NPW) { return with_bool(p.with_b, [&](auto B) {
        return go(k_gram_psplit<decltype(L)::value, decltype(FAST)::value, decltype(NPW)::value, decltype(B)::value ? 2 : 0>, dim3(p.psplit_groups(nfb), C, 1), p.psplit_lds_bytes(), 0, nfb);
      }); });
      return;
    case GRAM_ROLES: (void)roles(0, 2); return;
    case GRAM_ROLE_A: (void)roles(0, 1); return;
    case GRAM_FUSED: break;
  }
  switch (p.tail) {
    case GRAM_TAIL_NONE: (void)fused(nfb); return;
    case GRAM_TAIL_ROLES: (void)fused(head); (void)roles(head, 2); return;
    case GRAM_TAIL_CHUNKS: {
      (void)fused(head);
      double2* ck = reinterpret_cast<double2*>(chunk);
      (void)with_loss(loss, [&](auto L) { return with_bool(fast, [&](auto FAST) {
        launch(k_gram_chunk<decltype(L)::value, decltype(FAST)::value>, dim3(p.tail_blocks(), C, p.nrun), dim3(64), 0, st, o2, obj, s, x0, x1, ck, C, N, Fpad, nfb, head, nfb, fs2, ifs2, p.ppc, p.nrun);
        return launch(k_gram_combine<decltype(L)::value, decltype(FAST)::value>, dim3(GramPlan::quads(p.tail_blocks()), C, 1), block, 0, st, o2, obj, s, x0, x1, rec0, rec1, gp0, gp1, ck, C, N, Fpad, nfb, head, nfb, fs2, ifs2, p.nrun);
      }); });
      return;
    }
    case GRAM_TAIL_PSPLIT: {
      const int nf = GramPlan::quads(head), nt = p.psplit_groups(p.tail_blocks());
      (void)point_split([&](auto L, auto FAST, auto NPW) {
        return launch(k_gram_mixed<decltype(L)::value, decltype(FAST)::value, decltype(NPW)::value>, dim3((nf + nt) * C), block, p.psplit_lds_bytes(), st, o2, obj, s, x0, x1, rec0, rec1, gp0, gp1, C, N, Fpad, nfb, head, nf, nt, fs2, ifs2);
      });
      return;
    }
  }
}

void launch_cost(hipStream_t st, int loss, double f_scale, const double* obs_t, const double* obj, const double* x, double* cpart, double* res, int C, int F, int N, int Fpad, int nch, double fill) {
  int nfb = Fpad / 64;
  dim3 grid((nfb + 3) / 4, C, nch), block(256);
  double fs2 = f_scale * f_scale, ifs2 = 1.0 / fs2;
  if (loss == LOSS_TABLE) loss = LOSS_LINEAR;
  (void)with_loss(loss, [&](auto L) { return with_bool(res != nullptr, [&](auto WRITE_RES) {
    return launch(k_cost<decltype(L)::value, decltype(WRITE_RES)::value>, grid, block, 0, st, reinterpret_cast<const double2*>(obs_t), obj, x, cpart, res, C, F, N, Fpad, nfb, nch, fs2, ifs2, fill);
  }); });
}

size_t syrk_lds_bytes(int C, int FS, int cw) {
  int NT = (cw * C + 1 + 15) / 16;
  return ((size_t)NT * 16 * (6 * FS + 2) + (size_t)kSyrkSuper * (34 + 28)) * sizeof(double);
}

constexpr int kSyrkIpt = 5, kSyrkIptSmall = 3;
struct SyrkShape { int ppw, ipt, cw; };
constexpr SyrkShape kSyrkShapes[] = {{4, kSyrkIpt, 12}, {4, kSyrkIptSmall, 12}, {16, kSyrkIpt, 12}, {4, kSyrkIpt, 6}, {4, kSyrkIptSmall, 6}};
using SyrkShapeList = IntList<0, 1, 2, 3, 4>;
template <int SHAPE, bool DECIDE, bool XS>
constexpr auto syrk_kernel = k_syrk<kSyrkShapes[SHAPE].ppw, kSyrkShapes[SHAPE].ipt, DECIDE, XS, kSyrkShapes[SHAPE].cw>;

void launch_syrk(hipStream_t st, Sel s, const SyrkFuse& fz, const double* rec0, const double* rec1, double* fbuf, double* fpart, const int* tile_i, const int* tile_j, double* spart, int C, int F, int Fpad, int NT, int NP, int G, int sq, int sr, int FS, int ppw,
                 const double* dscale, int cw) {
  const size_t lds = syrk_lds_bytes(C, FS, cw);
  const bool small = (cw * C + 1) * FS <= 256 * kSyrkIptSmall;
  const int shape = cw == 6 ? (small ? 4 : 3) : ppw <= 4 ? (small ? 1 : 0) : 2;
  const int gy = (NP + 4 * kSyrkShapes[shape].ppw - 1) / (4 * kSyrkShapes[shape].ppw);
  const bool remap = gy > 1;
  const dim3 grid(remap ? 8 * ((G / 8) * gy + ((G % 8) * gy + 7) / 8) : G, remap ? 1 : gy);
  const int xg = remap ? G : 0, yg = remap ? gy : 0;
  (void)with_int(SyrkShapeList{}, shape, [&](auto SHAPE) { return with_bool(fz.decide != 0, [&](auto DECIDE) { return with_bool(dscale != nullptr, [&](auto XS) {
    return launch(syrk_kernel<decltype(SHAPE)::value, decltype(DECIDE)::value, decltype(XS)::value>, grid, dim3(256), lds, st, s, fz, rec0, rec1, fbuf, fpart, tile_i, tile_j, spart, C, F, Fpad, NT, NP, sq, sr, FS, dscale, xg, yg);
  }); }); });
}

int syrk_items_per_thread() { return kSyrkIpt; }

void launch_reduce_system(hipStream_t st, Sel s, const double* gp0, const double* gp1, const double* spart, const double* fpart, const int* tile_i, const int* tile_j, double* red, int C, int nfb, int G, int NT, int NP, int nfblocks, int rank_slot,
                          const double* bpart, int nbp, double* state_copy, int cw, const double* timeout_word, double seq_prev) {
  int n = cw * C;
  int tail_blocks = (2 * n + 16 + (bpart ? 9 : 0) + 15) / 16;
  if (NP >= 64 && G <= 128) k_reduce_system<4><<<dim3(4 * NP + tail_blocks), dim3(1024), 0, st>>>(s, gp0, gp1, spart, fpart, tile_i, tile_j, red, C, nfb, G, NT, NP, nfblocks, rank_slot, bpart, nbp, state_copy, cw, timeout_word, seq_prev);
  else k_reduce_system<1><<<dim3(16 * NP + tail_blocks), dim3(1024), 0, st>>>(s, gp0, gp1, spart, fpart, tile_i, tile_j, red, C, nfb, G, NT, NP, nfblocks, rank_slot, bpart, nbp, state_copy, cw, timeout_word, seq_prev);
}

template <class DcSrc>
static void backsub_go(hipStream_t st, Sel s, const double* rec0, const double* rec1, const double* fbuf, const DcSrc& dc, double* x0, double* x1, double* bpart, int C, int F, int Fpad, int cw) {
  (void)with_int<6, 12>(cw == 6 ? 6 : 12, [&](auto CW) {
    return launch(k_backsub<DcSrc, decltype(CW)::value>, dim3(Fpad / 64), dim3(64 * std::min(C, kBacksubWaves)), 0, st, s, rec0, rec1, fbuf, dc, x0, x1, bpart, C, F, Fpad);
  });
}
void launch_backsub(hipStream_t st, Sel s, const double* rec0, const double* rec1, const double* fbuf, const CamStep& dc, double* x0, double* x1, double* bpart, int C, int F, int Fpad, int cw) {
  backsub_go(st, s, rec0, rec1, fbuf, dc, x0, x1, bpart, C, F, Fpad, cw);
}
void launch_backsub_dev(hipStream_t st, Sel s, const double* rec0, const double* rec1, const double* fbuf, const double* dc_dev, double* x0, double* x1, double* bpart, int C, int F, int Fpad, int cw) {
  backsub_go(st, s, rec0, rec1, fbuf, DevStep{dc_dev}, x0, x1, bpart, C, F, Fpad, cw);
}

void launch_sum_trial(hipStream_t st, Sel s, const double* cp0, const double* cp1, int cstride, int cinner, size_t couter, int ncp, const double* bpart, int nbp, double* out, DecideArgs da) {
  k_sum_trial<<<dim3(1), dim3(512), 0, st>>>(s, cp0, cp1, cstride, cinner, couter, ncp, bpart, nbp, out, da);
}

__global__ void k_lm_init(const double* __restrict__ red_scal, double* __restrict__ lms, double lam0, double sel, double cfl, double cfl_switch, double* __restrict__ clear8) {
  const int i = threadIdx.x;
  if (clear8 && i >= 56) clear8[i - 56] = 0.0;
  if (i >= MCBA_LMS) return;
  double v = 0.0;
  if (i == 0) v = red_scal[0];
  else if (i == 1) v = lam0;
  else if (i == 2) v = 2.0;
  else if (i == 3) v = sel;
  else if (i == MCBA_LM_CFL) v = cfl;
  else if (i == MCBA_LM_CFL_SWITCH) v = cfl_switch;
  lms[i] = v;
}
void launch_lm_init(hipStream_t st, const double* red_scal, double* lms, double lam0, int sel, double cfl, double cfl_switch, double* clear8) {
  static_assert(MCBA_LMS <= 56, "threads 56..63 of k_lm_init clear the eight release words");
  k_lm_init<<<dim3(1), dim3(64), 0, st>>>(red_scal, lms, lam0, (double)sel, cfl, cfl_switch, clear8);
}

__global__ __launch_bounds__(256) void k_pack_result(const double* __restrict__ x, const double* __restrict__ gc, const double* __restrict__ fbuf, const unsigned char* __restrict__ fixed, double* __restrict__ out, int C, int F,
                                                     int cw) {
  const size_t nx = (size_t)12 * C + (size_t)6 * F, i = (size_t)blockIdx.x * 256 + threadIdx.x;
  if (i >= nx) return;
  out[i] = x[i];
  double g;
  if (i < (size_t)12 * C) {
    const int c = (int)i / 12, k = (int)i % 12;
    const int row = cw == 12 ? (int)i : (k >= 6 ? 6 * c + (k - 6) : -1);
    g = row >= 0 && !(fixed && fixed[row]) ? gc[row] : 0.0;
  } else {
    const size_t j = i - (size_t)12 * C, f = j / 6, k = j - 6 * f;
    g = fbuf[f * MCBA_FB + 27 + k];
  }
  out[nx + i] = g;
}
void launch_pack_result(hipStream_t st, const double* x, const double* gc, const double* fbuf, const unsigned char* fixed, double* out, int C, int F, int cw) {
  const size_t nx = (size_t)12 * C + (size_t)6 * F;
  k_pack_result<<<dim3((unsigned)((nx + 255) / 256)), dim3(256), 0, st>>>(x, gc, fbuf, fixed, out, C, F, cw);
}

void launch_decide(hipStream_t st, const double* trial8, DecideArgs da) {
  k_decide<<<dim3(1), dim3(64), 0, st>>>(trial8, da);
}

void launch_jacobian(hipStream_t st, int loss, double f_scale, const double* obs_raw, const double* obj, const double* x, double* jac, double* res, int C, int F, int N, int Fpad, int robust) {
  if (loss == LOSS_TABLE) { loss = LOSS_LINEAR; robust = 0; }
  double fs2 = f_scale * f_scale, ifs2 = 1.0 / fs2;
  (void)with_loss(loss, [&](auto L) { return launch(k_jacobian<decltype(L)::value>, dim3(F, C), dim3(64), 0, st, reinterpret_cast<const double2*>(obs_raw), obj, x, jac, res, C, F, N, Fpad, robust, fs2, ifs2); });
}

static int raise_lds_limit(const void* kernel, size_t bytes) { return (int)hipFuncSetAttribute(kernel, hipFuncAttributeMaxDynamicSharedMemorySize, (int)bytes); }

int gram_psplit_set_lds_limit() {
  int rc = 0;
  for_each_int(LossList{}, [&](auto L) { for_each_bool([&](auto FAST) { for_each_int(GramNpwList{}, [&](auto NPW) {
    constexpr int l = decltype(L)::value, npw = decltype(NPW)::value;
    constexpr bool fast = decltype(FAST)::value;
    static_assert(gram_xch_doubles(npw, false) * sizeof(double) <= 64 * 1024, "k_gram_psplit<..., ROLE 0> needs the LDS opt-in too");
    for (const void* k : {reinterpret_cast<const void*>(k_gram_psplit<l, fast, npw, 2>), reinterpret_cast<const void*>(k_gram_mixed<l, fast, npw>)}) {
      const int r = raise_lds_limit(k, kGramPsplitLdsMax);
      rc = rc ? rc : r;
    }
  }); }); });
  return rc;
}

int syrk_set_lds_limit(size_t bytes) {
  int rc = 0;
  for_each_int(SyrkShapeList{}, [&](auto SHAPE) { for_each_bool([&](auto DECIDE) { for_each_bool([&](auto XS) {
    const int r = raise_lds_limit(reinterpret_cast<const void*>(syrk_kernel<decltype(SHAPE)::value, decltype(DECIDE)::value, decltype(XS)::value>), bytes);
    rc = rc ? rc : r;
  }); }); });
  return rc;
}

}
```

Baseline: 9893.

## Pack 72-row Schur SYRK into 12 hand-picked 16x16 rectangles covering lower triangle

For the 6-camera, 12-parameter case (n=72), the SYRK stage now covers the symmetric Schur complement with 12 packed 16x16 MFMA tiles built from 8-row groups, instead of the generic tile list over a padded 73-column matrix. The RHS column is dropped from the MFMA tiles and computed as a per-row scalar dot product accumulated in registers, written to a new rpart buffer, and reduced in extra tail tasks of the reduce kernel. This is meant to cut redundant MFMA tiles and padding work, LDS rows and reduction blocks. The cost is a specialized kernel shape (smaller items per thread, PPW=3) and a fixed hard-coded covering that only applies when C*12 equals 72.

```diff
diff --git a/multicam-calibration_amd/build.py b/multicam-calibration_amd/build.py
--- a/multicam-calibration_amd/build.py
+++ b/multicam-calibration_amd/build.py
@@ -11,7 +11,7 @@
            "mcba_prefilter_api.hip", "mcba_calib_api.hip", "mcba_geom_api.hip", "mcba_comm_api.hip", "mcba_sparse.hip", "mcba_sparse_api.hip", "mcba_detect.hip", "mcba_keypoints.hip", "mcba_consensus.hip", "mcba_cov.hip", "mcba_cov_api.hip",
            "mcba_tricov.hip", "mcba_tricov_api.hip", "mcba_kpba.hip", "mcba_kpba_tiled.hip", "mcba_kpba_api.hip", "mcba_kpcam.hip", "mcba_kpcam_api.hip", "mcba_twoview.hip", "mcba_fivepoint.hip", "mcba_twoview_api.hip", "mcba_resect.hip", "mcba_resect_p3p.hip", "mcba_resect_api.hip",
            "mcba_smooth.hip", "mcba_smooth_api.hip", "mcba_smooth_cov.hip", "mcba_smooth_cov_api.hip", "mcba_traj_refine.hip", "mcba_traj_refine_api.hip"]
-DEPS = SOURCES + ["mcba_gram_finish.inc", "mcba_math.h", "mcba_geom_math.h", "mcba_pnp_math.h", "mcba_keypoint_math.h", "mcba_consensus_math.h", "mcba_cov_math.h", "mcba_tricov_math.h", "mcba_kpba_math.h", "mcba_kpcam_math.h", "mcba_detect_math.h", "mcba_twoview_math.h", "mcba_fivepoint_math.h", "mcba_resect_math.h", "mcba_resect_p3p_math.h", "mcba_smooth_math.h", "mcba_smooth_cov_math.h", "mcba_traj_refine_math.h", "mcba_smooth_host.h", "mcba_hyp_score.h", "mcba_ransac_host.h", "mcba_device.h", "mcba_quadform.h", "mcba_backsub.h", "mcba_kernels.h", "mcba_gram_plan.h", "mcba_lm.h", "mcba_lm_state.h", "mcba_handle.h", os.path.join("..", "..", "include", "mcba.h")]
+DEPS = SOURCES + ["mcba_gram_finish.inc", "mcba_math.h", "mcba_geom_math.h", "mcba_pnp_math.h", "mcba_keypoint_math.h", "mcba_consensus_math.h", "mcba_cov_math.h", "mcba_tricov_math.h", "mcba_kpba_math.h", "mcba_kpcam_math.h", "mcba_detect_math.h", "mcba_twoview_math.h", "mcba_fivepoint_math.h", "mcba_resect_math.h", "mcba_resect_p3p_math.h", "mcba_smooth_math.h", "mcba_smooth_cov_math.h", "mcba_traj_refine_math.h", "mcba_smooth_host.h", "mcba_hyp_score.h", "mcba_ransac_host.h", "mcba_device.h", "mcba_quadform.h", "mcba_backsub.h", "mcba_kernels.h", "mcba_gram_plan.h", "mcba_syrk_pack.h", "mcba_lm.h", "mcba_lm_state.h", "mcba_handle.h", os.path.join("..", "..", "include", "mcba.h")]
 
 
 SCHED_FLAGS = ["-mllvm", "-amdgpu-disable-unclustered-high-rp-reschedule=1", "-mllvm", "-greedy-reverse-local-assignment=1"]
diff --git a/multicam-calibration_amd/csrc/mcba_api.hip b/multicam-calibration_amd/csrc/mcba_api.hip
--- a/multicam-calibration_amd/csrc/mcba_api.hip
+++ b/multicam-calibration_amd/csrc/mcba_api.hip
@@ -144,6 +144,9 @@
       h->G = (nstage + h->sq - 1) / h->sq;
     }
   }
+  h->syrk_pack = mcba::syrk_pack_applies(C, h->cw, h->FS);
+  if (const char* e = getenv("MCBA_SYRK_PACK")) h->syrk_pack = h->syrk_pack && atoi(e) != 0;
+  if (h->syrk_pack) h->NP = mcba::kSyrkPackRects;
   }
   h->nbblocks = h->Fpad / 64;
   {
@@ -210,7 +213,7 @@
                       {&h->swork, n_swork}, {&h->dscale, h->nx}, {reinterpret_cast<double**>(&h->fixed), ((size_t)h->n + 7) / 8},
                       {&h->sp_damp, h->sparse ? (size_t)h->npad : 0}, {&h->sp_y, h->sparse ? (size_t)h->npad : 0}, {reinterpret_cast<double**>(&h->sp_ctl), h->sparse ? (size_t)1 : 0}};
     Piece plain[] = {{&h->rec2[0], (size_t)h->Fpad * C * MCBA_REC}, {&h->rec2[1], (size_t)h->Fpad * C * MCBA_REC},
-                     {&h->spart, (size_t)h->G * h->NP * 256 + 64},
+                     {&h->spart, (size_t)h->G * h->NP * 256 + 64}, {&h->rpart, h->syrk_pack ? (size_t)mcba::kSyrkPackN * h->G : 0},
                      {&h->gchunk, h->gram.chunk_doubles()}};
     auto padded = [](size_t count) { return (std::max<size_t>(count, 1) * sizeof(double) + 255) / 256 * 256; };
     size_t zero_bytes = 0, total = 0;
@@ -247,7 +250,7 @@
     h->pinned_bytes = (h->nsys + 8 + MCBA_LMS + h->n) * sizeof(double);
     HIPCHK(pool_host_malloc(reinterpret_cast<void**>(&h->pinned), h->pinned_bytes, hipHostMallocDefault));
   }
-  size_t lds = h->sparse ? 0 : mcba::syrk_lds_bytes(C, h->FS, h->cw);
+  size_t lds = h->sparse ? 0 : mcba::syrk_lds_bytes(C, h->FS, h->cw, h->syrk_pack);
   if (lds > 64 * 1024) {
     if (mcba::syrk_set_lds_limit(lds) != 0) return fail(MCBA_ERR_HIP, "cannot raise the dynamic LDS limit of k_syrk");
   }
@@ -309,7 +312,7 @@
     if (fz.decide) return fail(MCBA_ERR_ARG, "sparse-Schur handle: the decision is not fused into the Schur reduction");
     return sparse_build(h, sel);
   }
-  { Scope sc(h, K_SYRK); mcba::launch_syrk(h->stream, sel, fz, h->rec2[0], h->rec2[1], h->fbuf, h->fpart, h->tile_i, h->tile_j, h->spart, h->C, h->F, h->Fpad, h->NT, h->NP, h->G, h->sq, h->sr, h->FS, h->ppw, h->have_xscale ? h->dscale : nullptr, h->cw); }
+  { Scope sc(h, K_SYRK); mcba::launch_syrk(h->stream, sel, fz, h->rec2[0], h->rec2[1], h->fbuf, h->fpart, h->tile_i, h->tile_j, h->spart, h->C, h->F, h->Fpad, h->NT, h->NP, h->G, h->sq, h->sr, h->FS, h->ppw, h->have_xscale ? h->dscale : nullptr, h->cw, h->syrk_pack ? h->rpart : nullptr); }
   return check_launch();
 }
 
@@ -317,7 +320,7 @@
   {
     Scope sc(h, K_REDUCE);
     mcba::launch_reduce_system(h->stream, sel, h->gpart2[0], h->gpart2[1], h->spart, h->fpart, h->tile_i, h->tile_j, h->red, h->C, h->nfb, h->G, h->NT, h->NP, h->nfblocks, rank_slot,
-                               spec ? h->bpart : nullptr, h->nbblocks, spec ? post_state(h) : nullptr, h->cw, spec ? timeout_word(h) : nullptr, (double)h->last_solve_seq);
+                               spec ? h->bpart : nullptr, h->nbblocks, spec ? post_state(h) : nullptr, h->cw, spec ? timeout_word(h) : nullptr, (double)h->last_solve_seq, h->syrk_pack ? h->rpart : nullptr);
   }
   return check_launch();
 }
@@ -432,7 +435,7 @@
     *b.slot = nullptr;
   }
   h->bufs.swap(kept);
-  h->rec2[0] = h->rec2[1] = h->gpart2[0] = h->gpart2[1] = h->fbuf = h->fpart = h->spart = h->cpart = h->bpart = h->red_own = h->red = h->dcbuf = h->swork = h->dscale = h->gchunk = nullptr;
+  h->rec2[0] = h->rec2[1] = h->gpart2[0] = h->gpart2[1] = h->fbuf = h->fpart = h->spart = h->rpart = h->cpart = h->bpart = h->red_own = h->red = h->dcbuf = h->swork = h->dscale = h->gchunk = nullptr;
   h->fixed = nullptr;
   sparse_forget(h);
   h->cal_out_cap = h->cal_rel_cap = h->cal_sel_cap = h->cal_views_cap = 0;
diff --git a/multicam-calibration_amd/csrc/mcba_handle.h b/multicam-calibration_amd/csrc/mcba_handle.h
--- a/multicam-calibration_amd/csrc/mcba_handle.h
+++ b/multicam-calibration_amd/csrc/mcba_handle.h
@@ -61,6 +61,8 @@
   double* obj_host = nullptr;
   int planar = 0;
   int *tile_i = nullptr, *tile_j = nullptr;
+  bool syrk_pack = false;
+  double* rpart = nullptr;
   int NT = 0, NP = 0, G = 0, sq = 0, sr = 0, FS = 0, ppw = 4, nfblocks = 0, nbblocks = 0, nch = 1;
   mcba::GramPlan gram;
   double* gchunk = nullptr;
diff --git a/multicam-calibration_amd/csrc/mcba_kernels.h b/multicam-calibration_amd/csrc/mcba_kernels.h
--- a/multicam-calibration_amd/csrc/mcba_kernels.h
+++ b/multicam-calibration_amd/csrc/mcba_kernels.h
@@ -9,6 +9,7 @@
 #define MCBA_FB 40
 
 #include "mcba_gram_plan.h"
+#include "mcba_syrk_pack.h"
 #include "mcba_lm_state.h"
 #include "mcba_math.h"
 
@@ -104,14 +105,17 @@
 int gram_psplit_set_lds_limit();
 void launch_cost(hipStream_t st, int loss, double f_scale, const double* obs_t, const double* obj, const double* x, double* cpart, double* res, int C, int F, int N, int Fpad, int nch,
                  double fill = 0.0);
-size_t syrk_lds_bytes(int C, int FS, int cw = 12);
+size_t syrk_lds_bytes(int C, int FS, int cw = 12, bool pack = false);
 void launch_syrk(hipStream_t st, Sel s, const SyrkFuse& fz, const double* rec0, const double* rec1, double* fbuf, double* fpart, const int* tile_i, const int* tile_j, double* spart, int C, int F, int Fpad, int NT, int NP, int G, int sq, int sr, int FS, int ppw,
                  const double* dscale = nullptr,
-                 int cw = 12);
+                 int cw = 12,
+                 double* rpart = nullptr);
 int syrk_items_per_thread();
+bool syrk_pack_applies(int C, int cw, int FS);
 void launch_reduce_system(hipStream_t st, Sel s, const double* gp0, const double* gp1, const double* spart, const double* fpart, const int* tile_i, const int* tile_j, double* red, int C, int nfb, int G, int NT, int NP, int nfblocks, int rank_slot,
                           const double* bpart = nullptr, int nbp = 0, double* state_copy = nullptr, int cw = 12,
-                          const double* timeout_word = nullptr, double seq_prev = 0.0);
+                          const double* timeout_word = nullptr, double seq_prev = 0.0,
+                          const double* rpart = nullptr);
 void launch_backsub(hipStream_t st, Sel s, const double* rec0, const double* rec1, const double* fbuf, const CamStep& dc, double* x0, double* x1, double* bpart, int C, int F, int Fpad, int cw = 12);
 void launch_backsub_dev(hipStream_t st, Sel s, const double* rec0, const double* rec1, const double* fbuf, const double* dc_dev, double* x0, double* x1, double* bpart, int C, int F, int Fpad, int cw = 12);
 size_t solve_lds_bytes(int npad, int use_lds);
diff --git a/multicam-calibration_amd/csrc/mcba_kernels.hip b/multicam-calibration_amd/csrc/mcba_kernels.hip
--- a/multicam-calibration_amd/csrc/mcba_kernels.hip
+++ b/multicam-calibration_amd/csrc/mcba_kernels.hip
@@ -804,10 +804,10 @@
 typedef double mfma_d4 __attribute__((ext_vector_type(4)));
 constexpr int kSyrkSuper = 32;
 
-template <int PPW, int IPT, bool DECIDE, bool XS, int CW = 12>
+template <int PPW, int IPT, bool DECIDE, bool XS, int CW = 12, bool PACK = false>
 __global__ __launch_bounds__(256, PPW <= 4 ? 2 : 1) void k_syrk(Sel sl, SyrkFuse fz, const double* __restrict__ rec0, const double* __restrict__ rec1, double* __restrict__ fbuf, double* __restrict__ fpart,
                                               const int* __restrict__ tile_i, const int* __restrict__ tile_j, double* __restrict__ spart, int C, int F, int Fpad, int NT, int NP, int sq, int sr, int FS,
-                                              const double* __restrict__ dscale, int xg, int yg) {
+                                              const double* __restrict__ dscale, int xg, int yg, double* __restrict__ rpart) {
   int bx = blockIdx.x, by = blockIdx.y, gx = gridDim.x;
   if (xg > 0) {
     const int id = blockIdx.x, xcd = id & 7, slot = id >> 3, nfull = xg >> 3;
@@ -895,14 +895,25 @@
   const double* __restrict__ rec = sidx ? rec1 : rec0;
   const int n = CW * C, nfb = Fpad >> 6;
   const int RS = 6 * FS + 2;
+  const int yrows = PACK ? kSyrkPackN : NT * 16;
   double* s_y = lds;
-  double* s_L = lds + (size_t)NT * 16 * RS;
+  double* s_L = lds + (size_t)yrows * RS;
 
   int qi[PPW], rowa[PPW], rowb[PPW];
   mfma_d4 acc[PPW];
 #pragma unroll
   for (int k = 0; k < PPW; ++k) {
     int q = by * (4 * PPW) + wave + 4 * k;
+    if (PACK) {
+      unsigned w = syrk_pack_word(4 * k);
+#pragma unroll
+      for (int j = 1; j < 4; ++j) w = wave == j ? syrk_pack_word(4 * k + j) : w;
+      qi[k] = q;
+      rowa[k] = syrk_pack_a_offset(w, lane, RS);
+      rowb[k] = syrk_pack_b_offset(w, lane, RS);
+      acc[k] = mfma_d4{0.0, 0.0, 0.0, 0.0};
+      continue;
+    }
     qi[k] = q < NP ? q : -1;
     int ti = 0, tj = 0;
     if (q < NP) {
@@ -914,7 +925,10 @@
     rowb[k] = (16 * tj + (lane & 15)) * RS + (lane >> 4);
     acc[k] = mfma_d4{0.0, 0.0, 0.0, 0.0};
   }
-  for (int i = t; i < (NT * 16 - (n + 1)) * RS; i += 256) s_y[(size_t)(n + 1) * RS + i] = 0.0;
+  if (!PACK) { for (int i = t; i < (NT * 16 - (n + 1)) * RS; i += 256) s_y[(size_t)(n + 1) * RS + i] = 0.0; }
+  double racc[IPT];
+#pragma unroll
+  for (int it = 0; it < IPT; ++it) racc[it] = 0.0;
 
   const int f0 = (bx * sq + min(bx, sr)) * FS, f1 = min(F, f0 + (sq + (bx < sr ? 1 : 0)) * FS);
   double wreg[IPT][6];
@@ -1033,16 +1047,16 @@
     SLAP(0);
     for (int fb = s0; fb < s1; fb += FS) {
       {
-        double Lr[27];
+        double Lr[PACK ? 33 : 27];
         const double* Lp = s_L + (fb - s0 + tb) * 34;
 #pragma unroll
-        for (int k = 0; k < 27; ++k) Lr[k] = Lp[k];
+        for (int k = 0; k < (PACK ? 33 : 27); ++k) Lr[k] = Lp[k];
         const bool live = fb + tb < F;
         const unsigned fm = XS ? (unsigned)Lp[33] : 0u;
 #pragma unroll
         for (int it = 0; it < IPT; ++it) {
           const int row = tr0 + rstep * it;
-          if (row <= n) {
+          if (PACK ? row < n : row <= n) {
             double* dst = s_y + (size_t)row * RS + tb * 6;
             if (row < n) {
               double yr[6];
@@ -1052,7 +1066,11 @@
               }
               fwd6(Lr, Lr + 21, wreg[it], yr);
 #pragma unroll
-              for (int k = 0; k < 6; ++k) dst[k] = live ? yr[k] : 0.0;
+              for (int k = 0; k < 6; ++k) {
+                const double y = live ? yr[k] : 0.0;
+                dst[k] = y;
+                if (PACK) racc[it] = fma(y, Lr[27 + k], racc[it]);
+              }
             } else {
 #pragma unroll
               for (int k = 0; k < 6; ++k) dst[k] = Lp[27 + k];
@@ -1092,6 +1110,15 @@
     const double wm = wave_max(gmax), wn = wave_sum63(nfail);
     if (lane == 63) { fpart[2 * bx] = wm; fpart[2 * bx + 1] = wn; }
   }
+  if (PACK) {
+#pragma unroll
+    for (int it = 0; it < IPT; ++it) {
+      double v = racc[it];
+      for (int off = 1; off < FS; off <<= 1) v += __shfl_xor(v, off, 64);
+      const int row = tr0 + rstep * it;
+      if (row < n && tb == 0) rpart[(size_t)row * gx + bx] = v;
+    }
+  }
 #pragma unroll
   for (int k = 0; k < PPW; ++k) {
     if (qi[k] >= 0) {
@@ -1113,11 +1140,11 @@
   return wave_sum63(s);
 }
 
-template <int RR>
+template <int RR, bool PACK = false>
 __global__ __launch_bounds__(1024) void k_reduce_system(Sel sl, const double* __restrict__ gp0, const double* __restrict__ gp1, const double* __restrict__ spart, const double* __restrict__ fpart,
                                                         const int* __restrict__ tile_i, const int* __restrict__ tile_j, double* __restrict__ red, int C, int nfb, int G, int NT, int NP,
                                                         int nfblocks, int rank_slot, const double* __restrict__ bpart, int nbp, double* __restrict__ state_copy, int cw,
-                                                        const double* __restrict__ timeout_word, double seq_prev) {
+                                                        const double* __restrict__ timeout_word, double seq_prev, const double* __restrict__ rpart) {
   const int n = cw * C, coff = 12 - cw;
   const int wave = threadIdx.x >> 6, lane = threadIdx.x & 63;
   __shared__ double s_part[RR][16][64];
@@ -1126,7 +1153,8 @@
   constexpr int BPQ = 16 / RR;
   if ((int)blockIdx.x < BPQ * NP) {
     const int q = blockIdx.x / BPQ, reg = RR == 1 ? (blockIdx.x >> 2) & 3 : blockIdx.x & 3, rr0 = RR == 1 ? blockIdx.x & 3 : 0;
-    const int ti = tile_i[q], tj = tile_j[q];
+    const int ti = PACK ? 0 : tile_i[q], tj = PACK ? 0 : tile_j[q];
+    const unsigned pw = PACK ? syrk_pack_word(q) : 0u;
     const int rg = lane >> 4, el = lane & 15;
     constexpr int NK = RR == 1 ? 8 : 2;
     double pv[RR][NK];
@@ -1142,12 +1170,12 @@
 #pragma unroll
     for (int r = 0; r < RR; ++r) {
       up[r] = nullptr;
-      const int row = 16 * ti + (rr0 + r) + 4 * reg, col = 16 * tj + wave;
+      const int row = PACK ? syrk_pack_a_row(pw, (rr0 + r) + 4 * reg) : 16 * ti + (rr0 + r) + 4 * reg, col = PACK ? syrk_pack_b_row(pw, wave) : 16 * tj + wave;
       if (row < n && col < n && row / cw == col / cw) {
         int cam = row / cw, li = row - cw * cam + coff, lj = col - cw * cam + coff;
         int a = li <= lj ? li : lj, b2 = li <= lj ? lj : li;
         up[r] = gpart + cam * camstride + (size_t)tri12(a, b2) * nfb;
-      } else if (col == n && row < n) {
+      } else if (!PACK && col == n && row < n) {
         int cam = row / cw, li = row - cw * cam + coff;
         up[r] = gpart + cam * camstride + (size_t)(78 + li) * nfb;
       }
@@ -1181,7 +1209,14 @@
 #pragma unroll
       for (int k = 0; k < 16; ++k) t += s_part[r][k][lane];
       const double v = (__shfl(t, el, 64) + __shfl(t, el + 16, 64)) + (__shfl(t, el + 32, 64) + __shfl(t, el + 48, 64));
-      if (lane < 16) {
+      if (PACK) {
+        int row, col;
+        if (lane < 16 && syrk_pack_elem(pw, reg, 16 * (rr0 + r) + el, row, col)) {
+          const double out = s_u[r][el] - v;
+          red[(size_t)row * n + col] = out;
+          if (row != col) red[(size_t)col * n + row] = out;
+        }
+      } else if (lane < 16) {
         const int row = 16 * ti + (rr0 + r) + 4 * reg, col = 16 * tj + el;
         if (row < n && col < n) {
           double out = s_u[r][el] - v;
@@ -1261,6 +1296,11 @@
     if (lane == 63) tail[2 * n + 16 + jj] = v;
   } else if (bpart && state_copy && task == 2 * n + 24) {
     if (lane < MCBA_LMS) state_copy[lane] = sl.lms[lane];
+  } else if (PACK && task >= 2 * n + 25 && task < 3 * n + 25) {
+    const int jj = task - (2 * n + 25), cam = jj / cw, l = jj - cw * cam + coff;
+    const double yz = run_sum(rpart + (size_t)jj * G, G, lane);
+    const double gc = run_sum(gpart + cam * camstride + (size_t)(78 + l) * nfb, nfb, lane);
+    if (lane == 63) red[(size_t)n * n + jj] = yz - gc;
   }
 }
 
@@ -1465,40 +1505,48 @@
   }); });
 }
 
-size_t syrk_lds_bytes(int C, int FS, int cw) {
+size_t syrk_lds_bytes(int C, int FS, int cw, bool pack) {
   int NT = (cw * C + 1 + 15) / 16;
-  return ((size_t)NT * 16 * (6 * FS + 2) + (size_t)kSyrkSuper * (34 + 28)) * sizeof(double);
+  return ((size_t)(pack ? kSyrkPackN : NT * 16) * (6 * FS + 2) + (size_t)kSyrkSuper * (34 + 28)) * sizeof(double);
 }
 
 constexpr int kSyrkIpt = 5, kSyrkIptSmall = 3;
-struct SyrkShape { int ppw, ipt, cw; };
-constexpr SyrkShape kSyrkShapes[] = {{4, kSyrkIpt, 12}, {4, kSyrkIptSmall, 12}, {16, kSyrkIpt, 12}, {4, kSyrkIpt, 6}, {4, kSyrkIptSmall, 6}};
-using SyrkShapeList = IntList<0, 1, 2, 3, 4>;
+struct SyrkShape { int ppw, ipt, cw; bool pack; };
+constexpr SyrkShape kSyrkShapes[] = {{4, kSyrkIpt, 12, false}, {4, kSyrkIptSmall, 12, false}, {16, kSyrkIpt, 12, false}, {4, kSyrkIpt, 6, false}, {4, kSyrkIptSmall, 6, false},
+                                     {3, kSyrkIptSmall, 12, true}};
+using SyrkShapeList = IntList<0, 1, 2, 3, 4, 5>;
 template <int SHAPE, bool DECIDE, bool XS>
-constexpr auto syrk_kernel = k_syrk<kSyrkShapes[SHAPE].ppw, kSyrkShapes[SHAPE].ipt, DECIDE, XS, kSyrkShapes[SHAPE].cw>;
+constexpr auto syrk_kernel = k_syrk<kSyrkShapes[SHAPE].ppw, kSyrkShapes[SHAPE].ipt, DECIDE, XS, kSyrkShapes[SHAPE].cw, kSyrkShapes[SHAPE].pack>;
 
 void launch_syrk(hipStream_t st, Sel s, const SyrkFuse& fz, const double* rec0, const double* rec1, double* fbuf, double* fpart, const int* tile_i, const int* tile_j, double* spart, int C, int F, int Fpad, int NT, int NP, int G, int sq, int sr, int FS, int ppw,
-                 const double* dscale, int cw) {
-  const size_t lds = syrk_lds_bytes(C, FS, cw);
+                 const double* dscale, int cw, double* rpart) {
+  const bool pack = rpart != nullptr;
+  const size_t lds = syrk_lds_bytes(C, FS, cw, pack);
   const bool small = (cw * C + 1) * FS <= 256 * kSyrkIptSmall;
-  const int shape = cw == 6 ? (small ? 4 : 3) : ppw <= 4 ? (small ? 1 : 0) : 2;
+  const int shape = pack ? 5 : cw == 6 ? (small ? 4 : 3) : ppw <= 4 ? (small ? 1 : 0) : 2;
   const int gy = (NP + 4 * kSyrkShapes[shape].ppw - 1) / (4 * kSyrkShapes[shape].ppw);
   const bool remap = gy > 1;
   const dim3 grid(remap ? 8 * ((G / 8) * gy + ((G % 8) * gy + 7) / 8) : G, remap ? 1 : gy);
   const int xg = remap ? G : 0, yg = remap ? gy : 0;
   (void)with_int(SyrkShapeList{}, shape, [&](auto SHAPE) { return with_bool(fz.decide != 0, [&](auto DECIDE) { return with_bool(dscale != nullptr, [&](auto XS) {
-    return launch(syrk_kernel<decltype(SHAPE)::value, decltype(DECIDE)::value, decltype(XS)::value>, grid, dim3(256), lds, st, s, fz, rec0, rec1, fbuf, fpart, tile_i, tile_j, spart, C, F, Fpad, NT, NP, sq, sr, FS, dscale, xg, yg);
+    return launch(syrk_kernel<decltype(SHAPE)::value, decltype(DECIDE)::value, decltype(XS)::value>, grid, dim3(256), lds, st, s, fz, rec0, rec1, fbuf, fpart, tile_i, tile_j, spart, C, F, Fpad, NT, NP, sq, sr, FS, dscale, xg, yg, rpart);
   }); }); });
 }
 
 int syrk_items_per_thread() { return kSyrkIpt; }
+bool syrk_pack_applies(int C, int cw, int FS) { return cw == 12 && cw * C == kSyrkPackN && kSyrkPackN * FS <= 256 * kSyrkIptSmall; }
 
 void launch_reduce_system(hipStream_t st, Sel s, const double* gp0, const double* gp1, const double* spart, const double* fpart, const int* tile_i, const int* tile_j, double* red, int C, int nfb, int G, int NT, int NP, int nfblocks, int rank_slot,
-                          const double* bpart, int nbp, double* state_copy, int cw, const double* timeout_word, double seq_prev) {
+                          const double* bpart, int nbp, double* state_copy, int cw, const double* timeout_word, double seq_prev, const double* rpart) {
   int n = cw * C;
   int tail_blocks = (2 * n + 16 + (bpart ? 9 : 0) + 15) / 16;
-  if (NP >= 64 && G <= 128) k_reduce_system<4><<<dim3(4 * NP + tail_blocks), dim3(1024), 0, st>>>(s, gp0, gp1, spart, fpart, tile_i, tile_j, red, C, nfb, G, NT, NP, nfblocks, rank_slot, bpart, nbp, state_copy, cw, timeout_word, seq_prev);
-  else k_reduce_system<1><<<dim3(16 * NP + tail_blocks), dim3(1024), 0, st>>>(s, gp0, gp1, spart, fpart, tile_i, tile_j, red, C, nfb, G, NT, NP, nfblocks, rank_slot, bpart, nbp, state_copy, cw, timeout_word, seq_prev);
+  if (rpart) {
+    tail_blocks = (3 * n + 25 + 15) / 16;
+    k_reduce_system<1, true><<<dim3(16 * NP + tail_blocks), dim3(1024), 0, st>>>(s, gp0, gp1, spart, fpart, tile_i, tile_j, red, C, nfb, G, NT, NP, nfblocks, rank_slot, bpart, nbp, state_copy, cw, timeout_word, seq_prev, rpart);
+    return;
+  }
+  if (NP >= 64 && G <= 128) k_reduce_system<4><<<dim3(4 * NP + tail_blocks), dim3(1024), 0, st>>>(s, gp0, gp1, spart, fpart, tile_i, tile_j, red, C, nfb, G, NT, NP, nfblocks, rank_slot, bpart, nbp, state_copy, cw, timeout_word, seq_prev, nullptr);
+  else k_reduce_system<1><<<dim3(16 * NP + tail_blocks), dim3(1024), 0, st>>>(s, gp0, gp1, spart, fpart, tile_i, tile_j, red, C, nfb, G, NT, NP, nfblocks, rank_slot, bpart, nbp, state_copy, cw, timeout_word, seq_prev, nullptr);
 }
 
 template <class DcSrc>
diff --git a/multicam-calibration_amd/csrc/mcba_syrk_pack.h b/multicam-calibration_amd/csrc/mcba_syrk_pack.h
--- /dev/null
+++ b/multicam-calibration_amd/csrc/mcba_syrk_pack.h
@@ -0,0 +1,47 @@
+#pragma once
+
+#if defined(__HIPCC__)
+#define MCBA_PACK_HD __host__ __device__ __forceinline__
+#else
+#define MCBA_PACK_HD inline
+#endif
+
+namespace mcba {
+
+constexpr int kSyrkPackN = 72, kSyrkPackRects = 12;
+
+#define MCBA_PACK_RECT(x, p, q, d) ((unsigned)((x) | ((p) << 4) | ((q) << 8) | ((d) << 12)))
+MCBA_PACK_HD constexpr unsigned syrk_pack_word(int r) {
+  switch (r) {
+    case 0: return MCBA_PACK_RECT(1, 0, 2, 1);
+    case 1: return MCBA_PACK_RECT(4, 3, 5, 1);
+    case 2: return MCBA_PACK_RECT(7, 6, 8, 1);
+    case 3: return MCBA_PACK_RECT(3, 0, 6, 1);
+    case 4: return MCBA_PACK_RECT(4, 1, 7, 0);
+    case 5: return MCBA_PACK_RECT(5, 2, 8, 1);
+    case 6: return MCBA_PACK_RECT(0, 4, 8, 1);
+    case 7: return MCBA_PACK_RECT(6, 1, 5, 1);
+    case 8: return MCBA_PACK_RECT(2, 3, 7, 1);
+    case 9: return MCBA_PACK_RECT(0, 5, 7, 0);
+    case 10: return MCBA_PACK_RECT(8, 1, 3, 1);
+    default: return MCBA_PACK_RECT(2, 4, 6, 0);
+  }
+}
+#undef MCBA_PACK_RECT
+
+MCBA_PACK_HD constexpr int syrk_pack_a_group(unsigned w, int m) { return (int)((m < 8 ? w : w >> 4) & 15u); }
+MCBA_PACK_HD constexpr int syrk_pack_b_group(unsigned w, int m) { return (int)((m < 8 ? w : w >> 8) & 15u); }
+MCBA_PACK_HD constexpr int syrk_pack_a_row(unsigned w, int m) { return 8 * syrk_pack_a_group(w, m) + (m & 7); }
+MCBA_PACK_HD constexpr int syrk_pack_b_row(unsigned w, int m) { return 8 * syrk_pack_b_group(w, m) + (m & 7); }
+MCBA_PACK_HD constexpr int syrk_pack_a_offset(unsigned w, int lane, int rs) { return syrk_pack_a_row(w, lane & 15) * rs + (lane >> 4); }
+MCBA_PACK_HD constexpr int syrk_pack_b_offset(unsigned w, int lane, int rs) { return syrk_pack_b_row(w, lane & 15) * rs + (lane >> 4); }
+
+MCBA_PACK_HD constexpr bool syrk_pack_elem(unsigned w, int reg, int lane, int& row, int& col) {
+  const int i = (lane >> 4) + 4 * reg, j = lane & 15;
+  const int a = syrk_pack_a_row(w, i), b = syrk_pack_b_row(w, j);
+  row = a >= b ? a : b;
+  col = a >= b ? b : a;
+  return (i >= 8 || j >= 8) ? true : (((w >> 12) & 1u) != 0 && a >= b);
+}
+
+}
```

After: 9980, median of 6. Within noise of the previous version (+0.9%).
